# saiakarsh193/GenVox

Hardware: AMD Instinct MI355X
Metric: mel-frames/sec (teacher-forced batch) (higher is better)
Workload: dtype f32

## Files before the change

### genvox_amd/csrc/dec_resident.hip

```cpp
#include "gvx_kernels.h"

namespace gvx {

namespace {

using f32x16 = __attribute__((ext_vector_type(16))) float;

constexpr int RS_WAVES = 8;
constexpr int RS_THREADS = RS_WAVES * 64;
constexpr int RS_A = 1024, RS_D = 1024, RS_E = 512, RS_P = 256, RS_ATT = 128;
constexpr int RS_NKGW_ATT = (RS_P + RS_E + RS_A) / 8;
constexpr int RS_NKGW_DEC = (RS_A + RS_E + RS_D) / 8;
constexpr int RS_KG0_ATT = RS_P / 8;

template <int KIND> struct RsCfg {
    static constexpr bool XH = KIND == 0, ATT = KIND != 2;
    static constexpr int RT = KIND == 3 ? 2 : 1;
    static constexpr int NN = ATT ? 16 : 32, NC = 8;
    static constexpr int NRN = KIND == 0 ? 7 : (KIND == 1 ? 16 : (KIND == 2 ? 17 : 9));
    static constexpr int NLN = NN - NRN;
    static constexpr int WAVE_W = NLN * (XH ? 1536 : 1024 * RT);
    static constexpr int OFF_RED = RS_WAVES * WAVE_W;
    static constexpr int OFF_RED2 = OFF_RED + RS_WAVES * 16 * 64 * 4;
    static constexpr int OFF_HS = OFF_RED2 + (XH ? RS_WAVES * 8 * 64 * 4 : 0);
    static constexpr int OFF_HS2 = OFF_HS + 32 * 8 * 4 * RT;
    static constexpr int OFF_CTRL = OFF_HS2 + 32 * 4 * 4;
    static constexpr int LDS_BYTES = OFF_CTRL + 256;
};
constexpr int RS_LDS_BYTES = RsCfg<0>::LDS_BYTES > RsCfg<2>::LDS_BYTES ? RsCfg<0>::LDS_BYTES : RsCfg<2>::LDS_BYTES;
static_assert(RS_LDS_BYTES <= 160 * 1024 && RsCfg<1>::LDS_BYTES <= RS_LDS_BYTES && RsCfg<3>::LDS_BYTES <= RS_LDS_BYTES, "resident decoder LDS");
constexpr int RC_HA = 0;
constexpr int RC_CTX = 1;
constexpr int RC_HD = 2;
constexpr int RC_ABORT = 3;
constexpr int RC_LOCK = 4;
constexpr int RC_IDLE = 5;
constexpr int RC_PRE = 6;
constexpr int RC_Y1 = 7;
constexpr int RC_EXIT = 8;
constexpr int RC_WANT = 10;

struct RsArgs {
    const float* att_frag; const float* att_bias; const float* wq_t; const float* dec_frag; const float* dec_bias;
    const float* pre_gate;
    const float* proj_hd_t; const float* proj_ctx_t; const float* pre_w1; const uint8_t* keep1;
    float* prenet; const float* y1; float* p_slab; const int32_t* n_done; int PSB;
    float* h_a; float* hc; float* q_slab; float* c_a; float* c_d;
    const uint8_t* tr_keep_a; const uint8_t* tr_keep_d; float* tr_c_a; float* tr_c_d; float* tr_pre_a; float* tr_pre_d;
    float tr_scale_a, tr_scale_d;
    unsigned* sync;
    unsigned att_frag_bytes;
    int B, T;
    unsigned spin_limit;
    int debug, layout;
    int kg_pre;
};

#ifdef GVX_STAMPS
constexpr int RS_STAMP_T = 20;
__device__ unsigned long long rs_stamps[4][10][16];
__device__ unsigned long long rs_wg_stamps[224][4];
__device__ unsigned long long rs_wg_stamps_ar[224][4];
#define RS_STAMP(ev) do { if (stamp_wg && t == RS_STAMP_T && lane == 0) rs_stamps[KIND][wave][ev] = wall_clock64(); } while (0)
#define RS_WGSTAMP(i) do { if (t == RS_STAMP_T && tid == 0) rs_wg_stamps[bid][i] = wall_clock64(); } while (0)
#define RS_ARSTAMP(i) do { if (t == RS_STAMP_T && tid == 0) rs_wg_stamps_ar[bid][i] = wall_clock64(); } while (0)
#else
#define RS_STAMP(ev) do { } while (0)
#define RS_WGSTAMP(i) do { } while (0)
#define RS_ARSTAMP(i) do { } while (0)
#endif

__device__ __forceinline__ float sigmoidf_(float x) { return __builtin_amdgcn_rcpf(1.f + __expf(-x)); }
__device__ __forceinline__ float tanhf_(float x) { return 1.f - 2.f * __builtin_amdgcn_rcpf(__expf(2.f * x) + 1.f); }

struct RsPoll {
    const unsigned* f_att; const unsigned* f_dec; const unsigned* f_ctx; unsigned* tmo;
    const unsigned* f_pre; const unsigned* f_y1; const unsigned* stop;
    unsigned limit; int B, T, bid;
    int n_att;
    int sleep;
};

__device__ __forceinline__ bool rs_count(int* ctrl, int word, unsigned v, unsigned Tu, int lane) {
    const unsigned s0 = (unsigned)__hip_atomic_load(ctrl + word, __ATOMIC_RELAXED, __HIP_MEMORY_SCOPE_WORKGROUP);
    unsigned n = s0;
    while (n < Tu && __all(v > n)) ++n;
    if (lane == 0 && n != s0) __hip_atomic_store(ctrl + word, (int)n, __ATOMIC_RELEASE, __HIP_MEMORY_SCOPE_WORKGROUP);
    return n != s0;
}
__device__ __forceinline__ void rs_poll_once(int* ctrl, const RsPoll& q, int lane, int mask) {
    constexpr unsigned none = 0xffffffffu;
    unsigned va = none, vd = none, vc = none, vp = none, vy = none;
    if (mask & (1 << RC_HA)) {
        const unsigned a0 = __hip_atomic_load(q.f_att + lane, __ATOMIC_RELAXED, __HIP_MEMORY_SCOPE_AGENT);
        const unsigned a1 = lane + 64 < q.n_att ? __hip_atomic_load(q.f_att + 64 + lane, __ATOMIC_RELAXED, __HIP_MEMORY_SCOPE_AGENT) : none;
        va = min(a0, a1);
    }
    if (mask & (1 << RC_HD)) {
        const unsigned d0 = __hip_atomic_load(q.f_dec + lane, __ATOMIC_RELAXED, __HIP_MEMORY_SCOPE_AGENT);
        const unsigned d1 = __hip_atomic_load(q.f_dec + 64 + lane, __ATOMIC_RELAXED, __HIP_MEMORY_SCOPE_AGENT);
        vd = min(d0, d1);
    }
    if (mask & (1 << RC_CTX)) vc = lane < q.B ? __hip_atomic_load(q.f_ctx + lane * 32, __ATOMIC_RELAXED, __HIP_MEMORY_SCOPE_AGENT) : none;
    if (q.f_pre) {
        if (mask & (1 << RC_PRE)) vp = lane < 8 ? __hip_atomic_load(q.f_pre + lane * 32, __ATOMIC_RELAXED, __HIP_MEMORY_SCOPE_AGENT) : none;
        if (mask & (1 << RC_Y1)) vy = lane < q.B ? __hip_atomic_load(q.f_y1 + lane * 32, __ATOMIC_RELAXED, __HIP_MEMORY_SCOPE_AGENT) : none;
    }
    __builtin_amdgcn_fence(__ATOMIC_ACQUIRE, "wavefront");
    const unsigned Tu = (unsigned)q.T;
    bool moved = false;
    if (mask & (1 << RC_HA)) moved |= rs_count(ctrl, RC_HA, va, Tu, lane);
    if (mask & (1 << RC_HD)) moved |= rs_count(ctrl, RC_HD, vd, Tu, lane);
    if (mask & (1 << RC_CTX)) moved |= rs_count(ctrl, RC_CTX, vc, Tu, lane);
    if (q.f_pre) {
        if (mask & (1 << RC_PRE)) moved |= rs_count(ctrl, RC_PRE, vp, Tu, lane);
        if (mask & (1 << RC_Y1)) moved |= rs_count(ctrl, RC_Y1, vy, Tu, lane);
    }
    int idle = 0;
    if (lane == 0) {
        idle = moved ? 0 : __hip_atomic_load(ctrl + RC_IDLE, __ATOMIC_RELAXED, __HIP_MEMORY_SCOPE_WORKGROUP) + 1;
        __hip_atomic_store(ctrl + RC_IDLE, idle, __ATOMIC_RELAXED, __HIP_MEMORY_SCOPE_WORKGROUP);
    }
    idle = __builtin_amdgcn_readfirstlane(idle);
    if (idle == 0 || (idle & 15) != 0) return;
    bool give_up = __hip_atomic_load(q.tmo, __ATOMIC_RELAXED, __HIP_MEMORY_SCOPE_AGENT) != 0u;
    if (q.stop && __hip_atomic_load(q.stop, __ATOMIC_RELAXED, __HIP_MEMORY_SCOPE_AGENT) != 0u) give_up = true;
    if ((unsigned)idle > q.limit) {
        if (lane == 0) __hip_atomic_store(q.tmo, 0x500u + (unsigned)(q.bid & 0xff), __ATOMIC_RELAXED, __HIP_MEMORY_SCOPE_AGENT);
        give_up = true;
    }
    if (give_up && lane == 0) __hip_atomic_store(ctrl + RC_ABORT, 1, __ATOMIC_RELEASE, __HIP_MEMORY_SCOPE_WORKGROUP);
}

__device__ __forceinline__ void rs_gate(int* ctrl, int word, int need, const RsPoll& q, int lane) {
    while (__hip_atomic_load(ctrl + word, __ATOMIC_ACQUIRE, __HIP_MEMORY_SCOPE_WORKGROUP) < need) {
        if (__hip_atomic_load(ctrl + RC_ABORT, __ATOMIC_RELAXED, __HIP_MEMORY_SCOPE_WORKGROUP) != 0) return;
        int got = 0;
        if (lane == 0) {
            int expect = 0;
            got = __hip_atomic_compare_exchange_strong(ctrl + RC_LOCK, &expect, 1, __ATOMIC_ACQUIRE, __ATOMIC_RELAXED, __HIP_MEMORY_SCOPE_WORKGROUP) ? 1 : 0;
            if (got) got = __hip_atomic_exchange(ctrl + RC_WANT, 0, __ATOMIC_RELAXED, __HIP_MEMORY_SCOPE_WORKGROUP) | (1 << word);
            else __hip_atomic_fetch_or(ctrl + RC_WANT, 1 << word, __ATOMIC_RELAXED, __HIP_MEMORY_SCOPE_WORKGROUP);
        }
        got = __builtin_amdgcn_readfirstlane(got);
        if (got) {
            rs_poll_once(ctrl, q, lane, got);
            if (lane == 0) __hip_atomic_store(ctrl + RC_LOCK, 0, __ATOMIC_RELEASE, __HIP_MEMORY_SCOPE_WORKGROUP);
            if (q.sleep == 8) __builtin_amdgcn_s_sleep(8);
            else if (q.sleep == 32) __builtin_amdgcn_s_sleep(32);
        } else {
            __builtin_amdgcn_s_sleep(1);
        }
    }
}
__device__ __forceinline__ void rs_cbar() {
    asm volatile("s_waitcnt lgkmcnt(0)" ::: "memory");
    __builtin_amdgcn_s_barrier();
    asm volatile("" ::: "memory");
}

typedef __attribute__((ext_vector_type(4))) unsigned rs_u32x4;
__device__ __forceinline__ rs_u32x4 rs_rsrc(const void* p, unsigned bytes) {
    const unsigned long long a = reinterpret_cast<unsigned long long>(p);
    rs_u32x4 r;
    r.x = (unsigned)a; r.y = (unsigned)(a >> 32) & 0xffffu; r.z = bytes; r.w = 0x00020000u;
    return r;
}
__device__ __forceinline__ void rs_glds(rs_u32x4 rsrc, unsigned voff, unsigned soff, unsigned lds_addr) {
    unsigned keep;
    asm volatile("s_mov_b32 %0, m0\n\ts_mov_b32 m0, %1\n\ts_nop 0\n\tbuffer_load_dwordx4 %2, %3, %4 offen lds\n\ts_mov_b32 m0, %0"
                 : "=&s"(keep) : "s"(lds_addr), "v"(voff), "s"(rsrc), "s"(soff) : "memory");
}

#define RS_MFMA32(W, X)                                                   \
    acc = __builtin_amdgcn_mfma_f32_32x32x2f32((W).x, (X).x, acc, 0, 0, 0); \
    acc = __builtin_amdgcn_mfma_f32_32x32x2f32((W).y, (X).y, acc, 0, 0, 0); \
    acc = __builtin_amdgcn_mfma_f32_32x32x2f32((W).z, (X).z, acc, 0, 0, 0); \
    acc = __builtin_amdgcn_mfma_f32_32x32x2f32((W).w, (X).w, acc, 0, 0, 0);
#define RS_MFMA32B(W, X)                                                    \
    acc2 = __builtin_amdgcn_mfma_f32_32x32x2f32((W).x, (X).x, acc2, 0, 0, 0); \
    acc2 = __builtin_amdgcn_mfma_f32_32x32x2f32((W).y, (X).y, acc2, 0, 0, 0); \
    acc2 = __builtin_amdgcn_mfma_f32_32x32x2f32((W).z, (X).z, acc2, 0, 0, 0); \
    acc2 = __builtin_amdgcn_mfma_f32_32x32x2f32((W).w, (X).w, acc2, 0, 0, 0);
#define RS_MFMA16(W, X)                                                     \
    acc2 = __builtin_amdgcn_mfma_f32_16x16x1f32((W).x, (X).x, acc2, 0, 0, 0); \
    acc2 = __builtin_amdgcn_mfma_f32_16x16x1f32((W).y, (X).y, acc2, 0, 0, 0); \
    acc2 = __builtin_amdgcn_mfma_f32_16x16x1f32((W).z, (X).z, acc2, 0, 0, 0); \
    acc2 = __builtin_amdgcn_mfma_f32_16x16x1f32((W).w, (X).w, acc2, 0, 0, 0);

#define RS_VFMAC(A, W, X) asm("v_fmac_f32 %0, %1, %2" : "+v"(A) : "v"(W), "v"(X));
#define RS_VDOT(A, W, X) RS_VFMAC(A, (W).x, (X).x) RS_VFMAC(A, (W).y, (X).y) RS_VFMAC(A, (W).z, (X).z) RS_VFMAC(A, (W).w, (X).w)
#define RS_DPPSWAP(v) __int_as_float(__builtin_amdgcn_update_dpp(0, __float_as_int(v), 0xB1, 0xF, 0xF, true))
#define RS_XROW1(X) make_float4(RS_DPPSWAP((X).x), RS_DPPSWAP((X).y), RS_DPPSWAP((X).z), RS_DPPSWAP((X).w))
#define RS_MUL32(W, X) if (V) { RS_VDOT(av[0], W, X) if (two_rows) { const float4 x1_ = RS_XROW1(X); RS_VDOT(av[1], W, x1_) } } else { RS_MFMA32(W, X) }
#define RS_MUL32B(W, X) if (V) { RS_VDOT(av2[0], W, X) if (two_rows) { const float4 x1_ = RS_XROW1(X); RS_VDOT(av2[1], W, x1_) } } else { RS_MFMA32B(W, X) }
#define RS_MUL16(W, X) if (V) { RS_VDOT(av2[0], W, X) if (two_rows) { const float4 x1_ = RS_XROW1(X); RS_VDOT(av2[1], W, x1_) } } else { RS_MFMA16(W, X) }
template <bool B> struct RsBool { static constexpr bool value = B; };

}

typedef const __attribute__((address_space(4))) RsArgs* RsKarg;

template <int KIND, bool AR, bool TR = false, bool KA = AR>
__device__ __forceinline__ void rs_body(const RsArgs& p, char* smem, const int bid) {
    static_assert(!(AR && TR), "the tape belongs to the teacher-forced loop");
    using Cfg = RsCfg<KIND>;
    constexpr bool XH = Cfg::XH, ATT = Cfg::ATT;
    constexpr int NN = Cfg::NN, NC = Cfg::NC, NRN = Cfg::NRN, NLN = Cfg::NLN;
    constexpr int NKGW = ATT ? RS_NKGW_ATT : RS_NKGW_DEC;
    constexpr int H = ATT ? RS_A : RS_D;
    constexpr int NRH = XH ? NRN : 1, NCH = XH ? NC : 1;
    constexpr int RT = Cfg::RT;
    constexpr int NR2 = RT == 2 ? NRN : 1, NC2 = RT == 2 ? NC : 1;

    const int dec0 = p.layout == 2 ? 64 : 96;
    int tile, xt = 0, xhalf = 0;
    if (KIND == 0) { const int m = bid >> 1, odd = bid & 1; tile = 3 * m + 2 * odd; xt = 3 * m + 1; xhalf = odd; }
    else if (KIND == 1) tile = 96 + (bid - 64);
    else if (KIND == 3) tile = 2 * bid;
    else tile = bid - dec0;

    int* ctrl = reinterpret_cast<int*>(smem + Cfg::OFF_CTRL);
    float* red = reinterpret_cast<float*>(smem + Cfg::OFF_RED);
    float* red2 = reinterpret_cast<float*>(smem + Cfg::OFF_RED2);
    float* hs = reinterpret_cast<float*>(smem + Cfg::OFF_HS);
    float* hs2 = reinterpret_cast<float*>(smem + Cfg::OFF_HS2);
    const int tid = threadIdx.x, lane = tid & 63;
    const int wave = __builtin_amdgcn_readfirstlane(tid >> 6);
    const int B = p.B, T = p.T;
    const unsigned blkb = (unsigned)B * 32u;
    unsigned* const tmo_w = p.sync + HANDOFF_TIMEOUT;
    const int rep = bid % RS_REP;
    const RsPoll poll{p.sync + RS_FLAG_ATT + rep * 128, p.sync + RS_FLAG_DEC + rep * 128, p.sync + RS_FLAG_CTX + (bid % RS_REP1) * 32 * 32, tmo_w,
                      AR ? p.sync + RS_FLAG_PRE + (bid % RS_REP_PRE) * 8 * 32 : nullptr, AR ? p.sync + RS_FLAG_Y1 : nullptr, AR ? p.sync + HANDOFF_STOP : nullptr,
                      (p.spin_limit ? p.spin_limit : HANDOFF_SPIN_LIMIT) * 16u, B, T, bid, dec0,
                      (!ATT && (p.debug & 16)) ? 32 : ((p.debug & 8) ? 8 : 0)};
    const int bl = lane & 31, h = lane >> 5;
    const bool x_mine = ((lane >> 4) & 1) == xhalf;
    const int mlane = x_mine ? lane : (lane ^ 16);
    const bool vmode = B <= 2 && !(p.debug & 64), two_rows = B == 2;
    const unsigned x_lane = (unsigned)((vmode ? (two_rows ? (bl & 1) : 0) : (bl < B ? bl : 0)) * 8 + 4 * h) * 4u;

    const float4* wsrc = reinterpret_cast<const float4*>(ATT ? p.att_frag : p.dec_frag);
    constexpr bool ARD = AR && KIND == 2;
    constexpr bool PP = AR && ATT;
    constexpr int NSUB = ARD ? 2 : 1;
    const int kg_pre = AR ? RS_KG0_ATT : __builtin_amdgcn_readfirstlane(p.kg_pre);
    const int nkgw = ATT ? kg_pre + (RS_E + RS_A) / 8 : RS_NKGW_DEC;
    const int kn0 = ATT ? kg_pre + 64 + 16 * wave : (wave < 4 ? 32 * wave : 32 * wave + 64);
    auto kni = [&](int i) -> int { return ARD ? (i < 16 ? 192 + 16 * wave + i : 16 * wave + (i - 16)) : kn0 + i; };
    const int kc0 = ATT ? kg_pre + 8 * wave : 128 + 8 * wave;
    const float4* wt = wsrc + (long)tile * nkgw * 64 + lane;
    const float4* wx = wsrc + (long)xt * nkgw * 64 + mlane;
    float4 wn[NRN], wc[NC], hn[NRH], hc[NCH], wn2[NR2], wc2[NC2];
    const float4* wt2 = wt + (long)nkgw * 64;
#pragma unroll
    for (int i = 0; i < NRN; ++i) wn[i] = wt[(long)kni(i) * 64];
#pragma unroll
    for (int i = 0; i < NC; ++i) wc[i] = wt[(long)(kc0 + i) * 64];
#pragma unroll
    for (int i = 0; i < NR2; ++i) wn2[i] = RT == 2 ? wt2[(long)kni(i) * 64] : make_float4(0.f, 0.f, 0.f, 0.f);
#pragma unroll
    for (int i = 0; i < NC2; ++i) wc2[i] = RT == 2 ? wt2[(long)(kc0 + i) * 64] : make_float4(0.f, 0.f, 0.f, 0.f);
#pragma unroll
    for (int i = 0; i < NRH; ++i) hn[i] = XH ? wx[(long)kni(i) * 64] : make_float4(0.f, 0.f, 0.f, 0.f);
#pragma unroll
    for (int i = 0; i < NCH; ++i) hc[i] = XH ? wx[(long)(kc0 + i) * 64] : make_float4(0.f, 0.f, 0.f, 0.f);
    float4* lw = reinterpret_cast<float4*>(smem + wave * Cfg::WAVE_W);
    float4* lh = lw + NLN * 64;
    const int hidx = (mlane & 15) + 16 * (mlane >> 5);
#pragma unroll
    for (int i = 0; i < NLN; ++i) {
        lw[i * RT * 64 + lane] = wt[(long)kni(NRN + i) * 64];
        if (RT == 2) lw[(i * RT + 1) * 64 + lane] = wt2[(long)kni(NRN + i) * 64];
        if (XH && x_mine) lh[i * 32 + hidx] = wx[(long)kni(NRN + i) * 64];
    }

    constexpr int NP = (PP && KIND == 1) ? 4 : 1;
    float4 wp[NP], w1f[NP];
    const bool l2_wg = AR && KIND == 1 && bid - 64 < 8;
#pragma unroll
    for (int i = 0; i < NP; ++i) {
        wp[i] = (PP && KIND == 1) ? wt[(long)(4 * wave + i) * 64] : make_float4(0.f, 0.f, 0.f, 0.f);
        w1f[i] = l2_wg ? *reinterpret_cast<const float4*>(p.pre_w1 + (long)(32 * (bid - 64) + bl) * RS_P + 8 * (4 * wave + i) + 4 * h) : make_float4(0.f, 0.f, 0.f, 0.f);
    }
    const rs_u32x4 rw_att = rs_rsrc(p.att_frag, p.att_frag_bytes);
    const unsigned lds_base = (unsigned)(unsigned long long)(__attribute__((address_space(3))) char*)smem;
    const unsigned stage_t = lds_base + (unsigned)Cfg::OFF_RED + (unsigned)wave * 4096u;
    const unsigned stage_h = lds_base + (unsigned)Cfg::OFF_RED2 + (unsigned)wave * 2048u;
    const unsigned v_half = (((unsigned)bl < 16u ? 16u * (unsigned)xhalf + (unsigned)bl : 32u + 16u * (unsigned)xhalf + ((unsigned)bl - 16u)) * 16u) + (unsigned)h * 1024u;

    const bool cell_wave = wave < 4 * RT;
    const bool cell2_wave = XH && (wave == 4 || wave == 5);
    const int ctile = tile + (RT == 2 ? (wave >> 2) : 0);
    const int g = wave & 3, jloc = 2 * g + h, j = ctile * 8 + jloc;
    const int b2 = (lane & 15) + 16 * (wave - 4), g2 = lane >> 4, jloc2 = 4 * xhalf + g2, j2 = xt * 8 + jloc2;
    float* c_mem = ATT ? p.c_a : p.c_d;
    const float* bias = ATT ? p.att_bias : p.dec_bias;
    float c_state = 0.f;
    float4 bias4 = make_float4(0.f, 0.f, 0.f, 0.f);
    if (cell_wave) {
        if (bl < B) c_state = c_mem[(long)bl * H + j];
        bias4 = *reinterpret_cast<const float4*>(bias + ctile * 32 + 8 * g + 4 * h);
    } else if (cell2_wave) {
        if (b2 < B) c_state = c_mem[(long)b2 * H + j2];
        bias4 = *reinterpret_cast<const float4*>(bias + xt * 32 + 4 * jloc2);
    }
    const bool slab_wave = ATT ? wave < RS_ATT / 32 : (AR && wave < 3);

#ifdef GVX_STAMPS
    const bool stamp_wg = bid == 0 || bid == 64 || bid == dec0;
#endif
    for (int t = 0; t < T; ++t) {
        RS_STAMP(0);
        RS_WGSTAMP(0);
        RsKarg ka = nullptr;
        if (KA) { ka = (RsKarg)__builtin_amdgcn_kernarg_segment_ptr(); asm volatile("" : "+s"(ka)); }
        if (ATT && !AR && !TR && t >= RS_HA_SLOTS && (wave == 6 || ((XH || RT == 2) && wave == 7))) rs_gate(ctrl, RC_HD, t + 1 - RS_HA_SLOTS, poll, lane);
        float4 add4 = bias4;
        if (PP && XH) {
            const unsigned kg = (unsigned)(4 * wave);
#pragma unroll
            for (int i = 0; i < 4; ++i) rs_glds(rw_att, (unsigned)lane * 16u, ((unsigned)tile * NKGW + kg + (unsigned)i) * 1024u, stage_t + (unsigned)i * 1024u);
#pragma unroll
            for (int i = 0; i < 2; ++i) rs_glds(rw_att, v_half, ((unsigned)xt * NKGW + kg + 2u * (unsigned)i) * 1024u, stage_h + (unsigned)i * 1024u);
        }
        if (ATT && !PP) {
            if (cell_wave && bl < B) {
                const float4 ad = *reinterpret_cast<const float4*>(p.pre_gate + ((long)t * B + bl) * 4 * RS_A + ctile * 32 + 8 * g + 4 * h);
                add4.x += ad.x; add4.y += ad.y; add4.z += ad.z; add4.w += ad.w;
            } else if (cell2_wave && b2 < B) {
                const float4 ad = *reinterpret_cast<const float4*>(p.pre_gate + ((long)t * B + b2) * 4 * RS_A + xt * 32 + 4 * jloc2);
                add4.x += ad.x; add4.y += ad.y; add4.z += ad.z; add4.w += ad.w;
            }
        }
        f32x16 acc2x;
        float av2x[2] = {0.f, 0.f};
        auto body = [&](auto vc) __attribute__((always_inline)) {
        constexpr bool V = decltype(vc)::value;
        f32x16 acc, acc2;
#pragma unroll
        for (int q = 0; q < 16; ++q) { acc[q] = 0.f; acc2[q] = 0.f; }
        float av[2] = {0.f, 0.f}, av2[2] = {0.f, 0.f};
        auto prenet_part = [&]() __attribute__((always_inline)) {
            rs_gate(ctrl, RC_PRE, t, poll, lane);
            RS_ARSTAMP(2);
            const __amdgpu_buffer_rsrc_t rx = make_rsrc(ka->prenet + (long)(4 * wave) * B * 8);
            float4 xp[4];
#pragma unroll
            for (int u = 0; u < 4; ++u) xp[u] = load_sc1(rx, x_lane + (unsigned)u * blkb);
            if (XH) {
                asm volatile("s_waitcnt vmcnt(0)" ::: "memory");
                const float4* st = reinterpret_cast<const float4*>(red + wave * 16 * 64);
                const float4* sh = reinterpret_cast<const float4*>(red2 + wave * 8 * 64);
#pragma unroll
                for (int u = 0; u < 4; ++u) {
                    const float4 wl = st[u * 64 + lane];
                    const float4 hl = sh[u * 32 + hidx];
                    RS_MUL32(wl, xp[u])
                    RS_MUL16(hl, xp[u])
                }
            } else {
#pragma unroll
                for (int u = 0; u < 4; ++u) { RS_MUL32(wp[u < NP ? u : 0], xp[u]) }
            }
        };

        {
#pragma unroll
        for (int sub = 0; sub < NSUB; ++sub) {
            const float* xsrc;
            int word, need;
            if (ATT) { xsrc = p.h_a + (long)(TR ? t : t % RS_HA_SLOTS) * RS_A * B + (long)(16 * wave) * B * 8; word = RC_HA; need = t; }
            else if (ARD && sub == 0) { xsrc = p.hc + (long)t * B * (RS_D + RS_E) + (long)(16 * wave) * B * 8; word = RC_HD; need = t; }
            else if (ARD) { xsrc = p.h_a + (long)((t + 1) % RS_HA_SLOTS) * RS_A * B + (long)(16 * wave) * B * 8; word = RC_HA; need = t + 1; }
            else if (wave < 4) { xsrc = p.h_a + (long)(TR ? t + 1 : (t + 1) % RS_HA_SLOTS) * RS_A * B + (long)(32 * wave) * B * 8; word = RC_HA; need = t + 1; }
            else { xsrc = p.hc + (long)t * B * (RS_D + RS_E) + (long)(32 * (wave - 4)) * B * 8; word = RC_HD; need = t; }
            rs_gate(ctrl, word, need, poll, lane);
            if (sub == NSUB - 1) { RS_STAMP(1); RS_WGSTAMP(1); }
            const __amdgpu_buffer_rsrc_t rx = make_rsrc(xsrc);
            constexpr int XG = (XH || RT == 2) ? 2 : 4;
            constexpr int XD = ARD ? 3 : 2;
            constexpr int NNS = NN / NSUB;
            float4 xb[XD][XG];
#pragma unroll
            for (int d = 0; d < XD - 1; ++d)
#pragma unroll
                for (int u = 0; u < XG; ++u) xb[d][u] = load_sc1(rx, x_lane + (unsigned)(XG * d + u) * blkb);
#pragma unroll
            for (int gi = 0; gi < NNS / XG; ++gi) {
                if (gi + XD - 1 < NNS / XG) {
#pragma unroll
                    for (int u = 0; u < XG; ++u) xb[(gi + XD - 1) % XD][u] = load_sc1(rx, x_lane + (unsigned)(XG * (gi + XD - 1) + u) * blkb);
                }
#pragma unroll
                for (int u = 0; u < XG; ++u) {
                    const int i = sub * NNS + XG * gi + u;
                    const float4 xv = xb[gi % XD][u];
                    if (i < NRN) {
                        RS_MUL32(wn[i], xv)
                        if (XH) { RS_MUL16(hn[i < NRH ? i : 0], xv) }
                        if (RT == 2) { RS_MUL32B(wn2[i < NR2 ? i : 0], xv) }
                    } else {
                        const float4 wl = lw[(i - NRN) * RT * 64 + lane];
                        RS_MUL32(wl, xv)
                        if (XH) { const float4 hl = lh[(i - NRN) * 32 + hidx]; RS_MUL16(hl, xv) }
                        if (RT == 2) { const float4 wl2 = lw[((i - NRN) * RT + 1) * 64 + lane]; RS_MUL32B(wl2, xv) }
                    }
                }
            }
        }
        }
        RS_STAMP(2);
        {
            const float* xsrc = p.hc + (long)(ATT ? t : t + 1) * B * (RS_D + RS_E) + (long)RS_D * B + (long)(8 * wave) * B * 8;
            if (ATT) rs_gate(ctrl, RC_CTX, t, poll, lane);
            else if (AR) rs_gate(ctrl, RC_CTX, t + 1, poll, lane);
            else if (t + 2 <= T) rs_gate(ctrl, RC_HA, t + 2, poll, lane);
            else rs_gate(ctrl, RC_CTX, t + 1, poll, lane);
            RS_STAMP(3);
            RS_WGSTAMP(2);
            const __amdgpu_buffer_rsrc_t rx = make_rsrc(xsrc);
            constexpr int XG = 4;
            float4 xc[XG], xn[XG];
#pragma unroll
            for (int u = 0; u < XG; ++u) xc[u] = load_sc1(rx, x_lane + (unsigned)u * blkb);
#pragma unroll
            for (int gi = 0; gi < NC / XG; ++gi) {
                if (gi + 1 < NC / XG) {
#pragma unroll
                    for (int u = 0; u < XG; ++u) xn[u] = load_sc1(rx, x_lane + (unsigned)(XG * (gi + 1) + u) * blkb);
                }
#pragma unroll
                for (int u = 0; u < XG; ++u) {
                    const int i = XG * gi + u;
                    RS_MUL32(wc[i], xc[u])
                    if (XH) { RS_MUL16(hc[i < NCH ? i : 0], xc[u]) }
                    if (RT == 2) { RS_MUL32B(wc2[i < NC2 ? i : 0], xc[u]) }
                }
#pragma unroll
                for (int u = 0; u < XG; ++u) xc[u] = xn[u];
            }
        }
        if (AR && KIND == 1) {
            if (l2_wg && t >= 1) {
                unsigned km = 0;
                if (wave < 4 && bl < B) km = *reinterpret_cast<const unsigned*>(ka->keep1 + ((long)t * B + bl) * RS_P + 32 * (bid - 64) + 8 * wave + 4 * h);
                rs_gate(ctrl, RC_Y1, t, poll, lane);
                RS_ARSTAMP(0);
                const __amdgpu_buffer_rsrc_t ry = make_rsrc(ka->y1 + (long)(4 * wave) * B * 8);
                float4 xy[4];
#pragma unroll
                for (int u = 0; u < 4; ++u) xy[u] = load_sc1(ry, x_lane + (unsigned)u * blkb);
                if (bid == 64 && tid == 0 && __hip_atomic_load(ka->n_done, __ATOMIC_RELAXED, __HIP_MEMORY_SCOPE_AGENT) >= B) {
                    __hip_atomic_store(p.sync + HANDOFF_STOP, (unsigned)t, __ATOMIC_RELAXED, __HIP_MEMORY_SCOPE_AGENT);
                    __hip_atomic_store(ctrl + RC_ABORT, 2, __ATOMIC_RELAXED, __HIP_MEMORY_SCOPE_WORKGROUP);
                }
                if (V) {
#pragma unroll
                    for (int u = 0; u < 4; ++u) { RS_MUL32B(w1f[u < NP ? u : 0], xy[u]) }
                    if (two_rows && (lane & 1)) { const float s2 = av2[0]; av2[0] = av2[1]; av2[1] = s2; }
#pragma unroll
                    for (int b = 0; b < 2; ++b) {
                        av2[b] += __shfl_xor(av2[b], 32, 64);
                        if (h == 0 && b < B) red[(wave * 16 + 4 * (bl >> 3) + (bl & 3)) * 64 + b + 32 * ((bl >> 2) & 1)] = av2[b];
                        av2[b] = 0.f;
                    }
                } else {
#pragma unroll
                    for (int u = 0; u < 4; ++u) { RS_MFMA32B(w1f[u < NP ? u : 0], xy[u]) }
#pragma unroll
                    for (int q = 0; q < 16; ++q) { red[(wave * 16 + q) * 64 + lane] = acc2[q]; acc2[q] = 0.f; }
                }
                rs_cbar();
                if (wave < 4) {
                    float4 o;
                    float* op = &o.x;
#pragma unroll
                    for (int qq = 0; qq < 4; ++qq) {
                        float tt = 0.f;
#pragma unroll
                        for (int w = 0; w < RS_WAVES; ++w) tt += red[(w * 16 + 4 * wave + qq) * 64 + lane];
                        op[qq] = tt;
                    }
                    if (bl < B) {
                        o.x = (km & 0xffu) ? 2.f * fmaxf(o.x, 0.f) : 0.f;
                        o.y = (km & 0xff00u) ? 2.f * fmaxf(o.y, 0.f) : 0.f;
                        o.z = (km & 0xff0000u) ? 2.f * fmaxf(o.z, 0.f) : 0.f;
                        o.w = (km & 0xff000000u) ? 2.f * fmaxf(o.w, 0.f) : 0.f;
                        const __amdgpu_buffer_rsrc_t rp = make_rsrc(ka->prenet + (long)(4 * (bid - 64) + wave) * B * 8);
                        store_sc1(rp, (unsigned)(bl * 8 + 4 * h) * 4u, o);
                    }
                    asm volatile("s_waitcnt vmcnt(0)" ::: "memory");
                }
                rs_cbar();
                if (tid < RS_REP_PRE && __hip_atomic_load(ctrl + RC_ABORT, __ATOMIC_RELAXED, __HIP_MEMORY_SCOPE_WORKGROUP) == 0)
                    __hip_atomic_store(p.sync + RS_FLAG_PRE + (tid * 8 + (bid - 64)) * 32, (unsigned)t, __ATOMIC_RELAXED, __HIP_MEMORY_SCOPE_AGENT);
                RS_ARSTAMP(1);
            }
        }
        if (AR && PP) prenet_part();
        RS_STAMP(4);
        if (AR) RS_ARSTAMP(3);
        {
        int tr = tid;
        asm volatile("" : "+v"(tr));
        const int el = tr & 63;
        if (V) {
            const int en = el & 31;
            if (two_rows && (el & 1)) {
                const float s0 = av[0], s2 = av2[0];
                av[0] = av[1]; av[1] = s0; av2[0] = av2[1]; av2[1] = s2;
            }
#pragma unroll
            for (int b = 0; b < 2; ++b) {
                av[b] += __shfl_xor(av[b], 32, 64);
                if (XH || RT == 2) av2[b] += __shfl_xor(av2[b], 32, 64);
                if (el < 32 && b < B) red[(wave * 16 + 4 * (en >> 3) + (en & 3)) * 64 + b + 32 * ((en >> 2) & 1)] = av[b];
                if (XH && el < 32 && ((el >> 4) & 1) == xhalf && b < B) red2[(wave * 8 + (el & 3)) * 64 + b + 16 * ((el & 15) >> 2)] = av2[b];
            }
        } else {
#pragma unroll
            for (int q = 0; q < 16; ++q) red[(wave * 16 + q) * 64 + el] = acc[q];
            if (XH) {
#pragma unroll
                for (int q = 0; q < 8; ++q) red2[(wave * 8 + q) * 64 + el] = acc2[q] + acc2[8 + q];
            }
        }
        if (RT == 2) {
            if (V) { av2x[0] = av2[0]; av2x[1] = av2[1]; } else acc2x = acc2;
        }
        }
        };
        if (vmode) body(RsBool<true>{}); else body(RsBool<false>{});

        int te = tid;
        asm volatile("" : "+v"(te));
        const int el = te & 63, ebl = el & 31, eh = el >> 5;
        float4 wq_a = make_float4(0.f, 0.f, 0.f, 0.f), wq_b = wq_a, wq_c = wq_a, wq_d = wq_a;
        float4 xe = wq_a;
        if (AR && !ATT && slab_wave) {
            const int dd = min(32 * wave + ebl, ka->PSB - 1);
            const float* wp_l = ka->proj_hd_t + ((long)tile * ka->PSB + dd) * 8;
            wq_a = *reinterpret_cast<const float4*>(wp_l);
            wq_b = *reinterpret_cast<const float4*>(wp_l + 4);
            wq_c = *reinterpret_cast<const float4*>(ka->proj_ctx_t + ((long)tile * ka->PSB + dd) * 4);
            const __amdgpu_buffer_rsrc_t rc = make_rsrc(p.hc + (long)(t + 1) * B * (RS_D + RS_E) + (long)RS_D * B + (long)(tile >> 1) * B * 8);
            xe = load_sc1(rc, (unsigned)((ebl < B ? ebl : 0) * 8 + 4 * (tile & 1)) * 4u);
        }
        if (ATT && slab_wave) {
            const float* wq_l = p.wq_t + ((long)tile * RS_ATT + 32 * wave + ebl) * 8;
            wq_a = *reinterpret_cast<const float4*>(wq_l);
            wq_b = *reinterpret_cast<const float4*>(wq_l + 4);
            if (XH) wq_c = *reinterpret_cast<const float4*>(p.wq_t + ((long)xt * RS_ATT + 32 * wave + ebl) * 8 + 4 * xhalf);
            if (RT == 2) {
                const float* wq_l2 = p.wq_t + ((long)(tile + 1) * RS_ATT + 32 * wave + ebl) * 8;
                wq_c = *reinterpret_cast<const float4*>(wq_l2);
                wq_d = *reinterpret_cast<const float4*>(wq_l2 + 4);
            }
        }
        rs_cbar();
        RS_STAMP(5);
        if (cell2_wave) {
            const int rb = wave - 4;
            const int eb2 = (el & 15) + 16 * rb, eg2 = el >> 4;
            float s2[4];
#pragma unroll
            for (int qq = 0; qq < 4; ++qq) {
                float tt = 0.f;
#pragma unroll
                for (int w = 0; w < RS_WAVES; ++w) tt += red2[(w * 8 + 4 * rb + qq) * 64 + el];
                s2[qq] = tt;
            }
            float hval = 0.f;
            if (eb2 < B) {
                const float p0 = s2[0] + add4.x, p1 = s2[1] + add4.y, p2 = s2[2] + add4.z, p3 = s2[3] + add4.w;
                c_state = sigmoidf_(p1) * c_state + sigmoidf_(p0) * tanhf_(p2);
                hval = sigmoidf_(p3) * tanhf_(c_state);
                if (TR) {
                    RsKarg kq = (RsKarg)__builtin_amdgcn_kernarg_segment_ptr();
                    asm volatile("" : "+s"(kq));
                    const unsigned u = (unsigned)eb2 * (unsigned)H + (unsigned)(xt * 8 + 4 * xhalf + eg2);
                    const long tb = (long)t * B * H;
                    reinterpret_cast<float4*>(kq->tr_pre_a + tb * 4)[u] = make_float4(p0, p1, p2, p3);
                    (kq->tr_c_a + tb + (long)B * H)[u] = c_state;
                    hval = (kq->tr_keep_a + tb)[u] ? hval * kq->tr_scale_a : 0.f;
                }
            }
            hs2[eb2 * 4 + eg2] = hval;
        }
#pragma unroll
        for (int ph = 0; ph < RT; ++ph) {
            if (ph == 1) {
                rs_cbar();
                if (vmode) {
                    const int en = el & 31;
#pragma unroll
                    for (int b = 0; b < 2; ++b)
                        if (el < 32 && b < B) red[(wave * 16 + 4 * (en >> 3) + (en & 3)) * 64 + b + 32 * ((en >> 2) & 1)] = av2x[b];
                } else {
#pragma unroll
                    for (int q = 0; q < 16; ++q) red[(wave * 16 + q) * 64 + el] = acc2x[q];
                }
                rs_cbar();
            }
            if (cell_wave && (wave >> 2) == ph) {
                float s[4];
#pragma unroll
                for (int qq = 0; qq < 4; ++qq) {
                    float tt = 0.f;
#pragma unroll
                    for (int w = 0; w < RS_WAVES; ++w) tt += red[(w * 16 + 4 * g + qq) * 64 + el];
                    s[qq] = tt;
                }
                float hval = 0.f;
                if (ebl < B) {
                    const float p0 = s[0] + add4.x, p1 = s[1] + add4.y, p2 = s[2] + add4.z, p3 = s[3] + add4.w;
                    c_state = sigmoidf_(p1) * c_state + sigmoidf_(p0) * tanhf_(p2);
                    hval = sigmoidf_(p3) * tanhf_(c_state);
                    if (TR) {
                        RsKarg kq = (RsKarg)__builtin_amdgcn_kernarg_segment_ptr();
                        asm volatile("" : "+s"(kq));
                        const unsigned u = (unsigned)ebl * (unsigned)H + (unsigned)((tile + (RT == 2 ? ph : 0)) * 8 + 2 * g + eh);
                        const long tb = (long)t * B * H;
                        reinterpret_cast<float4*>((ATT ? kq->tr_pre_a : kq->tr_pre_d) + tb * 4)[u] = make_float4(p0, p1, p2, p3);
                        ((ATT ? kq->tr_c_a : kq->tr_c_d) + tb + (long)B * H)[u] = c_state;
                        hval = ((ATT ? kq->tr_keep_a : kq->tr_keep_d) + tb)[u] ? hval * (ATT ? kq->tr_scale_a : kq->tr_scale_d) : 0.f;
                    }
                }
                hs[(ebl * RT + ph) * 8 + 2 * g + eh] = hval;
            }
        }
        rs_cbar();
        RS_STAMP(6);

        float* hdst = ATT ? p.h_a + (long)(TR ? t + 1 : (t + 1) % RS_HA_SLOTS) * RS_A * B : p.hc + (long)(t + 1) * B * (RS_D + RS_E);
        if (slab_wave) {
            f32x16 qa;
#pragma unroll
            for (int q = 0; q < 16; ++q) qa[q] = 0.f;
            const float* hrow = hs + ebl * 8 * RT + eh;
            qa = __builtin_amdgcn_mfma_f32_32x32x2f32(hrow[0], eh ? wq_a.y : wq_a.x, qa, 0, 0, 0);
            qa = __builtin_amdgcn_mfma_f32_32x32x2f32(hrow[2], eh ? wq_a.w : wq_a.z, qa, 0, 0, 0);
            qa = __builtin_amdgcn_mfma_f32_32x32x2f32(hrow[4], eh ? wq_b.y : wq_b.x, qa, 0, 0, 0);
            qa = __builtin_amdgcn_mfma_f32_32x32x2f32(hrow[6], eh ? wq_b.w : wq_b.z, qa, 0, 0, 0);
            if (RT == 2) {
                qa = __builtin_amdgcn_mfma_f32_32x32x2f32(hrow[8], eh ? wq_c.y : wq_c.x, qa, 0, 0, 0);
                qa = __builtin_amdgcn_mfma_f32_32x32x2f32(hrow[10], eh ? wq_c.w : wq_c.z, qa, 0, 0, 0);
                qa = __builtin_amdgcn_mfma_f32_32x32x2f32(hrow[12], eh ? wq_d.y : wq_d.x, qa, 0, 0, 0);
                qa = __builtin_amdgcn_mfma_f32_32x32x2f32(hrow[14], eh ? wq_d.w : wq_d.z, qa, 0, 0, 0);
            }
            if (XH) {
                const float* hrow2 = hs2 + ebl * 4 + eh;
                qa = __builtin_amdgcn_mfma_f32_32x32x2f32(hrow2[0], eh ? wq_c.y : wq_c.x, qa, 0, 0, 0);
                qa = __builtin_amdgcn_mfma_f32_32x32x2f32(hrow2[2], eh ? wq_c.w : wq_c.z, qa, 0, 0, 0);
            }
            if (AR && !ATT) {
                qa = __builtin_amdgcn_mfma_f32_32x32x2f32(eh ? xe.y : xe.x, eh ? wq_c.y : wq_c.x, qa, 0, 0, 0);
                qa = __builtin_amdgcn_mfma_f32_32x32x2f32(eh ? xe.w : xe.z, eh ? wq_c.w : wq_c.z, qa, 0, 0, 0);
            }
            float* tq = red + wave * 16 * 64;
#pragma unroll
            for (int gg = 0; gg < 4; ++gg)
#pragma unroll
                for (int rr = 0; rr < 4; ++rr) tq[(8 * gg + 4 * eh + rr) * 32 + ebl] = qa[4 * gg + rr];
            const int sdim = ATT ? RS_ATT : ka->PSB;
            const __amdgpu_buffer_rsrc_t rq = make_rsrc(ATT ? p.q_slab + (long)bid * B * RS_ATT + 32 * wave : ka->p_slab + (long)tile * B * sdim + 32 * wave);
#pragma unroll
            for (int ps = 0; ps < 4; ++ps) {
                const int row = 8 * ps + (el >> 3), c4 = el & 7;
                const float4 v = *reinterpret_cast<const float4*>(tq + row * 32 + 4 * c4);
                if (row < B && (ATT || 32 * wave + 4 * c4 < sdim)) store_sc1(rq, (unsigned)(row * sdim + 4 * c4) * 4u, v);
            }
        } else if (wave == 6) {
            const __amdgpu_buffer_rsrc_t rh = make_rsrc(hdst + (long)tile * B * 8);
            if (4 * el < 8 * B) store_sc1(rh, (unsigned)el * 16u, *reinterpret_cast<const float4*>(hs + (el >> 1) * 8 * RT + 4 * (el & 1)));
        } else if (RT == 2 && wave == 7) {
            const __amdgpu_buffer_rsrc_t rh = make_rsrc(hdst + (long)(tile + 1) * B * 8);
            if (4 * el < 8 * B) store_sc1(rh, (unsigned)el * 16u, *reinterpret_cast<const float4*>(hs + (el >> 1) * 16 + 8 + 4 * (el & 1)));
        } else if (XH && wave == 7) {
            const __amdgpu_buffer_rsrc_t rh = make_rsrc(hdst + (long)xt * B * 8);
            if (el < B) store_sc1(rh, (unsigned)(el * 8 + 4 * xhalf) * 4u, *reinterpret_cast<const float4*>(hs2 + 4 * el));
        }
        RS_STAMP(7);
        asm volatile("s_waitcnt vmcnt(0)" ::: "memory");
        RS_STAMP(8);
        if (AR && tid == 0) ctrl[RC_EXIT + (t & 1)] = __hip_atomic_load(ctrl + RC_ABORT, __ATOMIC_RELAXED, __HIP_MEMORY_SCOPE_WORKGROUP);
        rs_cbar();
        RS_STAMP(9);
        const bool leave = AR && __builtin_amdgcn_readfirstlane(ctrl[RC_EXIT + (t & 1)]) != 0;
        if (leave) break;
        int tf = tid;
        asm volatile("" : "+v"(tf));
        if (tf < RS_REP) __hip_atomic_store(p.sync + (ATT ? RS_FLAG_ATT + bid : RS_FLAG_DEC + (bid - dec0)) + tf * 128, (unsigned)t + 1u, __ATOMIC_RELAXED, __HIP_MEMORY_SCOPE_AGENT);
        else if (ATT && tf < RS_REP + RS_REP1)
            __hip_atomic_store(p.sync + RS_FLAG_Q + ((tf - RS_REP) * dec0 + bid) * 32, (unsigned)t + 1u, __ATOMIC_RELAXED, __HIP_MEMORY_SCOPE_AGENT);
        else if (AR && !ATT && tf < RS_REP + RS_REP_P)
            __hip_atomic_store(p.sync + RS_FLAG_P + ((tf - RS_REP) * 128 + (bid - dec0)) * 32, (unsigned)t + 1u, __ATOMIC_RELAXED, __HIP_MEMORY_SCOPE_AGENT);
        RS_WGSTAMP(3);
    }
    if (cell_wave && bl < B) c_mem[(long)bl * H + j] = c_state;
    if (cell2_wave && b2 < B) c_mem[(long)b2 * H + j2] = c_state;
}

template <bool TR>
__device__ __forceinline__ void rs_kernel_224(const RsArgs& p, char* rs_smem) {
    const int bid = (int)blockIdx.x;
    const int kind = bid < 64 ? 0 : (bid < 96 ? 1 : 2);
    const int off_ctrl = kind == 0 ? RsCfg<0>::OFF_CTRL : (kind == 1 ? RsCfg<1>::OFF_CTRL : RsCfg<2>::OFF_CTRL);
    if (threadIdx.x < 64) reinterpret_cast<int*>(rs_smem + off_ctrl)[threadIdx.x] = 0;
    __syncthreads();
    if (kind == 0) rs_body<0, false, TR, !TR>(p, rs_smem, bid);
    else if (kind == 1) rs_body<1, false, TR, !TR>(p, rs_smem, bid);
    else rs_body<2, false, TR, !TR>(p, rs_smem, bid);
}
template <bool TR>
__device__ __forceinline__ void rs_kernel_192(const RsArgs& p, char* rs_smem) {
    const int bid = (int)blockIdx.x;
    const int kind = bid < 64 ? 3 : 2;
    const int off_ctrl = kind == 3 ? RsCfg<3>::OFF_CTRL : RsCfg<2>::OFF_CTRL;
    if (threadIdx.x < 64) reinterpret_cast<int*>(rs_smem + off_ctrl)[threadIdx.x] = 0;
    __syncthreads();
    if (kind == 3) rs_body<3, false, TR>(p, rs_smem, bid);
    else rs_body<2, false, TR>(p, rs_smem, bid);
}
__global__ __launch_bounds__(RS_THREADS) void decoder_resident_kernel(RsArgs p) {
    extern __shared__ __attribute__((aligned(16))) char rs_smem[];
    rs_kernel_224<false>(p, rs_smem);
}
__global__ __launch_bounds__(RS_THREADS) void decoder_resident_pairs_kernel(RsArgs p) {
    extern __shared__ __attribute__((aligned(16))) char rs_smem[];
    rs_kernel_192<false>(p, rs_smem);
}

__global__ __launch_bounds__(RS_THREADS) void decoder_resident_train_kernel(RsArgs p) {
    extern __shared__ __attribute__((aligned(16))) char rs_smem[];
    rs_kernel_224<true>(p, rs_smem);
}
__global__ __launch_bounds__(RS_THREADS) void decoder_resident_train_pairs_kernel(RsArgs p) {
    extern __shared__ __attribute__((aligned(16))) char rs_smem[];
    rs_kernel_192<true>(p, rs_smem);
}

__global__ __launch_bounds__(RS_THREADS) void decoder_ar_resident_kernel(RsArgs p) {
    extern __shared__ __attribute__((aligned(16))) char rs_smem[];
    const int bid = (int)blockIdx.x;
    const int kind = bid < 64 ? 0 : (bid < 96 ? 1 : 2);
    const int off_ctrl = kind == 0 ? RsCfg<0>::OFF_CTRL : (kind == 1 ? RsCfg<1>::OFF_CTRL : RsCfg<2>::OFF_CTRL);
    if (threadIdx.x < 64) reinterpret_cast<int*>(rs_smem + off_ctrl)[threadIdx.x] = 0;
    __syncthreads();
    if (kind == 0) rs_body<0, true>(p, rs_smem, bid);
    else if (kind == 1) rs_body<1, true>(p, rs_smem, bid);
    else rs_body<2, true>(p, rs_smem, bid);
}

#ifdef GVX_STAMPS
hipError_t read_stamps_resident(unsigned long long* host480) {
    return hipMemcpyFromSymbol(host480, HIP_SYMBOL(rs_stamps), sizeof(unsigned long long) * 480);
}
hipError_t read_wg_stamps_resident_ar(unsigned long long* host896) {
    return hipMemcpyFromSymbol(host896, HIP_SYMBOL(rs_wg_stamps_ar), sizeof(unsigned long long) * 896);
}
hipError_t read_wg_stamps_resident(unsigned long long* host896) {
    return hipMemcpyFromSymbol(host896, HIP_SYMBOL(rs_wg_stamps), sizeof(unsigned long long) * 896);
}
#endif

hipError_t decoder_resident_init() {
    hipError_t e = hipFuncSetAttribute(reinterpret_cast<const void*>(decoder_resident_kernel), hipFuncAttributeMaxDynamicSharedMemorySize, RS_LDS_BYTES);
    if (e != hipSuccess) return e;
    for (const void* k : {reinterpret_cast<const void*>(decoder_resident_train_kernel), reinterpret_cast<const void*>(decoder_resident_pairs_kernel),
                          reinterpret_cast<const void*>(decoder_resident_train_pairs_kernel)})
        if ((e = hipFuncSetAttribute(k, hipFuncAttributeMaxDynamicSharedMemorySize, RS_LDS_BYTES)) != hipSuccess) return e;
    return hipFuncSetAttribute(reinterpret_cast<const void*>(decoder_ar_resident_kernel), hipFuncAttributeMaxDynamicSharedMemorySize, RS_LDS_BYTES);
}

bool decoder_resident_supported(int B, int L) { const int lay = attention_persistent_layout(B, L); return lay == 1 || lay == 2; }

hipError_t launch_decoder_resident(const DecResidentParams& p, hipStream_t s) {
    if (p.B < 1 || p.B > 32 || p.T < 1 || !p.att_frag || !p.dec_frag || !p.att_bias || !p.dec_bias || !p.wq_t || !p.pre_gate || !p.h_a ||
        !p.hc || !p.q_slab || !p.c_a || !p.c_d || !p.sync)
        return hipErrorInvalidValue;
    if (p.layout != 1 && p.layout != 2) return hipErrorInvalidValue;
    if (p.kg_pre < 1 || (size_t)p.att_frag_bytes != (size_t)128 * (size_t)(p.kg_pre + (RS_E + RS_A) / 8) * 1024) return hipErrorInvalidValue;
    RsArgs a{};
    a.att_frag = p.att_frag; a.att_bias = p.att_bias; a.wq_t = p.wq_t; a.dec_frag = p.dec_frag; a.dec_bias = p.dec_bias;
    a.pre_gate = p.pre_gate; a.h_a = p.h_a; a.hc = p.hc; a.q_slab = p.q_slab; a.c_a = p.c_a; a.c_d = p.c_d; a.sync = p.sync;
    a.att_frag_bytes = p.att_frag_bytes; a.B = p.B; a.T = p.T; a.spin_limit = p.spin_limit; a.debug = p.debug; a.layout = p.layout;
    a.kg_pre = p.kg_pre;
    const dim3 grid(p.layout == 2 ? 192 : 224);
    if (p.tr_keep_a) {
        if (!p.tr_keep_d || !p.tr_c_a || !p.tr_c_d || !p.tr_pre_a || !p.tr_pre_d) return hipErrorInvalidValue;
        a.tr_keep_a = p.tr_keep_a; a.tr_keep_d = p.tr_keep_d; a.tr_c_a = p.tr_c_a; a.tr_c_d = p.tr_c_d; a.tr_pre_a = p.tr_pre_a; a.tr_pre_d = p.tr_pre_d;
        a.tr_scale_a = p.tr_scale_a; a.tr_scale_d = p.tr_scale_d;
        if (p.layout == 2) decoder_resident_train_pairs_kernel<<<grid, dim3(RS_THREADS), RS_LDS_BYTES, s>>>(a);
        else decoder_resident_train_kernel<<<grid, dim3(RS_THREADS), RS_LDS_BYTES, s>>>(a);
    } else if (p.layout == 2) {
        decoder_resident_pairs_kernel<<<grid, dim3(RS_THREADS), RS_LDS_BYTES, s>>>(a);
    } else {
        decoder_resident_kernel<<<grid, dim3(RS_THREADS), RS_LDS_BYTES, s>>>(a);
    }
    return hipGetLastError();
}

hipError_t launch_decoder_ar_resident(const ArResidentParams& p, hipStream_t s) {
    if (p.B < 1 || p.B > 32 || p.T < 1 || !p.att_frag || !p.dec_frag || !p.att_bias || !p.dec_bias || !p.wq_t || !p.proj_hd_t || !p.proj_ctx_t ||
        !p.pre_w1 || !p.keep1 || !p.prenet || !p.y1 || !p.h_a || !p.hc || !p.q_slab || !p.p_slab || !p.c_a || !p.c_d || !p.n_done || !p.sync)
        return hipErrorInvalidValue;
    if (p.PSB < 8 || p.PSB > 96 || (p.PSB & 3) || p.att_frag_bytes == 0) return hipErrorInvalidValue;
    RsArgs a{};
    a.att_frag = p.att_frag; a.att_bias = p.att_bias; a.wq_t = p.wq_t; a.dec_frag = p.dec_frag; a.dec_bias = p.dec_bias;
    a.proj_hd_t = p.proj_hd_t; a.proj_ctx_t = p.proj_ctx_t; a.pre_w1 = p.pre_w1; a.keep1 = p.keep1; a.prenet = p.prenet; a.y1 = p.y1;
    a.p_slab = p.p_slab; a.n_done = p.n_done; a.PSB = p.PSB;
    a.h_a = p.h_a; a.hc = p.hc; a.q_slab = p.q_slab; a.c_a = p.c_a; a.c_d = p.c_d; a.sync = p.sync;
    a.att_frag_bytes = p.att_frag_bytes; a.B = p.B; a.T = p.T; a.spin_limit = p.spin_limit; a.debug = p.debug; a.layout = 1;
    a.kg_pre = RS_KG0_ATT;
    decoder_ar_resident_kernel<<<dim3(224), dim3(RS_THREADS), RS_LDS_BYTES, s>>>(a);
    return hipGetLastError();
}

}
```

### genvox_amd/csrc/gvx_api.hip

```cpp
#include "gvx_internal.h"

namespace gvx {
#ifdef GVX_STAMPS
hipError_t read_stamps_skinny(unsigned long long* host96);
hipError_t read_stamps_attention(unsigned long long* host96);
hipError_t read_stamps_persist(unsigned long long* host96);
hipError_t read_wg_spans(unsigned long long* host1024);
hipError_t read_stamps_resident(unsigned long long* host480);
hipError_t read_wg_stamps_resident(unsigned long long* host896);
hipError_t read_wg_stamps_resident_ar(unsigned long long* host896);
hipError_t read_row_stamps_persist_ar(unsigned long long* host256);
hipError_t read_loc_stamps_persist(unsigned long long* host32);
hipError_t read_row_stamps_persist(unsigned long long* host512);
#endif
hipError_t skinny_init();
hipError_t gemm_init();
hipError_t attention_init();
hipError_t attention_persistent_init();
}

using namespace gvx;

namespace {
thread_local std::string g_err;
std::mutex g_capture_mutex;
}
namespace gvx {
int set_error(int code, const char* msg) { g_err = msg; return code; }

int fail(int code, const char* fmt, ...) {
    char buf[1024];
    va_list ap;
    va_start(ap, fmt);
    vsnprintf(buf, sizeof buf, fmt, ap);
    va_end(ap);
    g_err = buf;
    return code;
}

std::mutex& capture_mutex() { return g_capture_mutex; }

WsPlan make_ws_plan(const gvx_model* m, int B, int L, int T, int mode) {
    const gvx_dims& d = m->d;
    const int E = d.embed_dim, H = E / 2, M = d.n_mels, P = d.prenet_dim, A = d.att_rnn_dim, D = d.dec_rnn_dim;
    const int pe = (d.enc_kernel - 1) / 2, pp = (d.postnet_kernel - 1) / 2;
    WsPlan w{};
    size_t off = 0;
    auto take = [&](size_t floats) { size_t o = off; off = align_up(off + floats * sizeof(float), 256); return o; };
    w.flags = take(128);
    w.sync = take(HANDOFF_WORDS);
    w.xa = take((size_t)B * (L + 2 * pe) * E);
    w.xb = take((size_t)B * (L + 2 * pe) * E);
    w.xg = take((size_t)B * L * 8 * H);
    w.enc_h = take((size_t)2 * 2 * B * H);
    w.enc_c = take((size_t)2 * B * H);
    w.memory = take((size_t)B * L * E);
    w.len_copy = take((size_t)B);
    w.pm = take((size_t)B * L * d.att_dim);
    w.frames = take((size_t)(T + 1) * B * M);
    w.pre1 = take((size_t)(T + 1) * B * P);
    w.prenet = take((size_t)(T + 1) * B * P);
    w.h_a = take((size_t)RS_HA_SLOTS * B * A);
    w.c_a = take((size_t)B * A);
    w.c_d = take((size_t)B * D);
    w.hc = take((size_t)(T + 1) * B * (D + E));
    w.w_cum = take((size_t)B * L);
    w.q_slab = take((size_t)(A / 8) * B * d.att_dim);
    w.proj = take((size_t)B * T * m->PSB());
    w.energies = take((size_t)B * L);
    w.align_tm = take((size_t)T * B * L);
    w.loc = take((size_t)B * L * d.att_dim);
    w.p_slab = take((size_t)(D / 8) * B * m->PSB());
    w.p_ctx = take((size_t)B * m->PSB());
    w.att_part = take((size_t)2 * B * 4 * A);
    w.dec_part = take((size_t)2 * B * 4 * D);
    w.pre_gate = take(mode == WS_TEACHER_FORCED && plan_teacher_forced(m, B, L, TF_INFERENCE).pre_gate ? (size_t)T * B * 4 * A : 0);
    w.xchg = take(attention_persistent_xchg_floats(B));
    w.ar_masks = take(((size_t)2 * T * B * P + 3) / 4);
    const int cmax = d.postnet_dim > M ? d.postnet_dim : M;
    w.ya = take((size_t)B * (T + 2 * pp) * cmax);
    w.yb = take((size_t)B * (T + 2 * pp) * cmax);
    w.total = off;
    return w;
}

gvx_model::GraphSet* touch_graph_set(gvx_model* m, std::vector<gvx_model::GraphSet>& cache, const gvx_model::LoopKey& key) {
    gvx_model::GraphSet* hit = nullptr;
    for (auto& gs : cache)
        if (gs.key == key) hit = &gs;
    if (!hit) {
        if (cache.size() >= gvx_model::GRAPH_SETS) {
            size_t lru = 0;
            for (size_t i = 1; i < cache.size(); ++i)
                if (cache[i].last_use < cache[lru].last_use) lru = i;
            for (auto e : cache[lru].execs)
                if (e) (void)hipGraphExecDestroy(e);
            cache.erase(cache.begin() + lru);
        }
        cache.emplace_back();
        hit = &cache.back();
        hit->key = key;
    }
    ++hit->sightings;
    hit->last_use = ++m->use_clock;
    return hit;
}

int check_common(const gvx_model* m, int B, int L, int T, void* ws, size_t ws_bytes, int mode) {
    if (!m) return fail(GVX_ERR_INVALID_ARG, "null model");
    if (!m->dev_blob) return fail(GVX_ERR_STATE, "weights not bound (call gvx_model_bind_blob)");
    if (B < 1 || B > 64) return fail(GVX_ERR_UNSUPPORTED, "batch %d not in [1, 64] (shard larger batches across calls / GPUs)", B);
    if (L < 1 || T < 1) return fail(GVX_ERR_INVALID_ARG, "L and T must be >= 1");
    if (!ws) return fail(GVX_ERR_WORKSPACE, "null workspace");
    if (reinterpret_cast<uintptr_t>(ws) & 255) return fail(GVX_ERR_WORKSPACE, "workspace must be 256-byte aligned");
    const size_t need = make_ws_plan(m, B, L, T, mode).total;
    if (ws_bytes < need) return fail(GVX_ERR_WORKSPACE, "workspace too small: %zu < %zu bytes", ws_bytes, need);
    if (!attention_supported(L, m->d.att_dim, m->d.att_loc_filters, m->d.att_loc_kernel, m->d.embed_dim))
        return fail(GVX_ERR_UNSUPPORTED, "L = %d is too long for the attention kernels' LDS budget", L);
    return GVX_OK;
}

}

namespace {

int check_dims(const gvx_dims& d) {
    if (d.n_tokens < 1) return fail(GVX_ERR_INVALID_ARG, "n_tokens must be >= 1");
    const int dims8[] = {d.embed_dim, d.prenet_dim, d.att_rnn_dim, d.dec_rnn_dim, d.att_dim, d.postnet_dim, d.n_mels};
    const char* names[] = {"embed_dim", "prenet_dim", "att_rnn_dim", "dec_rnn_dim", "att_dim", "postnet_dim", "n_mels"};
    for (int i = 0; i < 7; ++i)
        if (dims8[i] < 8 || dims8[i] % 8) return fail(GVX_ERR_UNSUPPORTED, "%s = %d must be a positive multiple of 8", names[i], dims8[i]);
    if (d.embed_dim % 16) return fail(GVX_ERR_UNSUPPORTED, "embed_dim = %d must be a multiple of 16 (BiLSTM halves are multiples of 8)", d.embed_dim);
    if (d.att_dim > 256) return fail(GVX_ERR_UNSUPPORTED, "att_dim = %d > 256 is not supported", d.att_dim);
    if (d.att_loc_filters < 1 || d.att_loc_filters > 32) return fail(GVX_ERR_UNSUPPORTED, "att_loc_filters = %d must be in [1, 32]", d.att_loc_filters);
    const int ks[] = {d.enc_kernel, d.att_loc_kernel, d.postnet_kernel};
    for (int k : ks)
        if (k < 1 || k % 2 == 0) return fail(GVX_ERR_UNSUPPORTED, "kernel size %d must be odd (the reference pads (k-1)/2 on both sides)", k);
    if (d.enc_n_conv < 1 || d.enc_n_conv > MAX_CONV || d.postnet_n_conv < 1 || d.postnet_n_conv > MAX_CONV)
        return fail(GVX_ERR_UNSUPPORTED, "number of convolutions must be in [1, %d]", MAX_CONV);
    return GVX_OK;
}

void read_knobs(gvx_model* m) {
    auto env = [](const char* name) { const char* e = std::getenv(name); return e ? e : ""; };
    auto flag = [&](const char* name, bool dflt) { const char c = env(name)[0]; return c == '\0' ? dflt : dflt ? c != '0' : c == '1'; };
    auto number = [&](const char* name, int dflt) { const char* e = env(name); return e[0] ? std::atoi(e) : dflt; };
    m->use_graph = !flag("GVX_NO_GRAPH", false);
    m->capture_first = flag("GVX_GRAPH_FIRST", false);
    m->attn_one_launch = !flag("GVX_ATTN_SPLIT", false);
    m->attn_persistent = flag("GVX_ATTN_PERSISTENT", true);
    for (const char* name : {"AMD_SERIALIZE_KERNEL", "HIP_LAUNCH_BLOCKING"})
        if (env(name)[0] != '\0' && env(name)[0] != '0') m->attn_persistent = false;
    m->ar_resident = flag("GVX_AR_RESIDENT", false);
    m->ar_split_h = flag("GVX_AR_SPLIT_H", true);
    m->enc_persistent = flag("GVX_ENC_PERSISTENT", true);
    m->enc_fork_after = number("GVX_ENC_FORK_AFTER", 1);
    m->train_resident = flag("GVX_TRAIN_RESIDENT", true);
    m->train_resident_loop = flag("GVX_TRAIN_RESIDENT_LOOP", true);
    m->tf_rows64 = flag("GVX_TF_ROWS64", false);
    m->tf_resident = flag("GVX_TF_RESIDENT", true);
    m->ar_resident_loop = flag("GVX_AR_RESIDENT_LOOP", true);
    m->tf_long_rows_224 = flag("GVX_TF_LONG_224", true);
    m->attn_prefetch = flag("GVX_ATTN_PREFETCH", true);
    m->pa_depth = number("GVX_PA_DEPTH", 4) == 6 ? 6 : 4;
    m->side_pool = env("GVX_SIDE_POOL")[0] == '2' ? 2u : 1u;
    m->spin_limit = (unsigned)std::strtoul(env("GVX_HANDOFF_SPIN_LIMIT"), nullptr, 10);
    m->rs_debug = number("GVX_RS_DEBUG", 0);
    m->debug_skip_resident = flag("GVX_DEBUG_SKIP_RESIDENT", false);
    m->debug_enc_skip_block = number("GVX_DEBUG_ENC_SKIP_BLOCK", -1);
    m->debug_plan = std::getenv("GVX_DEBUG_PLAN") != nullptr;
}

}

extern "C" {

const char* gvx_last_error(void) { return g_err.c_str(); }
int gvx_version(void) { return 1; }

int gvx_model_create(const gvx_dims* dims, gvx_model** out) {
    if (!dims || !out) return fail(GVX_ERR_INVALID_ARG, "null argument");
    int rc = check_dims(*dims);
    if (rc != GVX_OK) return rc;
    gvx_model* m = new gvx_model();
    m->d = *dims;
    m->blob = make_blob_layout(*dims);
    read_knobs(m);
    *out = m;
    return GVX_OK;
}

void gvx_model_destroy(gvx_model* m) {
    if (m) {
        if (m->gather_off) (void)hipFree(m->gather_off);
        if (m->gather_tid) (void)hipFree(m->gather_tid);
    }
    if (!m) return;
    if (m->ev_valid)
        for (auto& e : m->ev) (void)hipEventDestroy(e);
    for (auto& e : m->kev) (void)hipEventDestroy(e);
    m->drop_graphs();
    if (m->cap_stream) (void)hipStreamDestroy(m->cap_stream);
    if (m->pa_fork) (void)hipEventDestroy(m->pa_fork);
    if (m->pa_join) (void)hipEventDestroy(m->pa_join);
    if (m->enc_mid) (void)hipEventDestroy(m->enc_mid);
    if (m->ar_done_host) (void)hipHostFree(m->ar_done_host);
    for (hipEvent_t e : m->ar_ev)
        if (e) (void)hipEventDestroy(e);
    delete m;
}

size_t gvx_model_blob_bytes(const gvx_model* m) { return m ? m->blob.total * sizeof(float) : 0; }

int gvx_model_bind_blob(gvx_model* m, const void* device_blob) {
    if (!m || !device_blob) return fail(GVX_ERR_INVALID_ARG, "null argument");
    if (reinterpret_cast<uintptr_t>(device_blob) & 255) return fail(GVX_ERR_INVALID_ARG, "blob must be 256-byte aligned");
    if (m->dev_blob != device_blob) m->drop_graphs();
    m->dev_blob = reinterpret_cast<const float*>(device_blob);
    HIP_TRY(gemm_init());
    HIP_TRY(skinny_init());
    HIP_TRY(attention_init());
    HIP_TRY(attention_persistent_init());
    HIP_TRY(decoder_resident_init());
    return GVX_OK;
}

size_t gvx_workspace_bytes(const gvx_model* m, int B, int L, int T) {
    if (!m || B < 1 || L < 1 || T < 1) return 0;
    return make_ws_plan(m, B, L, T).total;
}

size_t gvx_workspace_bytes_autoregressive(const gvx_model* m, int B, int L, int max_steps) {
    if (!m || B < 1 || L < 1 || max_steps < 1) return 0;
    return make_ws_plan(m, B, L, max_steps, WS_AUTOREGRESSIVE).total;
}

}

namespace {

int conv_layer(const gvx_model* m, const float* in, float* out, int B, int T, int cin, int cout, int k, size_t w_off, size_t b_off,
               int act, int out_halo, hipStream_t s) {
    const int p = (k - 1) / 2;
    GemmParams g{};
    g.A = in; g.amap = RowMap{T, (long)(T + 2 * p) * cin, (long)cin};
    g.W = m->dev_blob + w_off; g.ldw = (long)k * cin;
    g.C = out + (long)out_halo * cout; g.cmap = RowMap{T, (long)(T + 2 * out_halo) * cout, (long)cout};
    g.bias = m->dev_blob + b_off;
    g.M = B * T; g.N = cout; g.K = k * cin; g.act = act;
    HIP_TRY(launch_gemm(g, s));
    return GVX_OK;
}

int encoder_impl(gvx_model* m, const int64_t* tokens, const int32_t* lengths, int B, int L, float* memory_out, void* ws,
                 const WsPlan& wp, hipStream_t s, const float* conv_out = nullptr, float* c_seq_out = nullptr, float* xg_out = nullptr,
                 hipEvent_t dense_done = nullptr) {
    const gvx_dims& d = m->d;
    const int E = d.embed_dim, H = E / 2, pe = (d.enc_kernel - 1) / 2;
    float* xa = ws_ptr<float>(ws, wp.xa);
    float* xb = ws_ptr<float>(ws, wp.xb);
    float* xg = ws_ptr<float>(ws, wp.xg);
    float* enc_h = ws_ptr<float>(ws, wp.enc_h);
    float* enc_c = ws_ptr<float>(ws, wp.enc_c);
    int* flags = ws_ptr<int>(ws, wp.flags);
    float* cur = xa;
    float* nxt = xb;
    if (conv_out) {
        HIP_TRY(launch_to_channels_last(conv_out, xa, B, E, L, pe, nullptr, s));
    } else {
        HIP_TRY(launch_embed(tokens, m->dev_blob + m->blob.emb, d.n_tokens, xa, xb, B, L, E, pe, flags + FLAG_TOKEN, s));
        for (int i = 0; i < d.enc_n_conv; ++i) {
            if (dense_done && i == m->enc_fork_after) { HIP_TRY(hipEventRecord(dense_done, s)); dense_done = nullptr; }
            int rc = conv_layer(m, cur, nxt, B, L, E, E, d.enc_kernel, m->blob.enc_w[i], m->blob.enc_b[i], ACT_RELU, pe, s);
            if (rc != GVX_OK) return rc;
            float* t = cur; cur = nxt; nxt = t;
        }
    }
    if (dense_done) HIP_TRY(hipEventRecord(dense_done, s));
    {
        GemmParams g{};
        g.A = cur + (long)pe * E; g.amap = RowMap{L, (long)(L + 2 * pe) * E, (long)E};
        g.W = m->dev_blob + m->blob.enc_wih; g.ldw = E;
        g.C = xg; g.cmap = RowMap{B * L, 0, (long)8 * H};
        g.bias = m->dev_blob + m->blob.enc_bih;
        g.M = B * L; g.N = 8 * H; g.K = E; g.act = ACT_NONE;
        HIP_TRY(launch_gemm(g, s));
    }
    const bool resident = m->enc_persistent && encoder_persistent_supported(B, H);
    if (!resident) HIP_TRY(zero_async(enc_h, (size_t)4 * B * H * sizeof(float), s));
    if (!resident) HIP_TRY(zero_async(enc_c, (size_t)2 * B * H * sizeof(float), s));
    float* mem_ws = ws_ptr<float>(ws, wp.memory);
    if (!resident) HIP_TRY(zero_async(mem_ws, (size_t)B * L * E * sizeof(float), s));
    const int32_t* len_ws = nullptr;
    if (lengths) {
        int32_t* lc = ws_ptr<int32_t>(ws, wp.len_copy);
        HIP_TRY(hipMemcpyAsync(lc, lengths, (size_t)B * sizeof(int32_t), hipMemcpyDeviceToDevice, s));
        len_ws = lc;
    }
    auto enqueue = [&](hipStream_t st) -> int {
        for (int step = 0; step < L; ++step) {
            SkinnyJob jobs[2];
            for (int dir = 0; dir < 2; ++dir) {
                SkinnyJob& J = jobs[dir];
                std::memset(&J, 0, sizeof J);
                float* h_cur = enc_h + ((size_t)dir * 2 + (step & 1)) * B * H;
                float* h_nxt = enc_h + ((size_t)dir * 2 + ((step + 1) & 1)) * B * H;
                J.Wp = m->dev_blob + m->blob.enc_whh_frag[dir];
                J.x[0] = XSeg{h_cur, H};
                J.N = 4 * H; J.nkg = H / 8; J.mode = 0; J.B = B;
                J.c = enc_c + (size_t)dir * B * H;
                J.h_out = h_nxt;
                J.addend = xg + (size_t)dir * 4 * H; J.add_bs = (long)L * 8 * H; J.add_ts = 8 * H;
                J.lengths = len_ws; J.step = step; J.reverse = dir; J.seq_len = L;
                J.seq_out = mem_ws + (size_t)dir * H; J.seq_bs = (long)L * E; J.seq_ts = E;
                if (c_seq_out) J.c_seq_out = c_seq_out + (size_t)dir * H;
                J.h_prev = h_cur;
            }
            HIP_TRY(launch_skinny(jobs, 2, SK_ENCODER, st));
        }
        return GVX_OK;
    };
    if (resident) {
        unsigned* sync = ws_ptr<unsigned>(ws, wp.sync);
        void* const zp[2] = {enc_h, sync + HANDOFF_TIMEOUT};
        const size_t zb[2] = {(size_t)4 * B * H * sizeof(float), sizeof(unsigned)};
        HIP_TRY(launch_zero_many(zp, zb, 2, s));
        EncPersistParams ep{};
        ep.Wp[0] = m->dev_blob + m->blob.enc_whh_frag[0]; ep.Wp[1] = m->dev_blob + m->blob.enc_whh_frag[1];
        ep.xg = xg; ep.lengths = len_ws; ep.hx = enc_h; ep.seq_out = mem_ws; ep.c_seq_out = c_seq_out;
        ep.sync = sync; ep.spin_limit = m->spin_limit; ep.B = B; ep.L = L; ep.H = H;
        ep.debug_skip_block = m->debug_enc_skip_block;
        HIP_TRY(launch_encoder_persistent(ep, s));
        float* outs[2] = {mem_ws, c_seq_out};
        const size_t counts[2] = {(size_t)B * L * E, (size_t)B * L * E};
        HIP_TRY(launch_poison_on_timeout(sync + HANDOFF_TIMEOUT, flags + FLAG_TIMEOUT, outs, counts, c_seq_out ? 2 : 1, s));
    } else {
        const gvx_model::LoopKey key{ws, mem_ws, m->dev_blob, B, L, 0, lengths != nullptr};
        const int rc = run_chunk(m, m->use_graph && !c_seq_out ? touch_graph_set(m, m->enc_graphs, key) : nullptr, 0, s, enqueue);
        if (rc != GVX_OK) return rc;
    }
    if (xg_out) HIP_TRY(hipMemcpyAsync(xg_out, xg, (size_t)B * L * 8 * H * sizeof(float), hipMemcpyDeviceToDevice, s));
    if (memory_out != mem_ws)
        HIP_TRY(hipMemcpyAsync(memory_out, mem_ws, (size_t)B * L * E * sizeof(float), hipMemcpyDeviceToDevice, s));
    return GVX_OK;
}

int postnet_impl(gvx_model* m, const float* mel_in, const int32_t* mel_lengths, int B, int T, float* mel_post_out, float* ya,
                 float* yb, hipStream_t s) {
    const gvx_dims& d = m->d;
    const int M = d.n_mels, pp = (d.postnet_kernel - 1) / 2, n = d.postnet_n_conv;
    HIP_TRY(launch_to_channels_last(mel_in, ya, B, M, T, pp, mel_lengths, s));
    float* cur = ya;
    float* nxt = yb;
    for (int i = 0; i < n; ++i) {
        const int cin = i == 0 ? M : d.postnet_dim, cout = i == n - 1 ? M : d.postnet_dim;
        const bool last = i == n - 1;
        const int out_halo = last ? 0 : pp;
        const bool fused_halo = out_halo > 0 && T >= out_halo;
        if (out_halo > 0 && !fused_halo) HIP_TRY(launch_zero_halo(nxt, B, T, pp, cout, s));
        GemmParams g{};
        g.A = cur; g.amap = RowMap{T, (long)(T + 2 * pp) * cin, (long)cin};
        g.W = m->dev_blob + m->blob.post_w[i]; g.ldw = (long)d.postnet_kernel * cin;
        g.C = nxt + (long)out_halo * cout; g.cmap = RowMap{T, (long)(T + 2 * out_halo) * cout, (long)cout};
        g.bias = m->dev_blob + m->blob.post_b[i];
        g.M = B * T; g.N = cout; g.K = d.postnet_kernel * cin; g.act = last ? ACT_NONE : ACT_TANH;
        g.row_len = last ? nullptr : mel_lengths;
        g.c_halo = fused_halo ? out_halo : 0;
        HIP_TRY(launch_gemm(g, s));
        float* t = cur; cur = nxt; nxt = t;
    }
    HIP_TRY(launch_residual_to_channels_first(mel_in, cur, mel_post_out, B, M, T, mel_lengths, s));
    return GVX_OK;
}

struct PostnetPlan { size_t ya, yb, total; };
PostnetPlan make_postnet_plan(const gvx_model* m, int B, int T) {
    const gvx_dims& d = m->d;
    const int pp = (d.postnet_kernel - 1) / 2, cmax = d.postnet_dim > d.n_mels ? d.postnet_dim : d.n_mels;
    const size_t buf = align_up((size_t)B * (T + 2 * pp) * cmax * sizeof(float), 256);
    PostnetPlan p;
    p.ya = align_up((128 + HANDOFF_WORDS) * sizeof(float), 256);
    p.yb = p.ya + buf;
    p.total = p.yb + buf;
    return p;
}

}

extern "C" {

int gvx_teacher_forced_rows_per_call(const gvx_model* m, int L) {
    if (!m) return 0;
    return plan_teacher_forced(m, 64, L, TF_INFERENCE).kind != 0 ? 64 : 32;
}

int gvx_teacher_forced_resident(const gvx_model* m, int B, int L) {
    if (!m || B < 1 || L < 1) return 0;
    return plan_teacher_forced(m, B, L, TF_INFERENCE).kind != 0 ? 1 : 0;
}

int gvx_teacher_forced_loop_kind(const gvx_model* m, int B, int L) {
    if (!m || B < 1 || L < 1) return 0;
    return plan_teacher_forced(m, B, L, TF_INFERENCE).kind;
}

int gvx_autoregressive_loop_kind(const gvx_model* m, int B, int L) {
    if (!m || B < 1 || L < 1) return 0;
    return plan_autoregressive(m, B, L).kind;
}

int gvx_autoregressive_windowed_loop_kind(const gvx_model* m, int B, int L) {
    if (!m || B < 1 || L < 1) return 0;
    return plan_autoregressive(m, B, L, true).kind;
}

int gvx_debug_decoder_plan_windowed(const gvx_model* m, int B, int L, int* out) {
    if (!m || !out) return fail(GVX_ERR_INVALID_ARG, "null argument");
    if (B < 1 || L < 1) return fail(GVX_ERR_INVALID_ARG, "B, L >= 1 (got %d, %d)", B, L);
    const ArLoopPlan a = plan_autoregressive(m, B, L, true);
    out[0] = a.kind; out[1] = a.split_h; out[2] = a.fold; out[3] = a.graph;
    return GVX_OK;
}

int gvx_debug_decoder_plan(const gvx_model* m, int mode, int B, int L, int* out) {
    if (!m || !out) return fail(GVX_ERR_INVALID_ARG, "null argument");
    if (mode < 0 || mode > 2 || B < 1 || L < 1) return fail(GVX_ERR_INVALID_ARG, "mode must be 0, 1 or 2 and B, L >= 1 (got %d, %d, %d)", mode, B, L);
    const TfLoopPlan t = plan_teacher_forced(m, B, L, (TfMode)mode);
    const ArLoopPlan a = plan_autoregressive(m, B, L);
    const int v[12] = {t.kind, t.pa_layout, t.tile_layout, t.rows64, t.pre_gate, t.timeout_check, t.side_stream, t.graph,
                       a.kind, a.split_h, a.fold, a.graph};
    for (int i = 0; i < 12; ++i) out[i] = v[i];
    return GVX_OK;
}

long long gvx_debug_graph_replays(const gvx_model* m) { return m ? (long long)m->graph_replays : -1; }

int gvx_debug_encoder_resident(const gvx_model* m, int B) {
    if (!m || B < 1) return 0;
    return m->enc_persistent && encoder_persistent_supported(B, m->H()) ? 1 : 0;
}

int gvx_model_set_persistent_attention(gvx_model* m, int enable) {
    if (!m) return fail(GVX_ERR_INVALID_ARG, "null argument");
    m->attn_persistent = enable != 0;
    return GVX_OK;
}

int gvx_model_set_resident_kernels(gvx_model* m, int enable) {
    if (!m) return fail(GVX_ERR_INVALID_ARG, "null argument");
    m->attn_persistent = m->enc_persistent = m->tf_resident = enable != 0;
    if (!enable) m->ar_resident = false;
    return GVX_OK;
}

int gvx_workspace_status(const gvx_model* m, void* ws, size_t ws_bytes, void* stream, int32_t* host_out) {
    if (!m || !ws || !host_out) return fail(GVX_ERR_INVALID_ARG, "null argument");
    const WsPlan wp = make_ws_plan(m, 1, 1, 1, WS_AUTOREGRESSIVE);
    if (ws_bytes < wp.flags + 4 * sizeof(int32_t)) return fail(GVX_ERR_WORKSPACE, "workspace too small");
    hipStream_t s = (hipStream_t)stream;
    int32_t h[4] = {0, 0, 0, 0}, tmo = 0;
    int32_t* flags = ws_ptr<int32_t>(ws, wp.flags);
    HIP_TRY(hipMemcpyAsync(h, flags, sizeof h, hipMemcpyDeviceToHost, s));
    if (ws_bytes >= wp.sync + HANDOFF_WORDS * sizeof(unsigned))
        HIP_TRY(hipMemcpyAsync(&tmo, reinterpret_cast<const char*>(ws) + wp.sync + HANDOFF_TIMEOUT * sizeof(unsigned), sizeof tmo,
                               hipMemcpyDeviceToHost, s));
    HIP_TRY(zero_async(flags + FLAG_TOKEN, sizeof(int32_t), s));
    HIP_TRY(zero_async(flags + FLAG_TIMEOUT, sizeof(int32_t), s));
    if (ws_bytes >= wp.sync + HANDOFF_WORDS * sizeof(unsigned))
        HIP_TRY(zero_async(ws_ptr<unsigned>(ws, wp.sync) + HANDOFF_TIMEOUT, sizeof(unsigned), s));
    HIP_TRY(hipStreamSynchronize(s));
    host_out[0] = h[FLAG_TOKEN];
    host_out[1] = h[FLAG_TIMEOUT] ? h[FLAG_TIMEOUT] : tmo;
    return GVX_OK;
}

int gvx_encoder_forward(gvx_model* m, const int64_t* tokens, const int32_t* lengths, int B, int L, float* memory_out,
                        void* ws, size_t ws_bytes, void* stream) {
    int rc = check_common(m, B, L, 1, ws, ws_bytes, WS_AUTOREGRESSIVE);
    if (rc != GVX_OK) return rc;
    if (!tokens || !memory_out) return fail(GVX_ERR_INVALID_ARG, "null argument");
    return encoder_impl(m, tokens, lengths, B, L, memory_out, ws, make_ws_plan(m, B, L, 1, WS_AUTOREGRESSIVE), (hipStream_t)stream);
}

int gvx_decoder_teacher_forced(gvx_model* m, const float* memory, const int32_t* lengths, int B, int L, const float* mel_in, int T,
                               const uint8_t* keep_masks, float* mel_out, float* gate_out, float* align_out, void* ws,
                               size_t ws_bytes, void* stream) {
    int rc = check_common(m, B, L, T, ws, ws_bytes);
    if (rc != GVX_OK) return rc;
    if (!memory || !mel_in || !keep_masks || !mel_out || !gate_out || !align_out) return fail(GVX_ERR_INVALID_ARG, "null argument");
    const WsPlan wp = make_ws_plan(m, B, L, T);
    rc = decoder_tf_impl(m, memory, lengths, B, L, mel_in, T, keep_masks, mel_out, gate_out, align_out, ws, wp, (hipStream_t)stream);
    if (rc != GVX_OK) return rc;
    float* outs[3] = {mel_out, gate_out, align_out};
    const size_t counts[3] = {(size_t)B * m->d.n_mels * T, (size_t)B * T, (size_t)B * T * L};
    return poison_if_timed_out(m, B, L, ws, wp, outs, counts, 3, (hipStream_t)stream);
}

int gvx_encoder_lstm_forward(gvx_model* m, const float* conv_out, const int32_t* lengths, int B, int L, float* memory_out,
                             float* cell_states_out, float* input_preact_out, void* ws, size_t ws_bytes, void* stream) {
    int rc = check_common(m, B, L, 1, ws, ws_bytes, WS_AUTOREGRESSIVE);
    if (rc != GVX_OK) return rc;
    if (!conv_out || !memory_out) return fail(GVX_ERR_INVALID_ARG, "null argument");
    if (cell_states_out) HIP_TRY(zero_async(cell_states_out, (size_t)B * L * m->d.embed_dim * sizeof(float), (hipStream_t)stream));
    return encoder_impl(m, nullptr, lengths, B, L, memory_out, ws, make_ws_plan(m, B, L, 1, WS_AUTOREGRESSIVE), (hipStream_t)stream, conv_out,
                        cell_states_out, input_preact_out);
}

int gvx_decoder_teacher_forced_train(gvx_model* m, const float* memory, const int32_t* lengths, int B, int L, const float* mel_in, int T,
                                     const uint8_t* keep_masks, const uint8_t* att_keep, const uint8_t* dec_keep, float p_att, float p_dec,
                                     float* mel_out, float* gate_out, float* align_out, float* att_hidden_all, float* att_cell_all,
                                     float* dec_cell_all, float* dec_hidden_context_all, float* att_preact_all, float* dec_preact_all,
                                     void* ws, size_t ws_bytes, void* stream) {
    int rc = check_common(m, B, L, T, ws, ws_bytes);
    if (rc != GVX_OK) return rc;
    if (!memory || !mel_in || !keep_masks || !att_keep || !dec_keep || !mel_out || !gate_out || !align_out) return fail(GVX_ERR_INVALID_ARG, "null argument");
    if (!(p_att >= 0.f && p_att < 1.f && p_dec >= 0.f && p_dec < 1.f)) return fail(GVX_ERR_INVALID_ARG, "dropout probabilities must be in [0, 1)");
    if (plan_teacher_forced(m, B, L, TF_TRAIN_PARTIAL_TAPE).rows64)
        return fail(GVX_ERR_UNSUPPORTED, "training mode with %d rows on a GVX_TF_ROWS64 handle: the 64-row loop has no dropout and no tape (at most 32 rows per call)", B);
    hipStream_t s = (hipStream_t)stream;
    const int A = m->d.att_rnn_dim, D = m->d.dec_rnn_dim, E = m->d.embed_dim;
    const LstmDropout tr{att_keep, dec_keep, 1.f / (1.f - p_att), 1.f / (1.f - p_dec), att_hidden_all, att_cell_all, dec_cell_all, att_preact_all, dec_preact_all};
    if (att_hidden_all) HIP_TRY(zero_async(att_hidden_all, (size_t)B * A * sizeof(float), s));
    if (att_cell_all) HIP_TRY(zero_async(att_cell_all, (size_t)B * A * sizeof(float), s));
    if (dec_cell_all) HIP_TRY(zero_async(dec_cell_all, (size_t)B * D * sizeof(float), s));
    const WsPlan wp = make_ws_plan(m, B, L, T);
    rc = decoder_tf_impl(m, memory, lengths, B, L, mel_in, T, keep_masks, mel_out, gate_out, align_out, ws, wp, s, false, &tr);
    if (rc != GVX_OK) return rc;
    {
        float* outs[3] = {mel_out, gate_out, align_out};
        const size_t counts[3] = {(size_t)B * m->d.n_mels * T, (size_t)B * T, (size_t)B * T * L};
        rc = poison_if_timed_out(m, B, L, ws, wp, outs, counts, 3, s);
        if (rc != GVX_OK) return rc;
    }
    if (dec_hidden_context_all)
        HIP_TRY(hipMemcpyAsync(dec_hidden_context_all, ws_ptr<float>(ws, wp.hc), (size_t)(T + 1) * B * (D + E) * sizeof(float),
                               hipMemcpyDeviceToDevice, s));
    return GVX_OK;
}

int gvx_train_export(const gvx_model* m, const void* ws_c, size_t ws_bytes, int B, int L, int T, int what, float* dst, void* stream) {
    void* ws = const_cast<void*>(ws_c);
    if (!m || !ws || !dst) return fail(GVX_ERR_INVALID_ARG, "null argument");
    const WsPlan wp = make_ws_plan(m, B, L, T);
    if (ws_bytes < wp.total) return fail(GVX_ERR_WORKSPACE, "workspace too small");
    const gvx_dims& d = m->d;
    hipStream_t s = (hipStream_t)stream;
    const size_t rows = (size_t)(T + 1) * B;
    switch (what) {
        case 0: HIP_TRY(hipMemcpyAsync(dst, ws_ptr<float>(ws, wp.frames), rows * d.n_mels * sizeof(float), hipMemcpyDeviceToDevice, s)); break;
        case 1: HIP_TRY(hipMemcpyAsync(dst, ws_ptr<float>(ws, wp.pre1), rows * d.prenet_dim * sizeof(float), hipMemcpyDeviceToDevice, s)); break;
        case 2: return gvx_train_unblock(ws_ptr<float>(ws, wp.prenet), dst, T + 1, B, d.prenet_dim, stream);
        case 3: HIP_TRY(hipMemcpyAsync(dst, ws_ptr<float>(ws, wp.pm), (size_t)B * L * d.att_dim * sizeof(float), hipMemcpyDeviceToDevice, s)); break;
        default: return fail(GVX_ERR_INVALID_ARG, "gvx_train_export: unknown buffer %d", what);
    }
    return GVX_OK;
}

size_t gvx_postnet_workspace_bytes(const gvx_model* m, int B, int T) {
    if (!m || B < 1 || T < 1) return 0;
    return make_postnet_plan(m, B, T).total;
}

int gvx_postnet_forward(gvx_model* m, const float* mel_in, const int32_t* mel_lengths, int B, int T, float* mel_post_out, void* ws,
                        size_t ws_bytes, void* stream) {
    if (!m) return fail(GVX_ERR_INVALID_ARG, "null model");
    if (!m->dev_blob) return fail(GVX_ERR_STATE, "weights not bound (call gvx_model_bind_blob)");
    if (B < 1 || T < 1) return fail(GVX_ERR_INVALID_ARG, "B and T must be >= 1");
    if ((long)B * T > (1L << 30)) return fail(GVX_ERR_UNSUPPORTED, "B * T = %ld frames exceed the GEMM row index range", (long)B * T);
    if (!ws) return fail(GVX_ERR_WORKSPACE, "null workspace");
    if (reinterpret_cast<uintptr_t>(ws) & 255) return fail(GVX_ERR_WORKSPACE, "workspace must be 256-byte aligned");
    const PostnetPlan pp = make_postnet_plan(m, B, T);
    if (ws_bytes < pp.total) return fail(GVX_ERR_WORKSPACE, "workspace too small: %zu < %zu bytes", ws_bytes, pp.total);
    if (!mel_in || !mel_post_out) return fail(GVX_ERR_INVALID_ARG, "null argument");
    return postnet_impl(m, mel_in, mel_lengths, B, T, mel_post_out, ws_ptr<float>(ws, pp.ya), ws_ptr<float>(ws, pp.yb), (hipStream_t)stream);
}

int gvx_mask_padding(float* mel, float* mel_post, float* gate, const int32_t* mel_lengths, int B, int n_mels, int T, void* stream) {
    if (!mel_lengths || B < 1 || T < 1 || n_mels < 1) return fail(GVX_ERR_INVALID_ARG, "bad argument");
    HIP_TRY(launch_mask_padding(mel, mel_post, gate, mel_lengths, B, n_mels, T, (hipStream_t)stream));
    return GVX_OK;
}

int gvx_tacotron2_forward(gvx_model* m, const int64_t* tokens, const int32_t* token_lengths, int B, int L, const float* mel_in,
                          const int32_t* mel_lengths, int T, const uint8_t* keep_masks, float* mel_out, float* mel_post_out,
                          float* gate_out, float* align_out, void* ws, size_t ws_bytes, void* stream) {
    int rc = check_common(m, B, L, T, ws, ws_bytes);
    if (rc != GVX_OK) return rc;
    if (!tokens || !mel_in || !keep_masks || !mel_out || !gate_out || !align_out)
        return fail(GVX_ERR_INVALID_ARG, "null argument");
    hipStream_t s = (hipStream_t)stream;
    const WsPlan wp = make_ws_plan(m, B, L, T);
    const bool timed = m->timing && m->ev_valid;
    float* memory = ws_ptr<float>(ws, wp.memory);
    if (timed) HIP_TRY(hipEventRecord(m->ev[0], s));
    const bool overlap = plan_teacher_forced(m, B, L, TF_INFERENCE).side_stream;
    if (overlap) {
        rc = ensure_side_stream(m);
        if (rc != GVX_OK) return rc;
        HIP_TRY(hipEventRecord(m->pa_fork, s));
        HIP_TRY(hipStreamWaitEvent(m->pa_stream, m->pa_fork, 0));
        rc = encoder_impl(m, tokens, token_lengths, B, L, memory, ws, wp, m->pa_stream, nullptr, nullptr, nullptr, m->enc_mid);
        if (rc != GVX_OK) return rc;
        rc = decoder_init_states(m, memory, B, L, decoder_buffers(ws, wp), m->pa_stream);
        if (rc != GVX_OK) return rc;
        HIP_TRY(hipEventRecord(m->pa_join, m->pa_stream));
        HIP_TRY(hipStreamWaitEvent(s, m->enc_mid, 0));
        rc = decoder_prenet_part(m, B, L, mel_in, T, keep_masks, ws, wp, s);
        if (rc != GVX_OK) return rc;
        HIP_TRY(hipStreamWaitEvent(s, m->pa_join, 0));
    } else {
        rc = encoder_impl(m, tokens, token_lengths, B, L, memory, ws, wp, s);
        if (rc != GVX_OK) return rc;
    }
    if (timed) HIP_TRY(hipEventRecord(m->ev[1], s));
    rc = decoder_tf_impl(m, memory, token_lengths, B, L, mel_in, T, keep_masks, mel_out, gate_out, align_out, ws, wp, s, overlap);
    if (rc != GVX_OK) return rc;
    if (timed) HIP_TRY(hipEventRecord(m->ev[4], s));
    if (mel_post_out) {
        rc = postnet_impl(m, mel_out, nullptr, B, T, mel_post_out, ws_ptr<float>(ws, wp.ya), ws_ptr<float>(ws, wp.yb), s);
        if (rc != GVX_OK) return rc;
        if (mel_lengths) HIP_TRY(launch_mask_padding(mel_out, mel_post_out, gate_out, mel_lengths, B, m->d.n_mels, T, s));
    }
    float* outs[4] = {mel_out, gate_out, align_out, mel_post_out};
    const size_t nm = (size_t)B * m->d.n_mels * T;
    const size_t counts[4] = {nm, (size_t)B * T, (size_t)B * T * L, nm};
    rc = poison_if_timed_out(m, B, L, ws, wp, outs, counts, mel_post_out ? 4 : 3, s);
    if (rc != GVX_OK) return rc;
    if (timed) HIP_TRY(hipEventRecord(m->ev[5], s));
    return GVX_OK;
}

int gvx_tacotron2_loss(const float* mel_out, const float* mel_post_out, const float* gate_out, const float* mel_target,
                       const float* gate_target, int B, int n_mels, int T, float* loss_out, void* scratch, size_t scratch_bytes,
                       void* stream) {
    if (!mel_out || !mel_post_out || !gate_out || !mel_target || !gate_target || !loss_out || !scratch)
        return fail(GVX_ERR_INVALID_ARG, "null argument");
    if (B < 1 || n_mels < 1 || T < 1) return fail(GVX_ERR_INVALID_ARG, "B, n_mels and T must be >= 1");
    if (scratch_bytes < loss_scratch_bytes() || (reinterpret_cast<uintptr_t>(scratch) & 7))
        return fail(GVX_ERR_WORKSPACE, "scratch too small (%zu bytes needed) or not 8-byte aligned", loss_scratch_bytes());
    HIP_TRY(launch_tacotron2_loss(mel_out, mel_post_out, gate_out, mel_target, gate_target, (long)B * n_mels * T, (long)B * T,
                                  reinterpret_cast<double*>(scratch), loss_out, (hipStream_t)stream));
    return GVX_OK;
}

int gvx_prenet_masks_generate(uint8_t* masks_out, size_t n, uint64_t seed, void* stream) {
    if (!masks_out) return fail(GVX_ERR_INVALID_ARG, "null argument");
    HIP_TRY(launch_mask_gen(masks_out, n, seed, (hipStream_t)stream));
    return GVX_OK;
}

int gvx_stage_timing_enable(gvx_model* m, int enable) {
    if (!m) return fail(GVX_ERR_INVALID_ARG, "null model");
    if (enable && !m->ev_valid) {
        for (auto& e : m->ev) HIP_TRY(hipEventCreate(&e));
        m->ev_valid = true;
    }
    m->timing = enable != 0;
    return GVX_OK;
}

int gvx_kernel_timing_enable(gvx_model* m, int enable) {
    if (!m) return fail(GVX_ERR_INVALID_ARG, "null model");
    m->ktiming = enable != 0;
    return GVX_OK;
}

int gvx_kernel_times_ms(gvx_model* m, float* lstm_avg_ms, float* attn_avg_ms, int* n_steps) {
    if (!m || !lstm_avg_ms || !attn_avg_ms) return fail(GVX_ERR_INVALID_ARG, "null argument");
    if (m->n_lstm_ev < 1) return fail(GVX_ERR_STATE, "no timed decoder loop has run");
    HIP_TRY(hipEventSynchronize(m->kev[2]));
    float a = 0, b = 0;
    HIP_TRY(hipEventElapsedTime(&a, m->kev[0], m->kev[1]));
    HIP_TRY(hipEventElapsedTime(&b, m->kev[1], m->kev[2]));
    *lstm_avg_ms = a / m->n_lstm_ev;
    *attn_avg_ms = m->n_attn_ev > 0 ? b / m->n_attn_ev : 0.f;
    if (n_steps) *n_steps = m->n_lstm_ev;
    return GVX_OK;
}

int gvx_stage_times_ms(gvx_model* m, float* t5, int* launches) {
    if (!m || !t5) return fail(GVX_ERR_INVALID_ARG, "null argument");
    if (!m->ev_valid) return fail(GVX_ERR_STATE, "stage timing was not enabled");
    HIP_TRY(hipEventSynchronize(m->ev[5]));
    for (int i = 0; i < 5; ++i) HIP_TRY(hipEventElapsedTime(&t5[i], m->ev[i], m->ev[i + 1]));
    if (launches) *launches = m->last_decoder_launches;
    return GVX_OK;
}
#ifdef GVX_STAMPS
int gvx_debug_read_stamps_skinny(unsigned long long* host96) {
    HIP_TRY(hipDeviceSynchronize());
    HIP_TRY(gvx::read_stamps_skinny(host96));
    return GVX_OK;
}
int gvx_debug_read_stamps_persist(unsigned long long* host96) {
    HIP_TRY(hipDeviceSynchronize());
    HIP_TRY(gvx::read_stamps_persist(host96));
    return GVX_OK;
}
int gvx_debug_read_wg_spans(unsigned long long* host1024) {
    HIP_TRY(hipDeviceSynchronize());
    HIP_TRY(gvx::read_wg_spans(host1024));
    return GVX_OK;
}
int gvx_debug_read_stamps_resident(unsigned long long* host480) {
    HIP_TRY(hipDeviceSynchronize());
    HIP_TRY(gvx::read_stamps_resident(host480));
    return GVX_OK;
}
int gvx_debug_read_wg_stamps_resident(unsigned long long* host896, unsigned long long* rows512) {
    HIP_TRY(hipDeviceSynchronize());
    HIP_TRY(gvx::read_wg_stamps_resident(host896));
    HIP_TRY(gvx::read_row_stamps_persist(rows512));
    return GVX_OK;
}
int gvx_debug_read_loc_stamps(unsigned long long* host32) {
    HIP_TRY(hipDeviceSynchronize());
    HIP_TRY(gvx::read_loc_stamps_persist(host32));
    return GVX_OK;
}
int gvx_debug_read_stamps_ar(unsigned long long* host896, unsigned long long* rows256) {
    HIP_TRY(hipDeviceSynchronize());
    HIP_TRY(gvx::read_wg_stamps_resident_ar(host896));
    HIP_TRY(gvx::read_row_stamps_persist_ar(rows256));
    return GVX_OK;
}
int gvx_debug_read_stamps(unsigned long long* host96) {
    HIP_TRY(hipDeviceSynchronize());
    unsigned long long tmp[96];
    HIP_TRY(gvx::read_stamps_skinny(host96));
    HIP_TRY(gvx::read_stamps_attention(tmp));
    for (int i = 32; i < 96; ++i) host96[i] = tmp[i];
    return GVX_OK;
}
#endif

}
```

### genvox_amd/csrc/gvx_decoder.hip

```cpp
#include "gvx_internal.h"

using namespace gvx;

namespace gvx {

namespace {
bool resident_attention_serves(const gvx_model* m, int B, int L) {
    const gvx_dims& d = m->d;
    return attention_persistent_supported(B, L, d.att_dim, d.att_loc_filters, d.att_loc_kernel, d.embed_dim, d.att_rnn_dim, d.dec_rnn_dim);
}
}

TfLoopPlan plan_teacher_forced(const gvx_model* m, int B, int L, TfMode mode) {
    TfLoopPlan p{};
    const bool train = mode != TF_INFERENCE;
    const bool pa_shape = (B <= 32 || m->tf_rows64) && m->attn_persistent && m->attn_one_launch && resident_attention_serves(m, B, L);
    const bool pa = pa_shape && (!train || m->train_resident);
    p.pa_layout = attention_persistent_layout(B, L);
    const bool resident = pa && (p.pa_layout == 1 || p.pa_layout == 2) && m->tf_resident &&
                          (!train || (m->train_resident_loop && mode == TF_TRAIN_WHOLE_TAPE)) && decoder_resident_supported(B, L);
    p.kind = resident ? 2 : (pa ? 1 : 0);
    p.tile_layout = resident && p.pa_layout == 2 && B > 2 && B <= 16 && m->tf_long_rows_224 ? 1 : p.pa_layout;
    p.rows64 = p.kind == 1 && p.pa_layout == 3;
    p.pre_gate = p.timeout_check = pa_shape;
    p.side_stream = p.kind != 0;
    p.graph = m->use_graph && !m->ktiming && p.kind != 2 && (p.rows64 || !train);
    return p;
}

ArLoopPlan plan_autoregressive(const gvx_model* m, int B, int L, bool windowed) {
    ArLoopPlan p{};
    const gvx_dims& d = m->d;
    const int E = d.embed_dim, D = d.dec_rnn_dim, lay = attention_persistent_layout(B, L);
    const bool pa_any = m->attn_one_launch && resident_attention_serves(m, B, L);
    const bool pair = pa_any && B <= 32 && E / 4 == D / 8 && m->attn_persistent && m->tf_resident && m->ar_resident_loop &&
                      decoder_resident_supported(B, L) && (lay == 1 || (lay == 2 && B <= 16)) && d.prenet_dim == 256 && d.n_mels <= 80 &&
                      m->PSB() <= 96 && d.att_dim == 128;
    p.kind = pair ? 2 : (pa_any && lay == 1 && m->ar_resident ? 1 : 0);
    if (windowed && !(p.kind == 2 && lay == 1)) p.kind = 0;
    p.fold = B <= 32 && E / 4 == D / 8;
    p.split_h = p.kind == 0 && m->ar_split_h && m->attn_persistent && m->attn_one_launch && B <= 32 && d.att_dim > 32 && d.att_dim <= 128;
    p.graph = m->use_graph && p.kind != 2;
    return p;
}

DecoderBuffers decoder_buffers(void* ws, const WsPlan& wp) {
    DecoderBuffers b;
    b.pm = ws_ptr<float>(ws, wp.pm); b.frames = ws_ptr<float>(ws, wp.frames); b.pre1 = ws_ptr<float>(ws, wp.pre1);
    b.prenet = ws_ptr<float>(ws, wp.prenet); b.h_a = ws_ptr<float>(ws, wp.h_a); b.c_a = ws_ptr<float>(ws, wp.c_a);
    b.c_d = ws_ptr<float>(ws, wp.c_d); b.hc = ws_ptr<float>(ws, wp.hc); b.w_cum = ws_ptr<float>(ws, wp.w_cum);
    b.q_slab = ws_ptr<float>(ws, wp.q_slab); b.proj = ws_ptr<float>(ws, wp.proj); b.energies = ws_ptr<float>(ws, wp.energies);
    b.align_tm = ws_ptr<float>(ws, wp.align_tm); b.len_copy = ws_ptr<int32_t>(ws, wp.len_copy);
    b.loc = ws_ptr<float>(ws, wp.loc);
    b.p_slab = ws_ptr<float>(ws, wp.p_slab); b.p_ctx = ws_ptr<float>(ws, wp.p_ctx);
    b.att_part = ws_ptr<float>(ws, wp.att_part); b.dec_part = ws_ptr<float>(ws, wp.dec_part);
    b.pre_gate = ws_ptr<float>(ws, wp.pre_gate);
    return b;
}

int decoder_init_states(gvx_model* m, const float* memory, int B, int L, const DecoderBuffers& db, hipStream_t s) {
    const gvx_dims& d = m->d;
    const int E = d.embed_dim, A = d.att_rnn_dim, D = d.dec_rnn_dim;
    void* const zp[5] = {db.h_a, db.c_a, db.c_d, db.hc , db.w_cum};
    const size_t zb[5] = {(size_t)RS_HA_SLOTS * B * A * sizeof(float), (size_t)B * A * sizeof(float), (size_t)B * D * sizeof(float),
                          (size_t)B * (D + E) * sizeof(float), (size_t)B * L * sizeof(float)};
    HIP_TRY(launch_zero_many(zp, zb, 5, s));
    GemmParams g{};
    g.A = memory; g.amap = RowMap{B * L, 0, (long)E};
    g.W = m->dev_blob + m->blob.wmem; g.ldw = E;
    g.C = db.pm; g.cmap = RowMap{B * L, 0, (long)d.att_dim};
    g.M = B * L; g.N = d.att_dim; g.K = E; g.act = ACT_NONE;
    HIP_TRY(launch_gemm(g, s));
    return GVX_OK;
}

namespace {

void fill_att_job(const gvx_model* m, SkinnyJob& J, const float* prenet_t, int t, int B, const DecoderBuffers& db) {
    const gvx_dims& d = m->d;
    const int E = d.embed_dim, P = d.prenet_dim, A = d.att_rnn_dim, D = d.dec_rnn_dim;
    std::memset(&J, 0, sizeof J);
    const float* hc_t = db.hc + (size_t)t * B * (D + E);
    J.Wp = m->dev_blob + m->blob.att_frag; J.bias = m->dev_blob + m->blob.att_bias;
    J.x[0] = XSeg{prenet_t, P};
    J.x[1] = XSeg{hc_t + (size_t)D * B, E};
    J.x[2] = XSeg{db.h_a + (size_t)(t & 1) * B * A, A};
    J.N = 4 * A; J.nkg = (P + E + A) / 8; J.mode = 0; J.B = B;
    J.c = db.c_a;
    J.h_out = db.h_a + (size_t)((t + 1) & 1) * B * A;
    J.Wq_t = m->dev_blob + m->blob.wq_t; J.q_slab = db.q_slab; J.att_dim = d.att_dim;
}

void fill_dec_job(const gvx_model* m, SkinnyJob& J, int t, int B, const DecoderBuffers& db) {
    const gvx_dims& d = m->d;
    const int E = d.embed_dim, A = d.att_rnn_dim, D = d.dec_rnn_dim;
    std::memset(&J, 0, sizeof J);
    const float* hc_t = db.hc + (size_t)t * B * (D + E);
    float* hc_n = db.hc + (size_t)(t + 1) * B * (D + E);
    J.Wp = m->dev_blob + m->blob.dec_frag; J.bias = m->dev_blob + m->blob.dec_bias;
    J.x[0] = XSeg{db.h_a + (size_t)((t + 1) & 1) * B * A, A};
    J.x[1] = XSeg{hc_n + (size_t)D * B, E};
    J.x[2] = XSeg{hc_t, D};
    J.N = 4 * D; J.nkg = (A + E + D) / 8; J.mode = 0; J.B = B;
    J.c = db.c_d;
    J.h_out = hc_n;
}

void fill_loc(const gvx_model* m, LocJob& q, int t, int B, int L, const float* align_base, long align_bs, long align_ts,
              const DecoderBuffers& db) {
    const gvx_dims& d = m->d;
    q.w_prev = t > 0 ? align_base + (size_t)(t - 1) * align_ts : nullptr; q.w_prev_bs = align_bs;
    q.w_cum = db.w_cum;
    q.loc_conv_t = m->dev_blob + m->blob.loc_conv; q.loc_dense_t = m->dev_blob + m->blob.loc_dense;
    q.loc_out = db.loc;
    q.pm = m->attn_one_launch ? db.pm : nullptr;
    q.B = B; q.L = L; q.a = d.att_dim; q.kl = d.att_loc_kernel; q.G = attention_groups(B, L);
}

void fill_attn(const gvx_model* m, AttnParams& p, const float* memory, const int32_t* lengths, int t, int B, int L,
               float* align_out, long align_bs, long align_ts, const DecoderBuffers& db) {
    const gvx_dims& d = m->d;
    const int E = d.embed_dim, D = d.dec_rnn_dim;
    std::memset(&p, 0, sizeof p);
    p.q_slab = db.q_slab; p.n_slabs = d.att_rnn_dim / 8;
    p.w_cum = db.w_cum;
    p.loc = db.loc; p.v = m->dev_blob + m->blob.v;
    p.pm = db.pm; p.memory = memory; p.lengths = lengths;
    p.w_out = align_out + (size_t)t * align_ts; p.w_out_bs = align_bs;
    p.ctx_out = db.hc + (size_t)(t + 1) * B * (D + E) + (size_t)D * B;
    p.energies = db.energies;
    p.B = B; p.L = L; p.a = d.att_dim; p.F = d.att_loc_filters; p.kl = d.att_loc_kernel; p.E = E;
    p.G = m->attn_one_launch ? attention_slices(B, E) : attention_groups(B, L);
}

hipError_t launch_attn(const gvx_model* m, const AttnParams& p, hipStream_t s) {
    return m->attn_one_launch ? launch_attention_step(p, s) : launch_attention(p, s);
}

struct SidePool { hipStream_t s[2] = {nullptr, nullptr}; unsigned next = 0; };
std::mutex g_pool_mutex;
std::unordered_map<int, SidePool> g_side_pools;

struct ResidentTurn { hipEvent_t ev[4] = {nullptr, nullptr, nullptr, nullptr}; unsigned n = 0; };
std::mutex g_turn_mutex;
std::unordered_map<int, ResidentTurn> g_turns;

int turn_begin(hipStream_t s) {
    int dev = 0;
    HIP_TRY(hipGetDevice(&dev));
    ResidentTurn& t = g_turns[dev];
    if (!t.ev[0])
        for (auto& e : t.ev) HIP_TRY(hipEventCreateWithFlags(&e, hipEventDisableTiming));
    if (t.n > 0) HIP_TRY(hipStreamWaitEvent(s, t.ev[(t.n - 1) & 3], 0));
    return GVX_OK;
}
int turn_end(hipStream_t s) {
    int dev = 0;
    HIP_TRY(hipGetDevice(&dev));
    ResidentTurn& t = g_turns[dev];
    HIP_TRY(hipEventRecord(t.ev[t.n & 3], s));
    ++t.n;
    return GVX_OK;
}

}

int ensure_side_stream(gvx_model* m) {
    if (!m->pa_fork) {
        HIP_TRY(hipEventCreateWithFlags(&m->pa_fork, hipEventDisableTiming));
        HIP_TRY(hipEventCreateWithFlags(&m->pa_join, hipEventDisableTiming));
        HIP_TRY(hipEventCreateWithFlags(&m->enc_mid, hipEventDisableTiming));
    }
    int dev = 0;
    HIP_TRY(hipGetDevice(&dev));
    std::lock_guard<std::mutex> lock(g_pool_mutex);
    SidePool& pool = g_side_pools[dev];
    if (!pool.s[0]) {
        int least = 0, greatest = 0;
        HIP_TRY(hipDeviceGetStreamPriorityRange(&least, &greatest));
        for (auto& st : pool.s) HIP_TRY(hipStreamCreateWithPriority(&st, hipStreamNonBlocking, greatest));
    }
    m->pa_stream = pool.s[pool.next++ % m->side_pool];
    return GVX_OK;
}

namespace {

AttnPersistParams fill_attn_persist(const gvx_model* m, const DecoderBuffers& db, const float* memory, const int32_t* len_ws,
                                    unsigned* sync, int B, int L, int T) {
    const gvx_dims& d = m->d;
    const int E = d.embed_dim, D = d.dec_rnn_dim;
    AttnPersistParams pp{};
    pp.q_slab = db.q_slab;
    pp.v = m->dev_blob + m->blob.v; pp.pm = db.pm; pp.memory = memory; pp.lengths = len_ws;
    pp.loc_conv_t = m->dev_blob + m->blob.loc_conv; pp.loc_dense_t = m->dev_blob + m->blob.loc_dense;
    pp.w_out = db.align_tm; pp.w_out_bs = (long)L; pp.w_out_ts = (long)B * L;
    pp.ctx_base = db.hc + (size_t)B * (D + E) + (size_t)D * B; pp.ctx_ts = (long)B * (D + E);
    pp.sync = sync; pp.B = B; pp.L = L; pp.T = T; pp.kl = d.att_loc_kernel;
    pp.spin_limit = m->spin_limit;
    return pp;
}
void use_resident_flags(const gvx_model* m, AttnPersistParams& pp) {
    pp.q_flags = pp.sync + RS_FLAG_Q; pp.n_q_flags = pp.n_slabs;
    pp.ctx_flags = pp.sync + RS_FLAG_CTX;
    pp.debug = m->rs_debug;
}

int launch_resident_attention(gvx_model* m, const AttnPersistParams& pp, hipStream_t s) {
    HIP_TRY(hipEventRecord(m->pa_fork, s));
    HIP_TRY(hipStreamWaitEvent(m->pa_stream, m->pa_fork, 0));
    if (!m->debug_skip_resident) HIP_TRY(launch_attention_persistent(pp, m->pa_stream));
    HIP_TRY(hipEventRecord(m->pa_join, m->pa_stream));
    return GVX_OK;
}

template <class P>
void fill_resident_common(const gvx_model* m, const DecoderBuffers& db, unsigned* sync, int B, int T, P& rp) {
    const gvx_dims& d = m->d;
    rp.att_frag = m->dev_blob + m->blob.att_frag; rp.att_bias = m->dev_blob + m->blob.att_bias; rp.wq_t = m->dev_blob + m->blob.wq_t;
    rp.dec_frag = m->dev_blob + m->blob.dec_frag; rp.dec_bias = m->dev_blob + m->blob.dec_bias;
    rp.h_a = db.h_a; rp.hc = db.hc; rp.q_slab = db.q_slab; rp.c_a = db.c_a; rp.c_d = db.c_d;
    rp.sync = sync;
    rp.att_frag_bytes = (unsigned)(frag_floats(4 * d.att_rnn_dim, d.prenet_dim + d.embed_dim + d.att_rnn_dim) * sizeof(float));
    rp.B = B; rp.T = T; rp.spin_limit = m->spin_limit; rp.debug = m->rs_debug;
}

int ensure_ar_host_slots(gvx_model* m) {
    if (m->ar_done_host) return GVX_OK;
    HIP_TRY(hipHostMalloc(reinterpret_cast<void**>(&m->ar_done_host), 2 * sizeof(int32_t), hipHostMallocDefault));
    for (auto& e : m->ar_ev) HIP_TRY(hipEventCreateWithFlags(&e, hipEventDisableTiming));
    return GVX_OK;
}

}

int decoder_prenet_part(gvx_model* m, int B, int L, const float* mel_in, int T, const uint8_t* keep_masks, void* ws, const WsPlan& wp,
                        hipStream_t s) {
    const gvx_dims& d = m->d;
    const int M = d.n_mels, P = d.prenet_dim;
    const DecoderBuffers db = decoder_buffers(ws, wp);
    HIP_TRY(zero_async(db.frames, (size_t)B * M * sizeof(float), s));
    HIP_TRY(launch_frames_from_mel(mel_in, db.frames, B, M, T, s));
    const int rows = (T + 1) * B;
    GemmParams g{};
    g.A = db.frames; g.amap = RowMap{rows, 0, (long)M};
    g.W = m->dev_blob + m->blob.pre_w0; g.ldw = M;
    g.C = db.pre1; g.cmap = RowMap{rows, 0, (long)P};
    g.keep = keep_masks; g.keep_ld = P;
    g.M = rows; g.N = P; g.K = M; g.act = ACT_RELU;
    HIP_TRY(launch_gemm(g, s));
    g.A = db.pre1; g.amap = RowMap{rows, 0, (long)P};
    g.W = m->dev_blob + m->blob.pre_w1; g.ldw = P;
    g.C = db.prenet; g.cmap = RowMap{B, (long)B * P, 8}; g.c_nblk = (long)B * 8;
    g.keep = keep_masks + (size_t)rows * P;
    g.K = P;
    HIP_TRY(launch_gemm(g, s));
    if (plan_teacher_forced(m, B, L, TF_INFERENCE).pre_gate) {
        GemmParams h{};
        h.A = db.prenet; h.amap = RowMap{B, (long)B * P, 8}; h.a_kblk = (long)B * 8;
        h.W = m->dev_blob + m->blob.att_wpre; h.ldw = P;
        h.C = db.pre_gate; h.cmap = RowMap{T * B, 0, (long)4 * d.att_rnn_dim};
        h.M = T * B; h.N = 4 * d.att_rnn_dim; h.K = P; h.act = ACT_NONE;
        HIP_TRY(launch_gemm(h, s));
    }
    return GVX_OK;
}

int poison_if_timed_out(const gvx_model* m, int B, int L, void* ws, const WsPlan& wp, float* const* outs, const size_t* counts, int n,
                        hipStream_t s) {
    if (!plan_teacher_forced(m, B, L, TF_INFERENCE).timeout_check) return GVX_OK;
    HIP_TRY(launch_poison_on_timeout(ws_ptr<unsigned>(ws, wp.sync) + HANDOFF_TIMEOUT, ws_ptr<int>(ws, wp.flags) + FLAG_TIMEOUT, outs, counts, n, s));
    return GVX_OK;
}

namespace {

struct TfLoop {
    gvx_model* m; TfLoopPlan plan; DecoderBuffers db;
    const float* memory; const int32_t* len_ws; void* ws; unsigned* sync; float* xchg;
    int B, L, T;
    const LstmDropout* train;
};

void defer_context(const TfLoop& c, SkinnyJob& J, int t_ctx, bool first) {
    if (c.plan.kind == 0) return;
    const gvx_dims& d = c.m->d;
    J.defer_seg = 1;
    if (J.q_slab) {
        const int P = d.prenet_dim, E = d.embed_dim, A = d.att_rnn_dim;
        J.x[0] = XSeg{J.x[1].p, 0};
        J.kg0 = P / 8; J.nkg_w = (P + E + A) / 8; J.nkg = (E + A) / 8;
        J.addend = c.db.pre_gate + (size_t)(t_ctx + 1) * c.B * 4 * A; J.add_bs = 4 * A;
    }
    J.tmo = c.sync + HANDOFF_TIMEOUT;
    J.spin_limit = c.m->spin_limit;
    if (t_ctx >= 0) { J.ctx_cnt = c.sync + HANDOFF_CNT_CTX; J.ctx_target = (unsigned)c.B * (unsigned)(t_ctx + 1); }
    J.start_cnt = c.sync + HANDOFF_CNT_Q;
    if (first) { J.ready_cnt = c.sync + HANDOFF_READY; J.ready_target = (unsigned)attention_persistent_workgroups(c.B, c.L); }
}

void wire_tape(const LstmDropout& tr, SkinnyJob* att, SkinnyJob* dec, int t, size_t BA, size_t BD) {
    if (att) {
        att->h_keep = tr.att_keep + (size_t)t * BA; att->h_scale = tr.att_scale;
        if (tr.h_a_all) { att->x[2].p = tr.h_a_all + (size_t)t * BA; att->h_out = tr.h_a_all + (size_t)(t + 1) * BA; }
        if (tr.c_a_all) { att->c = tr.c_a_all + (size_t)t * BA; att->c_out = tr.c_a_all + (size_t)(t + 1) * BA; }
        if (tr.pre_a_all) att->pre_out = tr.pre_a_all + (size_t)t * 4 * BA;
    }
    if (dec) {
        if (tr.pre_d_all) dec->pre_out = tr.pre_d_all + (size_t)(t - 1) * 4 * BD;
        dec->h_keep = tr.dec_keep + (size_t)(t - 1) * BD; dec->h_scale = tr.dec_scale;
        if (tr.h_a_all) dec->x[0].p = tr.h_a_all + (size_t)t * BA;
        if (tr.c_d_all) { dec->c = tr.c_d_all + (size_t)(t - 1) * BD; dec->c_out = tr.c_d_all + (size_t)t * BD; }
    }
}

int tf_step_jobs(const TfLoop& c, int t, SkinnyJob* jobs) {
    const gvx_dims& d = c.m->d;
    SkinnyJob* att = t < c.T ? &jobs[0] : nullptr;
    SkinnyJob* dec = t > 0 ? &jobs[att ? 1 : 0] : nullptr;
    if (att) {
        fill_att_job(c.m, *att, c.db.prenet + (size_t)t * c.B * d.prenet_dim, t, c.B, c.db);
        defer_context(c, *att, t - 1, t == 0);
    }
    if (dec) {
        fill_dec_job(c.m, *dec, t - 1, c.B, c.db);
        defer_context(c, *dec, t - 1, false);
    }
    if (c.train) wire_tape(*c.train, att, dec, t, (size_t)c.B * d.att_rnn_dim, (size_t)c.B * d.dec_rnn_dim);
    return (att ? 1 : 0) + (dec ? 1 : 0);
}

int tf_step_jobs64(const TfLoop& c, int t, SkinnyJob* jobs) {
    const gvx_model* m = c.m;
    const gvx_dims& d = m->d;
    const int E = d.embed_dim, P = d.prenet_dim, A = d.att_rnn_dim, D = d.dec_rnn_dim, B = c.B, T = c.T;
    const DecoderBuffers& db = c.db;
    float* dec_part2[2] = {db.dec_part, db.dec_part + (size_t)B * 4 * D};
    int n = 0;
    if (t < T) {
        fill_att_job(m, jobs[n], db.prenet + (size_t)t * B * P, t, B, db);
        defer_context(c, jobs[n], t - 1, t == 0);
        ++n;
    }
    if (t >= 1 && t - 1 < T) {
        SkinnyJob& J = jobs[n];
        fill_dec_job(m, J, t - 1, B, db);
        J.x[2] = XSeg{nullptr, 0};
        J.nkg = (A + E) / 8; J.kg0 = 0; J.nkg_w = (A + E + D) / 8;
        J.mode = 2; J.bias = nullptr; J.c = nullptr; J.h_out = nullptr;
        J.y = dec_part2[t & 1];
        defer_context(c, J, t - 1, false);
        ++n;
    }
    if (t >= 2 && t - 2 < T) {
        SkinnyJob& J = jobs[n];
        std::memset(&J, 0, sizeof J);
        const float* hc_t = db.hc + (size_t)(t - 2) * B * (D + E);
        float* hc_n = db.hc + (size_t)(t - 1) * B * (D + E);
        J.Wp = m->dev_blob + m->blob.dec_frag; J.bias = m->dev_blob + m->blob.dec_bias;
        J.x[0] = XSeg{hc_t, D};
        J.N = 4 * D; J.nkg = D / 8; J.kg0 = (A + E) / 8; J.nkg_w = (A + E + D) / 8; J.mode = 0; J.B = B;
        J.c = db.c_d; J.h_out = hc_n;
        J.addend = dec_part2[(t - 1) & 1]; J.add_bs = 4 * D;
        J.start_cnt = c.sync + HANDOFF_CNT_Q;
        ++n;
    }
    return n;
}

template <class F>
int enqueue_or_replay(const TfLoop& c, int variant, hipStream_t s, F&& enqueue) {
    if (!c.plan.graph) return enqueue(s);
    const gvx_model::LoopKey key{c.ws, c.memory, c.m->dev_blob, c.B, c.L, c.T, c.len_ws != nullptr, 0.f, variant};
    return run_chunk(c.m, touch_graph_set(c.m, c.m->loop_graphs, key), 0, s, enqueue);
}

int tf_loop_resident(const TfLoop& c, hipStream_t s, int* launches) {
    gvx_model* m = c.m;
    const gvx_dims& d = m->d;
    DecResidentParams rp{};
    fill_resident_common(m, c.db, c.sync, c.B, c.T, rp);
    rp.pre_gate = c.db.pre_gate;
    rp.kg_pre = d.prenet_dim / 8;
    if (const LstmDropout* train = c.train) {
        rp.h_a = train->h_a_all;
        rp.tr_keep_a = train->att_keep; rp.tr_keep_d = train->dec_keep; rp.tr_scale_a = train->att_scale; rp.tr_scale_d = train->dec_scale;
        rp.tr_c_a = train->c_a_all; rp.tr_c_d = train->c_d_all; rp.tr_pre_a = train->pre_a_all; rp.tr_pre_d = train->pre_d_all;
    }
    rp.dec_frag_bytes = (unsigned)(frag_floats(4 * d.dec_rnn_dim, d.att_rnn_dim + d.embed_dim + d.dec_rnn_dim) * sizeof(float));
    rp.layout = c.plan.tile_layout;
    if (m->ktiming) HIP_TRY(hipEventRecord(m->kev[0], s));
    HIP_TRY(launch_decoder_resident(rp, s));
    if (m->ktiming) {
        HIP_TRY(hipEventRecord(m->kev[1], s));
        HIP_TRY(hipEventRecord(m->kev[2], s));
        m->n_lstm_ev = c.T; m->n_attn_ev = 0;
    }
    *launches = 1;
    return GVX_OK;
}

int tf_loop_beside_attention(const TfLoop& c, hipStream_t s, int* launches) {
    *launches = c.plan.rows64 ? c.T + 2 : c.T + 1;
    if (c.plan.rows64)
        return enqueue_or_replay(c, 48, s, [&](hipStream_t st) -> int {
            SkinnyJob jobs[3];
            for (int t = 0; t < c.T + 2; ++t) HIP_TRY(launch_skinny_pa64(jobs, tf_step_jobs64(c, t, jobs), st));
            return GVX_OK;
        });
    return enqueue_or_replay(c, c.m->pa_depth + 16 * c.plan.pa_layout, s, [&](hipStream_t st) -> int {
        SkinnyJob jobs[2];
        for (int t = 0; t < c.T; ++t) {
            tf_step_jobs(c, t, jobs);
            HIP_TRY(launch_skinny_pa(jobs[0], t > 0 ? &jobs[1] : nullptr, st, c.m->pa_depth, c.plan.pa_layout));
        }
        tf_step_jobs(c, c.T, jobs);
        HIP_TRY(launch_skinny(jobs, 1, SK_DECODER, st));
        return GVX_OK;
    });
}

int tf_loop_per_step(const TfLoop& c, hipStream_t s, int* launches) {
    const gvx_model* m = c.m;
    const gvx_dims& d = m->d;
    const int B = c.B, L = c.L, T = c.T;
    *launches = (m->attn_one_launch ? 2 : 3) * T + 1;
    return enqueue_or_replay(c, 0, s, [&](hipStream_t st) -> int {
        SkinnyJob jobs[2];
        for (int t = 0; t < T; ++t) {
            const int n = tf_step_jobs(c, t, jobs);
            LocJob lq;
            fill_loc(m, lq, t, B, L, c.db.align_tm, (long)L, (long)B * L, c.db);
            HIP_TRY(launch_skinny(jobs, n, SK_DECODER, st, &lq));
            AttnParams ap;
            fill_attn(m, ap, c.memory, c.len_ws, t, B, L, c.db.align_tm, (long)L, (long)B * L, c.db);
            if (m->attn_prefetch && m->attn_one_launch && B <= 32) {
                ap.pf_w[0] = m->dev_blob + m->blob.att_frag; ap.pf_w[1] = m->dev_blob + m->blob.dec_frag;
                ap.pf_nkg[0] = (d.prenet_dim + d.embed_dim + d.att_rnn_dim) / 8; ap.pf_nkg[1] = (d.att_rnn_dim + d.embed_dim + d.dec_rnn_dim) / 8;
                ap.pf_tiles0 = 4 * d.att_rnn_dim / 32; ap.pf_tiles = ap.pf_tiles0 + 4 * d.dec_rnn_dim / 32;
            }
            HIP_TRY(launch_attn(m, ap, st));
        }
        tf_step_jobs(c, T, jobs);
        HIP_TRY(launch_skinny(jobs, 1, SK_DECODER, st));
        return GVX_OK;
    });
}

int tf_time_step_launches(const TfLoop& c, hipStream_t s) {
    gvx_model* m = c.m;
    const int B = c.B, L = c.L, REPS = 64, tm = c.T > 1 ? c.T / 2 : 0;
    SkinnyJob jobs[3];
    fill_att_job(m, jobs[0], c.db.prenet + (size_t)tm * B * m->d.prenet_dim, tm, B, c.db);
    if (tm > 0) fill_dec_job(m, jobs[1], tm - 1, B, c.db);
    m->n_lstm_ev = REPS;
    m->n_attn_ev = 0;
    if (c.plan.kind == 0) {
        LocJob lq;
        fill_loc(m, lq, tm, B, L, c.db.align_tm, (long)L, (long)B * L, c.db);
        AttnParams ap;
        fill_attn(m, ap, c.memory, c.len_ws, tm, B, L, c.db.align_tm, (long)L, (long)B * L, c.db);
        ap.w_out = c.db.energies;
        ap.w_cum = c.db.energies;
        HIP_TRY(hipEventRecord(m->kev[0], s));
        for (int i = 0; i < REPS; ++i) HIP_TRY(launch_skinny(jobs, tm > 0 ? 2 : 1, SK_DECODER, s, &lq));
        HIP_TRY(hipEventRecord(m->kev[1], s));
        for (int i = 0; i < REPS; ++i) HIP_TRY(launch_attn(m, ap, s));
        HIP_TRY(hipEventRecord(m->kev[2], s));
        m->n_attn_ev = REPS;
        return GVX_OK;
    }
    HIP_TRY(hipStreamWaitEvent(s, m->pa_join, 0));
    int n = 0;
    if (c.plan.rows64) {
        n = tf_step_jobs64(c, tm > 2 ? tm : 2, jobs);
    } else {
        defer_context(c, jobs[0], tm - 1, false);
        if (tm > 0) defer_context(c, jobs[1], tm - 1, false);
        n = tm > 0 ? 2 : 1;
    }
    for (int i = 0; i < n; ++i) jobs[i].start_cnt = nullptr;
    HIP_TRY(hipEventRecord(m->kev[0], s));
    for (int i = 0; i < REPS; ++i)
        HIP_TRY(c.plan.rows64 ? launch_skinny_pa64(jobs, n, s) : launch_skinny_pa(jobs[0], tm > 0 ? &jobs[1] : nullptr, s, m->pa_depth, c.plan.pa_layout));
    HIP_TRY(hipEventRecord(m->kev[1], s));
    HIP_TRY(hipEventRecord(m->kev[2], s));
    return GVX_OK;
}

}

int decoder_tf_impl(gvx_model* m, const float* memory, const int32_t* lengths, int B, int L, const float* mel_in, int T,
                    const uint8_t* keep_masks, float* mel_out, float* gate_out, float* align_out, void* ws, const WsPlan& wp,
                    hipStream_t s, bool prenet_done, const LstmDropout* train) {
    const gvx_dims& d = m->d;
    const int E = d.embed_dim, M = d.n_mels, D = d.dec_rnn_dim;
    const DecoderBuffers db = decoder_buffers(ws, wp);
    unsigned* sync = ws_ptr<unsigned>(ws, wp.sync);
    HIP_TRY(zero_async(sync, HANDOFF_WORDS * sizeof(unsigned), s));
    const bool timed = m->timing && m->ev_valid;
    int rc = GVX_OK;
    if (!prenet_done) {
        rc = decoder_prenet_part(m, B, L, mel_in, T, keep_masks, ws, wp, s);
        if (rc != GVX_OK) return rc;
        rc = decoder_init_states(m, memory, B, L, db, s);
        if (rc != GVX_OK) return rc;
    }
    if (timed) HIP_TRY(hipEventRecord(m->ev[2], s));
    const int32_t* len_ws = nullptr;
    if (lengths) {
        HIP_TRY(hipMemcpyAsync(db.len_copy, lengths, (size_t)B * sizeof(int32_t), hipMemcpyDeviceToDevice, s));
        len_ws = db.len_copy;
    }
    if (m->ktiming) {
        rc = m->reserve_events(4);
        if (rc != GVX_OK) return rc;
        m->n_lstm_ev = m->n_attn_ev = 0;
    }
    const bool tape_whole = train && train->h_a_all && train->c_a_all && train->c_d_all && train->pre_a_all && train->pre_d_all;
    const TfLoopPlan plan = plan_teacher_forced(m, B, L, !train ? TF_INFERENCE : (tape_whole ? TF_TRAIN_WHOLE_TAPE : TF_TRAIN_PARTIAL_TAPE));
    const TfLoop c{m, plan, db, memory, len_ws, ws, sync, ws_ptr<float>(ws, wp.xchg), B, L, T, train};
    std::unique_lock<std::mutex> turn;
    if (plan.side_stream) {
        if (!prenet_done) {
            rc = ensure_side_stream(m);
            if (rc != GVX_OK) return rc;
        }
        turn = std::unique_lock<std::mutex>(g_turn_mutex);
        rc = turn_begin(s);
        if (rc != GVX_OK) return rc;
        AttnPersistParams pp = fill_attn_persist(m, db, memory, len_ws, sync, B, L, T);
        pp.n_slabs = attention_persistent_slabs(plan.tile_layout);
        pp.xchg = c.xchg;
        pp.q_first = 2;
        if (plan.kind == 2) use_resident_flags(m, pp);
        rc = launch_resident_attention(m, pp, s);
        if (rc != GVX_OK) return rc;
    }
    int launches = 0;
    switch (plan.kind) {
        case 2: rc = tf_loop_resident(c, s, &launches); break;
        case 1: rc = tf_loop_beside_attention(c, s, &launches); break;
        default: rc = tf_loop_per_step(c, s, &launches); break;
    }
    if (rc != GVX_OK) return rc;
    if (plan.side_stream) {
        HIP_TRY(hipStreamWaitEvent(s, m->pa_join, 0));
        ++launches;
        rc = turn_end(s);
        if (rc != GVX_OK) return rc;
        turn.unlock();
    }
    if (m->ktiming && plan.kind != 2) {
        rc = tf_time_step_launches(c, s);
        if (rc != GVX_OK) return rc;
    }
    HIP_TRY(launch_permute01(db.align_tm, align_out, T, B, L, s));
    m->last_decoder_launches = launches;
    if (timed) HIP_TRY(hipEventRecord(m->ev[3], s));
    {
        const int PS = m->PS();
        GemmParams g{};
        g.A = db.hc + (size_t)B * (D + E); g.amap = RowMap{B, (long)B * (D + E), 8}; g.a_kblk = (long)B * 8;
        g.W = m->dev_blob + m->blob.proj_w; g.ldw = D + E;
        g.C = db.proj; g.cmap = RowMap{B, (long)PS, (long)T * PS};
        g.bias = m->dev_blob + m->blob.proj_b;
        g.M = T * B; g.N = M + 1; g.K = D + E; g.act = ACT_NONE;
        HIP_TRY(launch_gemm(g, s));
        HIP_TRY(launch_split_projection(db.proj, mel_out, gate_out, B, M, T, s));
    }
    return GVX_OK;
}

namespace {

struct ArLoop {
    gvx_model* m; ArLoopPlan plan; DecoderBuffers db;
    const float* memory_ws; const int32_t* len_ws; const uint8_t* masks_ws; void* ws; unsigned* sync; float* xchg;
    int32_t* n_done; int32_t* n_frames_ws;
    int B, L, T;
    float gate_threshold;
    int32_t* centres; int win_back, win_ahead;
};

void print_ws_plan_once(const WsPlan& wp) {
    static bool printed = false;
    if (printed) return;
    printed = true;
#define GVX_PL(f) std::fprintf(stderr, "wsplan %s %zu\n", #f, wp.f);
    GVX_PL(xa) GVX_PL(xb) GVX_PL(xg) GVX_PL(enc_h) GVX_PL(enc_c) GVX_PL(flags) GVX_PL(sync) GVX_PL(memory) GVX_PL(pm) GVX_PL(frames) GVX_PL(pre1) GVX_PL(prenet) GVX_PL(h_a) GVX_PL(c_a) GVX_PL(c_d)
    GVX_PL(hc) GVX_PL(w_cum) GVX_PL(q_slab) GVX_PL(proj) GVX_PL(energies) GVX_PL(align_tm) GVX_PL(len_copy) GVX_PL(loc) GVX_PL(ar_masks)
    GVX_PL(p_slab) GVX_PL(p_ctx) GVX_PL(att_part) GVX_PL(dec_part) GVX_PL(pre_gate) GVX_PL(xchg) GVX_PL(ya) GVX_PL(yb) GVX_PL(total)
#undef GVX_PL
}

struct ArStep {
    const float* hc_t; float* hc_n; float* ctx_n; float* ha_new; float* att_part2; float* dec_part2;
    int kgP, kgE, kgA, kgD;
};
ArStep ar_step(const ArLoop& c, int t) {
    const gvx_dims& d = c.m->d;
    const int E = d.embed_dim, A = d.att_rnn_dim, D = d.dec_rnn_dim, B = c.B;
    ArStep q;
    q.hc_t = c.db.hc + (size_t)t * B * (D + E);
    q.hc_n = c.db.hc + (size_t)(t + 1) * B * (D + E);
    q.ctx_n = q.hc_n + (size_t)D * B;
    q.ha_new = c.db.h_a + (size_t)((t + 1) & 1) * B * A;
    q.att_part2 = c.db.att_part + (size_t)B * 4 * A;
    q.dec_part2 = c.db.dec_part + (size_t)B * 4 * D;
    q.kgP = d.prenet_dim / 8; q.kgE = E / 8; q.kgA = A / 8; q.kgD = D / 8;
    return q;
}

int ar_launch_a(const ArLoop& c, const ArStep& q, int t, hipStream_t st) {
    const gvx_model* m = c.m;
    const gvx_dims& d = m->d;
    const DecoderBuffers& db = c.db;
    const int P = d.prenet_dim, A = d.att_rnn_dim, D = d.dec_rnn_dim, B = c.B, L = c.L;
    const int kgP = q.kgP, kgE = q.kgE, kgA = q.kgA, kgD = q.kgD;
    SkinnyJob ja[2];
    std::memset(ja, 0, sizeof ja);
    {
        SkinnyJob& J = ja[0];
        J.Wp = m->dev_blob + m->blob.att_frag; J.bias = m->dev_blob + m->blob.att_bias;
        J.x[0] = XSeg{db.prenet, P};
        J.N = 4 * A; J.nkg = kgP; J.kg0 = 0; J.nkg_w = kgP + kgE + kgA; J.mode = 0; J.B = B;
        J.addend = db.att_part; J.add_bs = 4 * A; J.add_ts = 0;
        J.c = db.c_a; J.h_out = q.ha_new;
        J.Wq_t = m->dev_blob + m->blob.wq_t; J.q_slab = db.q_slab; J.att_dim = d.att_dim;
    }
    {
        SkinnyJob& J = ja[1];
        J.Wp = m->dev_blob + m->blob.dec_frag;
        J.x[0] = XSeg{q.hc_t, D};
        J.N = 4 * D; J.nkg = kgD; J.kg0 = kgA + kgE; J.nkg_w = kgA + kgE + kgD; J.mode = 2; J.B = B;
        J.y = db.dec_part;
    }
    if (c.plan.kind != 0) {
        if (t == 0) {
            ja[0].ready_cnt = c.sync + HANDOFF_READY; ja[0].ready_target = (unsigned)B;
            ja[0].tmo = c.sync + HANDOFF_TIMEOUT; ja[0].spin_limit = m->spin_limit;
        }
        HIP_TRY(launch_skinny(ja, 2, SK_AR, st));
        return GVX_OK;
    }
    LocJob lq;
    fill_loc(m, lq, t, B, L, db.align_tm, (long)L, (long)B * L, db);
    HIP_TRY(launch_skinny(ja, 2, SK_AR, st, &lq));
    AttnParams ap;
    fill_attn(m, ap, c.memory_ws, c.len_ws, t, B, L, db.align_tm, (long)L, (long)B * L, db);
    if (c.centres) {
        ap.c_prev = t > 0 ? c.centres + (t - 1) : nullptr; ap.c_out = c.centres + t; ap.c_bs = (long)c.T;
        ap.win_back = c.win_back; ap.win_ahead = c.win_ahead;
    }
    if (!c.plan.split_h) {
        HIP_TRY(launch_attn(m, ap, st));
        return GVX_OK;
    }
    SkinnyJob jb[2];
    std::memset(jb, 0, sizeof jb);
    {
        SkinnyJob& J = jb[0];
        J.Wp = m->dev_blob + m->blob.dec_frag;
        J.x[0] = XSeg{q.ha_new, A};
        J.N = 4 * D; J.nkg = kgA; J.kg0 = 0; J.nkg_w = kgA + kgE + kgD; J.mode = 2; J.B = B;
        J.y = q.dec_part2;
    }
    {
        SkinnyJob& J = jb[1];
        J.Wp = m->dev_blob + m->blob.att_frag;
        J.x[0] = XSeg{q.ha_new, A};
        J.N = 4 * A; J.nkg = kgA; J.kg0 = kgP + kgE; J.nkg_w = kgP + kgE + kgA; J.mode = 2; J.B = B;
        J.y = q.att_part2;
    }
    HIP_TRY(launch_skinny_attn(jb, 2, ap, st));
    return GVX_OK;
}

int ar_launch_cd(const ArLoop& c, const ArStep& q, int t, hipStream_t st) {
    const gvx_model* m = c.m;
    const gvx_dims& d = m->d;
    const DecoderBuffers& db = c.db;
    const int E = d.embed_dim, M = d.n_mels, P = d.prenet_dim, A = d.att_rnn_dim, D = d.dec_rnn_dim, B = c.B, T = c.T, PSB = m->PSB();
    const int kgP = q.kgP, kgE = q.kgE, kgA = q.kgA, kgD = q.kgD;
    const bool fold = c.plan.fold;
    SkinnyJob jc[3];
    std::memset(jc, 0, sizeof jc);
    {
        SkinnyJob& J = jc[0];
        J.Wp = m->dev_blob + m->blob.dec_frag; J.bias = m->dev_blob + m->blob.dec_bias;
        J.x[0] = XSeg{q.ha_new, A};
        J.x[1] = XSeg{q.ctx_n, E};
        J.N = 4 * D; J.nkg = kgA + kgE; J.kg0 = 0; J.nkg_w = kgA + kgE + kgD; J.mode = 0; J.B = B;
        J.addend = db.dec_part; J.add_bs = 4 * D; J.add_ts = 0;
        J.c = db.c_d; J.h_out = q.hc_n;
        J.Wq_t = m->dev_blob + m->blob.proj_hd_t; J.q_slab = db.p_slab; J.att_dim = PSB;
        if (fold) { J.xw = m->dev_blob + m->blob.proj_ctx_t; J.xsrc = q.ctx_n; }
    }
    {
        SkinnyJob& J = jc[1];
        J.Wp = m->dev_blob + m->blob.att_frag;
        J.x[0] = XSeg{q.ctx_n, 0};
        J.x[1] = XSeg{q.ctx_n, E};
        J.x[2] = XSeg{q.ha_new, A};
        J.N = 4 * A; J.nkg = kgE + kgA; J.kg0 = kgP; J.nkg_w = kgP + kgE + kgA; J.mode = 2; J.B = B;
        J.y = db.att_part;
    }
    if (c.plan.split_h) {
        SkinnyJob& Jd = jc[0];
        Jd.x[0] = XSeg{q.ctx_n, E}; Jd.x[1] = XSeg{nullptr, 0};
        Jd.nkg = kgE; Jd.kg0 = kgA;
        Jd.addend2 = q.dec_part2;
        SkinnyJob& Ja = jc[1];
        Ja.x[0] = XSeg{q.ctx_n, E}; Ja.x[1] = XSeg{nullptr, 0}; Ja.x[2] = XSeg{nullptr, 0};
        Ja.nkg = kgE; Ja.kg0 = kgP;
        Ja.addend = q.att_part2; Ja.add_bs = 4 * A;
    }
    if (c.plan.kind != 0)
        for (int i = 0; i < 2; ++i) {
            SkinnyJob& J = jc[i];
            J.defer_seg = 1;
            J.ctx_cnt = c.sync + HANDOFF_CNT_CTX; J.ctx_target = (unsigned)B * (unsigned)(t + 1);
            J.tmo = c.sync + HANDOFF_TIMEOUT; J.spin_limit = m->spin_limit;
            if (i == 0) J.start_cnt = c.sync + HANDOFF_CNT_Q;
        }
    if (!fold) {
        SkinnyJob& J = jc[2];
        J.Wp = m->dev_blob + m->blob.proj_ctx_frag; J.bias = m->dev_blob + m->blob.proj_b;
        J.x[0] = XSeg{q.ctx_n, E};
        J.N = M + 1; J.nkg = kgE; J.mode = 1; J.B = B; J.act = ACT_NONE;
        J.y = db.p_ctx;
    }
    HIP_TRY(launch_skinny(jc, fold ? 2 : 3, SK_AR, st));
    const bool more = t + 1 < T;
    HIP_TRY(launch_ar_project(db.p_slab, D / 8, db.p_ctx, db.proj + (size_t)t * B * PSB, M, c.gate_threshold, t, B, c.n_frames_ws, c.n_done,
                              m->dev_blob + m->blob.pre_w0_t, m->dev_blob + m->blob.pre_w1_t, P,
                              more ? c.masks_ws + (size_t)(t + 1) * B * P : nullptr,
                              more ? c.masks_ws + ((size_t)T + t + 1) * B * P : nullptr, db.prenet, st));
    return GVX_OK;
}

int ar_enqueue_steps(const ArLoop& c, hipStream_t st, int t0, int t1) {
    for (int t = t0; t < t1; ++t) {
        const ArStep q = ar_step(c, t);
        int rc = ar_launch_a(c, q, t, st);
        if (rc == GVX_OK) rc = ar_launch_cd(c, q, t, st);
        if (rc != GVX_OK) return rc;
    }
    return GVX_OK;
}

int ar_loop_resident(const ArLoop& c, hipStream_t s, int* steps) {
    gvx_model* m = c.m;
    const gvx_dims& d = m->d;
    const DecoderBuffers& db = c.db;
    const int B = c.B, T = c.T, P = d.prenet_dim, PSB = m->PSB();
    std::unique_lock<std::mutex> turn(g_turn_mutex);
    int rc = turn_begin(s);
    if (rc != GVX_OK) return rc;
    AttnPersistParams pp = fill_attn_persist(m, db, c.memory_ws, c.len_ws, c.sync, B, c.L, T);
    pp.n_slabs = attention_persistent_slabs(1);
    pp.xchg = c.xchg;
    pp.q_first = 1;
    use_resident_flags(m, pp);
    pp.p_slab = db.p_slab; pp.PSB = PSB; pp.n_mels = d.n_mels; pp.proj_b = m->dev_blob + m->blob.proj_b; pp.proj_out = db.proj;
    pp.pre_w0_t = m->dev_blob + m->blob.pre_w0_t; pp.keep0 = c.masks_ws; pp.y1 = db.pre1;
    pp.n_frames = c.n_frames_ws; pp.n_done = c.n_done; pp.gate_threshold = c.gate_threshold;
    pp.p_flags = c.sync + RS_FLAG_P; pp.y1_flags = c.sync + RS_FLAG_Y1;
    pp.centres = c.centres; pp.win_back = c.win_back; pp.win_ahead = c.win_ahead;
    rc = launch_resident_attention(m, pp, s);
    if (rc != GVX_OK) return rc;
    ArResidentParams rp{};
    fill_resident_common(m, db, c.sync, B, T, rp);
    rp.proj_hd_t = m->dev_blob + m->blob.proj_hd_t; rp.proj_ctx_t = m->dev_blob + m->blob.proj_ctx_t;
    rp.pre_w1 = m->dev_blob + m->blob.pre_w1; rp.keep1 = c.masks_ws + (size_t)T * B * P;
    rp.prenet = db.prenet; rp.y1 = db.pre1;
    rp.p_slab = db.p_slab;
    rp.n_done = c.n_done;
    rp.PSB = PSB;
    HIP_TRY(launch_decoder_ar_resident(rp, s));
    HIP_TRY(hipStreamWaitEvent(s, m->pa_join, 0));
    rc = turn_end(s);
    if (rc != GVX_OK) return rc;
    turn.unlock();
    rc = ensure_ar_host_slots(m);
    if (rc != GVX_OK) return rc;
    HIP_TRY(hipMemcpyAsync(m->ar_done_host, c.sync + HANDOFF_STOP, sizeof(int32_t), hipMemcpyDeviceToHost, s));
    HIP_TRY(hipStreamSynchronize(s));
    *steps = m->ar_done_host[0] > 0 && m->ar_done_host[0] < T ? m->ar_done_host[0] : T;
    return GVX_OK;
}

int ar_loop_chunked(const ArLoop& c, hipStream_t s, int* steps) {
    gvx_model* m = c.m;
    const gvx_dims& d = m->d;
    const DecoderBuffers& db = c.db;
    const int B = c.B, L = c.L, T = c.T;
    if (c.plan.fold) {
        SkinnyJob J;
        std::memset(&J, 0, sizeof J);
        J.Wp = m->dev_blob + m->blob.proj_ctx_frag; J.bias = m->dev_blob + m->blob.proj_b;
        J.x[0] = XSeg{db.hc + (size_t)d.dec_rnn_dim * B, d.embed_dim};
        J.N = d.n_mels + 1; J.nkg = d.embed_dim / 8; J.mode = 1; J.B = B; J.act = ACT_NONE;
        J.y = db.p_ctx;
        HIP_TRY(launch_skinny(&J, 1, SK_AR, s));
    }
    if (c.plan.kind == 1) {
        AttnPersistParams pp = fill_attn_persist(m, db, c.memory_ws, c.len_ws, c.sync, B, L, T);
        pp.n_slabs = d.att_rnn_dim / 8;
        pp.q_first = 1;
        const int rc = launch_resident_attention(m, pp, s);
        if (rc != GVX_OK) return rc;
    }
    const int CHUNK = 16;
    gvx_model::GraphSet* gset = nullptr;
    if (c.plan.graph) {
        gvx_model::LoopKey key{c.ws, c.memory_ws, m->dev_blob, B, L, T, c.len_ws != nullptr};
        key.threshold = c.gate_threshold;
        key.variant = c.plan.kind == 1 ? 1 : (c.plan.split_h ? 2 : 0);
        key.centres = c.centres; key.win_back = c.win_back; key.win_ahead = c.win_ahead;
        gset = touch_graph_set(m, m->ar_graphs, key);
    }
    int rc = ensure_ar_host_slots(m);
    if (rc != GVX_OK) return rc;
    auto enqueue_chunk = [&](int t0, int slot) -> int {
        const int t1 = t0 + CHUNK < T ? t0 + CHUNK : T;
        const int r = run_chunk(m, gset, (size_t)(t0 / CHUNK), s, [&](hipStream_t st) { return ar_enqueue_steps(c, st, t0, t1); });
        if (r != GVX_OK) return r;
        HIP_TRY(hipMemcpyAsync(m->ar_done_host + slot, c.n_done, sizeof(int32_t), hipMemcpyDeviceToHost, s));
        HIP_TRY(hipEventRecord(m->ar_ev[slot], s));
        return GVX_OK;
    };
    rc = enqueue_chunk(0, 0);
    if (rc != GVX_OK) return rc;
    int t_enq = CHUNK < T ? CHUNK : T, slot = 0;
    for (;;) {
        const int t_chunk_end = t_enq;
        const bool more = t_enq < T;
        if (more) {
            rc = enqueue_chunk(t_enq, slot ^ 1);
            if (rc != GVX_OK) return rc;
            t_enq = t_enq + CHUNK < T ? t_enq + CHUNK : T;
        }
        HIP_TRY(hipEventSynchronize(m->ar_ev[slot]));
        *steps = t_chunk_end;
        if (m->ar_done_host[slot] >= B || !more) break;
        slot ^= 1;
    }
    if (c.plan.kind == 1) {
        HIP_TRY(launch_handoff_set(c.sync + HANDOFF_STOP, s));
        HIP_TRY(hipStreamWaitEvent(s, m->pa_join, 0));
    }
    return GVX_OK;
}

int decoder_ar_impl(gvx_model* m, const float* memory, const int32_t* lengths, int B, int L, int max_steps, float gate_threshold,
                    const uint8_t* keep_masks, float* mel_out, float* gate_out, float* align_out, int32_t* n_frames_out, int* steps_run_out,
                    void* ws, size_t ws_bytes, void* stream, int window_back, int window_ahead, int32_t* centres_out) {
    int rc = check_common(m, B, L, max_steps, ws, ws_bytes, WS_AUTOREGRESSIVE);
    if (rc != GVX_OK) return rc;
    if (!memory || !keep_masks || !mel_out || !gate_out || !align_out || !n_frames_out)
        return fail(GVX_ERR_INVALID_ARG, "null argument");
    hipStream_t s = (hipStream_t)stream;
    const gvx_dims& d = m->d;
    const int E = d.embed_dim, M = d.n_mels, P = d.prenet_dim, A = d.att_rnn_dim, T = max_steps;
    const WsPlan wp = make_ws_plan(m, B, L, T, WS_AUTOREGRESSIVE);
    const DecoderBuffers db = decoder_buffers(ws, wp);
    if (m->debug_plan) print_ws_plan_once(wp);
    unsigned* sync = ws_ptr<unsigned>(ws, wp.sync);
    HIP_TRY(zero_async(sync, HANDOFF_WORDS * sizeof(unsigned), s));
    int32_t* flags = ws_ptr<int32_t>(ws, wp.flags);
    float* memory_ws = ws_ptr<float>(ws, wp.memory);
    if (memory != memory_ws)
        HIP_TRY(hipMemcpyAsync(memory_ws, memory, (size_t)B * L * E * sizeof(float), hipMemcpyDeviceToDevice, s));
    uint8_t* masks_ws = ws_ptr<uint8_t>(ws, wp.ar_masks);
    HIP_TRY(hipMemcpyAsync(masks_ws, keep_masks, (size_t)2 * T * B * P, hipMemcpyDeviceToDevice, s));
    const int32_t* len_ws = nullptr;
    if (lengths) {
        HIP_TRY(hipMemcpyAsync(db.len_copy, lengths, (size_t)B * sizeof(int32_t), hipMemcpyDeviceToDevice, s));
        len_ws = db.len_copy;
    }
    rc = decoder_init_states(m, memory_ws, B, L, db, s);
    if (rc != GVX_OK) return rc;
    const ArLoop c{m, plan_autoregressive(m, B, L, centres_out != nullptr), db, memory_ws, len_ws, masks_ws, ws, sync, ws_ptr<float>(ws, wp.xchg),
                   flags + FLAG_AR_DONE, flags + FLAG_AR_FRAMES, B, L, T, gate_threshold, centres_out, window_back, window_ahead};
    if (c.plan.kind != 0) {
        rc = ensure_side_stream(m);
        if (rc != GVX_OK) return rc;
    }
    HIP_TRY(zero_async(db.prenet, (size_t)B * P * sizeof(float), s));
    HIP_TRY(zero_async(db.att_part, (size_t)B * 4 * A * sizeof(float), s));
    HIP_TRY(zero_async(c.n_done, sizeof(int32_t), s));
    HIP_TRY(zero_async(c.n_frames_ws, (size_t)64 * sizeof(int32_t), s));
    int t = 0;
    rc = c.plan.kind == 2 ? ar_loop_resident(c, s, &t) : ar_loop_chunked(c, s, &t);
    if (rc != GVX_OK) return rc;
    HIP_TRY(launch_ar_stop(db.proj, M, -1.f, t - 1, B, c.n_frames_ws, c.n_done, s));
    HIP_TRY(hipMemcpyAsync(n_frames_out, c.n_frames_ws, (size_t)B * sizeof(int32_t), hipMemcpyDeviceToDevice, s));
    HIP_TRY(launch_ar_emit_all(db.proj, mel_out, gate_out, B, M, T, t, c.n_frames_ws, s));
    HIP_TRY(launch_permute01_partial(db.align_tm, align_out, t, T, B, L, c.n_frames_ws, s));
    if (centres_out) HIP_TRY(launch_ar_centres_finish(centres_out, c.n_frames_ws, c.plan.kind != 0 ? sync + HANDOFF_TIMEOUT : nullptr, B, T, s));
    if (c.plan.kind != 0) {
        float* outs[3] = {mel_out, gate_out, align_out};
        const size_t counts[3] = {(size_t)B * M * T, (size_t)B * T, (size_t)B * T * L};
        HIP_TRY(launch_poison_on_timeout(sync + HANDOFF_TIMEOUT, flags + FLAG_TIMEOUT, outs, counts, 3, s));
    }
    HIP_TRY(hipStreamSynchronize(s));
    if (steps_run_out) *steps_run_out = t;
    return GVX_OK;
}

}
}

extern "C" int gvx_decoder_autoregressive(gvx_model* m, const float* memory, const int32_t* lengths, int B, int L, int max_steps,
                                          float gate_threshold, const uint8_t* keep_masks, float* mel_out, float* gate_out, float* align_out,
                                          int32_t* n_frames_out, int* steps_run_out, void* ws, size_t ws_bytes, void* stream) {
    return decoder_ar_impl(m, memory, lengths, B, L, max_steps, gate_threshold, keep_masks, mel_out, gate_out, align_out, n_frames_out,
                           steps_run_out, ws, ws_bytes, stream, 0, 0, nullptr);
}

extern "C" int gvx_decoder_autoregressive_windowed(gvx_model* m, const float* memory, const int32_t* lengths, int B, int L, int max_steps,
                                                   float gate_threshold, const uint8_t* keep_masks, float* mel_out, float* gate_out,
                                                   float* align_out, int32_t* n_frames_out, int* steps_run_out, void* ws, size_t ws_bytes,
                                                   void* stream, int window_back, int window_ahead, int32_t* centres_out) {
    if (window_back < 0 || window_ahead < 0)
        return fail(GVX_ERR_INVALID_ARG, "window_back and window_ahead must be >= 0 (got %d, %d)", window_back, window_ahead);
    if (!centres_out) return fail(GVX_ERR_INVALID_ARG, "null argument: centres_out is the window's state and is mandatory");
    if (L > 0) {
        window_back = window_back < L ? window_back : L;
        window_ahead = window_ahead < L ? window_ahead : L;
    }
    return decoder_ar_impl(m, memory, lengths, B, L, max_steps, gate_threshold, keep_masks, mel_out, gate_out, align_out, n_frames_out,
                           steps_run_out, ws, ws_bytes, stream, window_back, window_ahead, centres_out);
}
```

### genvox_amd/csrc/gvx_internal.h

```cpp
#pragma once
#include "../../include/genvox_amd.h"
#include "gvx_kernels.h"

#include <cmath>
#include <cstdarg>
#include <cstdio>
#include <cstdlib>
#include <cstring>
#include <mutex>
#include <string>
#include <unordered_map>
#include <vector>

namespace gvx {

int fail(int code, const char* fmt, ...);

#define HIP_TRY(expr)                                                                          \
    do {                                                                                       \
        hipError_t _e = (expr);                                                                \
        if (_e != hipSuccess) return fail(GVX_ERR_HIP, "%s failed: %s", #expr, hipGetErrorString(_e)); \
    } while (0)

constexpr int MAX_CONV = 8;
constexpr double BN_EPS = 1e-5;

struct Blob {
    size_t emb;
    size_t enc_w[MAX_CONV], enc_b[MAX_CONV];
    size_t enc_wih, enc_bih, enc_whh_frag[2];
    size_t pre_w0, pre_w1, pre_w0_t, pre_w1_t;
    size_t att_frag, att_bias, att_wpre, wq_t, wmem, v, loc_conv, loc_dense;
    size_t dec_frag, dec_bias;
    size_t proj_w, proj_b, proj_frag, proj_hd_t, proj_ctx_frag, proj_ctx_t;
    size_t post_w[MAX_CONV], post_b[MAX_CONV];
    size_t total;
};
Blob make_blob_layout(const gvx_dims& d);

inline size_t frag_floats(int N, int K) { return (size_t)((N + 31) / 32) * (K / 8) * 64 * 4; }

struct WsPlan {
    size_t xa, xb, xg, enc_h, enc_c, flags, sync, memory;
    size_t pm, frames, pre1, prenet, h_a, c_a, c_d, hc, w_cum, q_slab, proj, energies, align_tm, len_copy, loc, ar_masks, p_slab, p_ctx;
    size_t att_part, dec_part, pre_gate, xchg;
    size_t ya, yb;
    size_t total;
};

}

struct gvx_model {
    gvx_dims d;
    gvx::Blob blob;
    const float* dev_blob = nullptr;
    bool use_graph = true;
    bool capture_first = false;
    bool attn_one_launch = true;
    bool attn_persistent = true;
    bool ar_resident = false;
    bool enc_persistent = true;
    bool ar_split_h = true;
    bool tf_rows64 = false;
    bool tf_resident = true;
    bool ar_resident_loop = true;
    bool tf_long_rows_224 = true;
    bool train_resident = true;
    bool train_resident_loop = true;
    bool attn_prefetch = true;
    int enc_fork_after = 1;
    int pa_depth = 4;
    unsigned side_pool = 1;
    unsigned spin_limit = 0;
    int rs_debug = 0;
    bool debug_skip_resident = false;
    int debug_enc_skip_block = -1;
    bool debug_plan = false;
    bool timing = false;
    hipEvent_t ev[6] = {nullptr, nullptr, nullptr, nullptr, nullptr, nullptr};
    bool ev_valid = false;
    int last_decoder_launches = 0;
    struct LoopKey {
        const void* ws; const void* memory; const void* blob; int B, L, T; bool has_len;
        float threshold = 0.f;
        int variant = 0;
        const void* centres = nullptr; int win_back = 0, win_ahead = 0;
        bool operator==(const LoopKey& o) const {
            return ws == o.ws && memory == o.memory && blob == o.blob && B == o.B && L == o.L && T == o.T &&
                   has_len == o.has_len && threshold == o.threshold && variant == o.variant && centres == o.centres &&
                   win_back == o.win_back && win_ahead == o.win_ahead;
        }
    };
    struct GraphSet {
        LoopKey key;
        int sightings = 0;
        uint64_t last_use = 0;
        std::vector<hipGraphExec_t> execs;
    };
    static constexpr size_t GRAPH_SETS = 4;
    std::vector<GraphSet> ar_graphs, loop_graphs, enc_graphs;
    uint64_t use_clock = 0;
    uint64_t graph_replays = 0;
    hipStream_t pa_stream = nullptr;
    hipEvent_t pa_fork = nullptr, pa_join = nullptr, enc_mid = nullptr;
    int32_t* ar_done_host = nullptr;
    hipEvent_t ar_ev[2] = {nullptr, nullptr};
    std::vector<std::string> gather_names;
    std::vector<int64_t> gather_numel;
    int32_t* gather_off = nullptr;
    uint8_t* gather_tid = nullptr;
    void drop_graphs() {
        for (auto* c : {&ar_graphs, &loop_graphs, &enc_graphs}) {
            for (auto& gs : *c)
                for (auto e : gs.execs)
                    if (e) (void)hipGraphExecDestroy(e);
            c->clear();
        }
    }
    hipStream_t cap_stream = nullptr;
    bool ktiming = false;
    std::vector<hipEvent_t> kev;
    int n_lstm_ev = 0, n_attn_ev = 0;
    int reserve_events(size_t n) {
        while (kev.size() < n) {
            hipEvent_t e;
            if (hipEventCreate(&e) != hipSuccess) return GVX_ERR_HIP;
            kev.push_back(e);
        }
        return GVX_OK;
    }
    int H() const { return d.embed_dim / 2; }
    int PS() const { return (d.n_mels + 1 + 3) & ~3; }
    int PSB() const { return (d.n_mels + 1 + 7) & ~7; }
};

namespace gvx {

enum TfMode : int { TF_INFERENCE = 0, TF_TRAIN_WHOLE_TAPE = 1, TF_TRAIN_PARTIAL_TAPE = 2 };
struct TfLoopPlan {
    int kind;
    int pa_layout;
    int tile_layout;
    bool rows64;
    bool pre_gate;
    bool timeout_check;
    bool side_stream;
    bool graph;
};
struct ArLoopPlan {
    int kind;
    bool split_h;
    bool fold;
    bool graph;
};
TfLoopPlan plan_teacher_forced(const gvx_model* m, int B, int L, TfMode mode);
ArLoopPlan plan_autoregressive(const gvx_model* m, int B, int L, bool windowed = false);

enum WsMode : int { WS_TEACHER_FORCED = 0, WS_AUTOREGRESSIVE = 1 };

constexpr int FLAG_TOKEN = 0;
constexpr int FLAG_AR_DONE = 1;
constexpr int FLAG_TIMEOUT = 2;
constexpr int FLAG_AR_FRAMES = 64;

WsPlan make_ws_plan(const gvx_model* m, int B, int L, int T, int mode = WS_TEACHER_FORCED);
int check_common(const gvx_model* m, int B, int L, int T, void* ws, size_t ws_bytes, int mode = WS_TEACHER_FORCED);

template <typename T>
T* ws_ptr(void* ws, size_t off) { return reinterpret_cast<T*>(reinterpret_cast<char*>(ws) + off); }

inline hipError_t zero_async(void* p, size_t bytes, hipStream_t s) { return hipMemsetAsync(p, 0, bytes, s); }

gvx_model::GraphSet* touch_graph_set(gvx_model* m, std::vector<gvx_model::GraphSet>& cache, const gvx_model::LoopKey& key);
std::mutex& capture_mutex();

template <class F>
int run_chunk(gvx_model* m, gvx_model::GraphSet* gs, size_t chunk, hipStream_t s, F&& enqueue) {
    if (!m->use_graph || !gs || (gs->sightings < 2 && !m->capture_first)) return enqueue(s);
    if (gs->execs.size() <= chunk) gs->execs.resize(chunk + 1, nullptr);
    hipGraphExec_t exec = gs->execs[chunk];
    if (!exec) {
        std::lock_guard<std::mutex> lock(capture_mutex());
        hipGraph_t graph = nullptr;
        if (!m->cap_stream) HIP_TRY(hipStreamCreateWithFlags(&m->cap_stream, hipStreamNonBlocking));
        HIP_TRY(hipStreamBeginCapture(m->cap_stream, hipStreamCaptureModeThreadLocal));
        const int rc = enqueue(m->cap_stream);
        const hipError_t ce = hipStreamEndCapture(m->cap_stream, &graph);
        if (rc != GVX_OK) { if (graph) (void)hipGraphDestroy(graph); return rc; }
        HIP_TRY(ce);
        HIP_TRY(hipGraphInstantiate(&exec, graph, nullptr, nullptr, 0));
        HIP_TRY(hipGraphDestroy(graph));
        gs->execs[chunk] = exec;
    }
    HIP_TRY(hipGraphLaunch(exec, s));
    ++m->graph_replays;
    return GVX_OK;
}

struct DecoderBuffers {
    float *pm, *frames, *pre1, *prenet, *h_a, *c_a, *c_d, *hc, *w_cum, *q_slab, *proj, *energies, *align_tm, *loc, *p_slab, *p_ctx;
    float *att_part, *dec_part, *pre_gate;
    int32_t* len_copy;
};
DecoderBuffers decoder_buffers(void* ws, const WsPlan& wp);

struct LstmDropout {
    const uint8_t* att_keep; const uint8_t* dec_keep; float att_scale, dec_scale;
    float* h_a_all; float* c_a_all; float* c_d_all;
    float* pre_a_all; float* pre_d_all;
};

int ensure_side_stream(gvx_model* m);
int decoder_init_states(gvx_model* m, const float* memory, int B, int L, const DecoderBuffers& db, hipStream_t s);
int decoder_prenet_part(gvx_model* m, int B, int L, const float* mel_in, int T, const uint8_t* keep_masks, void* ws, const WsPlan& wp,
                        hipStream_t s);
int decoder_tf_impl(gvx_model* m, const float* memory, const int32_t* lengths, int B, int L, const float* mel_in, int T,
                    const uint8_t* keep_masks, float* mel_out, float* gate_out, float* align_out, void* ws, const WsPlan& wp,
                    hipStream_t s, bool prenet_done = false, const LstmDropout* train = nullptr);
int poison_if_timed_out(const gvx_model* m, int B, int L, void* ws, const WsPlan& wp, float* const* outs, const size_t* counts, int n,
                        hipStream_t s);

}
```

### genvox_amd/csrc/gvx_kernels.h

```cpp
#pragma once
#include <hip/hip_runtime.h>
#include <stddef.h>
#include <stdint.h>

#ifdef GVX_STAMPS
namespace gvx { namespace { __device__ unsigned long long gvx_stamps[3][32]; } }
#define GVX_STAMP(k, i)                                                                         \
    do {                                                                                        \
        if (blockIdx.x == 0 && blockIdx.y == 0 && threadIdx.x == 0) gvx::gvx_stamps[k][i] = wall_clock64(); \
    } while (0)
#else
#define GVX_STAMP(k, i) do { } while (0)
#endif

namespace gvx {

int set_error(int code, const char* msg);

inline size_t align_up(size_t x, size_t a) { return (x + a - 1) / a * a; }

enum Act : int { ACT_NONE = 0, ACT_RELU = 1, ACT_TANH = 2 };

struct RowMap {
    int R;
    long s1, s0;
};

struct GemmParams {
    const float* A; RowMap amap; long a_kblk = 8;
    const float* W; long ldw;
    float* C; RowMap cmap; long c_nblk = 8;
    const float* bias;
    const uint8_t* keep; long keep_ld;
    int M, N, K;
    int act;
    int splitk = 1; int kchunk = 0; long c_split = 0;
    bool kmajor = false; RowMap wmap{1, 0, 0};
    int m_begin = 0;
    const int32_t* row_len = nullptr;
    int c_halo = 0;
};
hipError_t launch_gemm(const GemmParams& p, hipStream_t s);
struct GemmPlan { hipError_t err; int tile; int rows_big; };
GemmPlan plan_gemm(const GemmParams& p);
void set_splitk(GemmParams& p, int splitk);
hipError_t launch_gemm_splitk(const GemmParams& p, int splitk, float* scratch, hipStream_t s);

struct XSeg { const float* p; int len; };

struct SkinnyJob {
    const float* Wp;
    const float* bias;
    XSeg x[3];
    int N;
    int nkg;
    int kg0, nkg_w;
    int mode;
    float* c;
    float* h_out;
    const float* addend; long add_bs, add_ts;
    const float* addend2;
    const int32_t* lengths; int step; int reverse; int seq_len;
    float* seq_out; long seq_bs, seq_ts;
    const float* h_prev;
    const uint8_t* h_keep; float h_scale;
    float* c_out; float* c_seq_out;
    float* pre_out;
    const float* Wq_t;
    float* q_slab; int att_dim;
    const float* xw; const float* xsrc;
    int defer_seg;
    const unsigned* ctx_cnt; unsigned ctx_target;
    unsigned* start_cnt;
    const unsigned* ready_cnt; unsigned ready_target;
    unsigned* tmo;
    unsigned spin_limit;
    float* y;
    const uint8_t* keep; long keep_stride;
    int act;
    int B;
};
struct LocJob {
    const float* w_prev; long w_prev_bs;
    const float* w_cum;
    const float* loc_conv_t;
    const float* loc_dense_t;
    const float* pm;
    float* loc_out;
    int B, L, a, kl, G;
};
enum SkinnyKind : int { SK_DECODER = 0, SK_ENCODER = 1, SK_AR = 2, SK_TRAIN = 3 };
hipError_t launch_skinny(const SkinnyJob* jobs, int njobs, int kind, hipStream_t s, const LocJob* loc = nullptr);
struct AttnParams;
hipError_t launch_skinny_attn(const SkinnyJob* jobs, int njobs, const AttnParams& ap, hipStream_t s);
struct EncPersistParams {
    const float* Wp[2];
    const float* xg;
    const int32_t* lengths;
    float* hx;
    float* seq_out;
    float* c_seq_out;
    unsigned* sync;
    unsigned spin_limit;
    int B, L, H;
    int debug_skip_block;
};
bool encoder_persistent_supported(int B, int H);
hipError_t launch_encoder_persistent(const EncPersistParams& p, hipStream_t s);
hipError_t launch_skinny_pa(const SkinnyJob& att, const SkinnyJob* dec, hipStream_t s, int depth = 4, int layout = 1);
hipError_t launch_skinny_pa64(const SkinnyJob* jobs, int njobs, hipStream_t s);

struct AttnParams {
    const float* q_slab; int n_slabs;
    float* w_cum;
    const float* loc;
    const float* v;
    const float* pm;
    const float* memory;
    const int32_t* lengths;
    float* energies;
    float* w_out; long w_out_bs;
    float* ctx_out;
    int B, L, a, F, kl, E, G;
    const float* pf_w[2]; int pf_nkg[2]; int pf_tiles0, pf_tiles;
    const int32_t* c_prev; int32_t* c_out; long c_bs; int win_back, win_ahead;
};
hipError_t launch_attention(const AttnParams& p, hipStream_t s);
hipError_t launch_attention_step(const AttnParams& p, hipStream_t s);
int attention_slices(int B, int E);
int attention_groups(int B, int L);
bool attention_supported(int L, int a, int F, int kl, int E);

constexpr int HANDOFF_CNT_Q = 0, HANDOFF_CNT_CTX = 1024, HANDOFF_READY = 2048, HANDOFF_TIMEOUT = 3072;
constexpr int HANDOFF_STOP = 3072 + 512;
constexpr int HANDOFF_PAIR = 4096;
constexpr int HANDOFF_WORDS = 69632;
constexpr unsigned HANDOFF_SPIN_LIMIT = 200000u;
struct AttnPersistParams {
    const float* q_slab; int n_slabs;
    const float* v; const float* pm; const float* memory; const int32_t* lengths;
    const float* loc_conv_t; const float* loc_dense_t;
    float* w_out; long w_out_bs, w_out_ts;
    float* ctx_base; long ctx_ts;
    unsigned* sync;
    int B, L, T, kl;
    unsigned spin_limit;
    float* xchg;
    unsigned q_first;
    const unsigned* q_flags; int n_q_flags;
    unsigned* ctx_flags;
    int debug;
    const float* p_slab; int PSB, n_mels;
    const float* proj_b;
    float* proj_out;
    const float* pre_w0_t;
    const uint8_t* keep0;
    float* y1;
    int32_t* n_frames; int32_t* n_done; float gate_threshold;
    const unsigned* p_flags;
    unsigned* y1_flags;
    int32_t* centres; int win_back, win_ahead;
};
constexpr int RS_REP = 32;
constexpr int RS_FLAG_ATT = 8192;
constexpr int RS_FLAG_DEC = RS_FLAG_ATT + RS_REP * 128;
constexpr int RS_REP1 = 8;
constexpr int RS_FLAG_CTX = RS_FLAG_DEC + RS_REP * 128;
constexpr int RS_FLAG_Q = RS_FLAG_CTX + RS_REP1 * 32 * 32;
constexpr int RS_FLAG_Y1 = RS_FLAG_Q + RS_REP1 * 96 * 32;
constexpr int RS_REP_PRE = 8;
constexpr int RS_FLAG_PRE = RS_FLAG_Y1 + 32 * 32;
constexpr int RS_REP_P = 4;
constexpr int RS_FLAG_P = RS_FLAG_PRE + RS_REP_PRE * 8 * 32;
static_assert(RS_FLAG_P + RS_REP_P * 128 * 32 <= HANDOFF_WORDS, "flag replicas inside the hand-off block");
constexpr int RS_HA_SLOTS = 8;
struct DecResidentParams {
    const float* att_frag; const float* att_bias; const float* wq_t;
    const float* dec_frag; const float* dec_bias;
    const float* pre_gate;
    float* h_a;
    float* hc;
    float* q_slab;
    float* c_a; float* c_d;
    unsigned* sync;
    unsigned att_frag_bytes, dec_frag_bytes;
    int B, T;
    unsigned spin_limit;
    int debug;
    int kg_pre;
    int layout;
    const uint8_t* tr_keep_a; const uint8_t* tr_keep_d; float tr_scale_a, tr_scale_d;
    float* tr_c_a; float* tr_c_d; float* tr_pre_a; float* tr_pre_d;
};
struct ArResidentParams {
    const float* att_frag; const float* att_bias; const float* wq_t;
    const float* dec_frag; const float* dec_bias;
    const float* proj_hd_t;
    const float* proj_ctx_t;
    const float* pre_w1;
    const uint8_t* keep1;
    float* prenet;
    const float* y1;
    float* h_a; float* hc; float* q_slab;
    float* p_slab;
    float* c_a; float* c_d;
    const int32_t* n_done;
    unsigned* sync;
    unsigned att_frag_bytes;
    int B, T, PSB;
    unsigned spin_limit;
    int debug;
};
bool decoder_resident_supported(int B, int L);
hipError_t launch_decoder_ar_resident(const ArResidentParams& p, hipStream_t s);
hipError_t decoder_resident_init();
hipError_t launch_decoder_resident(const DecResidentParams& p, hipStream_t s);

bool attention_persistent_supported(int B, int L, int a, int F, int kl, int E, int att_rnn_dim, int dec_rnn_dim);
int attention_persistent_layout(int B, int L);
int attention_persistent_slabs(int layout);
int attention_persistent_workgroups(int B, int L);
size_t attention_persistent_xchg_floats(int B);
hipError_t attention_persistent_init();
hipError_t launch_attention_persistent(const AttnPersistParams& p, hipStream_t s);
hipError_t launch_handoff_set(unsigned* word, hipStream_t s);

#if defined(__HIPCC__)
typedef __attribute__((ext_vector_type(4))) unsigned gvx_u32x4;
__device__ __forceinline__ __amdgpu_buffer_rsrc_t make_rsrc(const void* p) {
    return __builtin_amdgcn_make_buffer_rsrc(const_cast<void*>(p), 0, 0x7fffffff, 0x00020000);
}
__device__ __forceinline__ float4 load_sc1(__amdgpu_buffer_rsrc_t r, unsigned byte_off) {
    const gvx_u32x4 v = __builtin_amdgcn_raw_buffer_load_b128(r, (int)byte_off, 0, 16);
    return make_float4(__uint_as_float(v.x), __uint_as_float(v.y), __uint_as_float(v.z), __uint_as_float(v.w));
}
__device__ __forceinline__ float load_sc1_f32(__amdgpu_buffer_rsrc_t r, unsigned byte_off) {
    return __uint_as_float(__builtin_amdgcn_raw_buffer_load_b32(r, (int)byte_off, 0, 16));
}
__device__ __forceinline__ void store_sc1(__amdgpu_buffer_rsrc_t r, unsigned byte_off, float4 v) {
    gvx_u32x4 u;
    u.x = __float_as_uint(v.x); u.y = __float_as_uint(v.y); u.z = __float_as_uint(v.z); u.w = __float_as_uint(v.w);
    __builtin_amdgcn_raw_buffer_store_b128(u, r, (int)byte_off, 0, 16);
}
template <bool FEW_WAITERS = false>
__device__ __forceinline__ bool handoff_wait(const unsigned* cnt, unsigned target, unsigned* tmo, unsigned code, unsigned limit = 0u,
                                             const unsigned* stop = nullptr) {
    if (limit == 0u) limit = HANDOFF_SPIN_LIMIT;
    unsigned spins = 0;
    while (__hip_atomic_load(cnt, __ATOMIC_RELAXED, __HIP_MEMORY_SCOPE_AGENT) < target) {
        ++spins;
        if ((spins & (FEW_WAITERS ? 127u : 7u)) == 1u) {
            if (__hip_atomic_load(tmo, __ATOMIC_RELAXED, __HIP_MEMORY_SCOPE_AGENT) != 0u) return false;
            if (stop && __hip_atomic_load(stop, __ATOMIC_RELAXED, __HIP_MEMORY_SCOPE_AGENT) != 0u) return false;
            if (spins > (FEW_WAITERS ? 16u : 1u) * limit) {
                __hip_atomic_store(tmo, code, __ATOMIC_RELAXED, __HIP_MEMORY_SCOPE_AGENT);
                return false;
            }
        }
        if (FEW_WAITERS || spins < 8u) __builtin_amdgcn_s_sleep(FEW_WAITERS ? 2 : 8);
        else __builtin_amdgcn_s_sleep(64);
    }
    return true;
}
#endif

hipError_t launch_embed(const int64_t* tokens, const float* emb, int n_tokens, float* x, float* x2, int B, int L, int E, int halo,
                        int* err_flag, hipStream_t s);
hipError_t launch_frames_from_mel(const float* mel_in, float* frames, int B, int M, int T, hipStream_t s);
hipError_t launch_split_projection(const float* proj, float* mel_out, float* gate_out, int B, int M, int T, hipStream_t s);
hipError_t launch_to_channels_last(const float* src, float* dst, int B, int M, int T, int halo, const int32_t* lens, hipStream_t s);
hipError_t launch_residual_to_channels_first(const float* mel, const float* y, float* mel_post, int B, int M, int T,
                                             const int32_t* lens, hipStream_t s);
hipError_t launch_zero_halo(float* buf, int B, int T, int halo, int C, hipStream_t s);
hipError_t launch_mask_padding(float* mel, float* mel_post, float* gate, const int32_t* mel_lengths, int B, int M, int T,
                               hipStream_t s);
hipError_t launch_zero_many(void* const* ptrs, const size_t* bytes, int n_arrays, hipStream_t s);
hipError_t launch_poison_on_timeout(const unsigned* tmo, int* sticky, float* const* ptrs, const size_t* counts, int n_arrays, hipStream_t s);
hipError_t launch_permute01(const float* src, float* dst, int T, int B, int n, hipStream_t s);
size_t loss_scratch_bytes();
hipError_t launch_tacotron2_loss(const float* mel, const float* mel_post, const float* gate, const float* mel_t, const float* gate_t,
                                 long n_mel, long n_gate, double* scratch, float* out3, hipStream_t s);
hipError_t launch_mask_gen(uint8_t* out, size_t n, uint64_t seed, hipStream_t s);
hipError_t launch_ar_stop(const float* proj_t, int gate_col, float threshold, int t, int B,
                          int32_t* n_frames, int32_t* n_done, hipStream_t s);
hipError_t launch_ar_project(const float* p_slab, int n_slabs, const float* p_ctx, float* proj_t, int M, float threshold, int t, int B,
                             int32_t* n_frames, int32_t* n_done, const float* w0t, const float* w1t, int P, const uint8_t* keep0,
                             const uint8_t* keep1, float* prenet_out, hipStream_t s);
hipError_t launch_ar_centres_finish(int32_t* centres, const int32_t* n_frames, const unsigned* tmo, int B, int T, hipStream_t s);
hipError_t launch_ar_emit_all(const float* proj, float* mel_out, float* gate_out, int B, int M, int Tmax, int steps,
                              const int32_t* n_frames, hipStream_t s);
hipError_t launch_permute01_partial(const float* src, float* dst, int steps, int Tdst, int B, int n, const int32_t* n_frames,
                                    hipStream_t s);

}
```

Before: 1.862 million.

## Cede attention k-group half-fragments from att workgroups to kind-1 workgroups

Adds a cede variant of the 224-workgroup resident teacher-forced decoder. Kind-1 workgroups stage part of the kind-0 (attention LSTM) h-side weight fragments in LDS, compute those partial MFMA products, and publish them through a slab and flag. The kind-0 upper waves skip that work and instead wait for and load the handed-over partials. This rebalances per-step work across workgroup kinds, at the cost of extra cross-workgroup synchronisation, global traffic, and loss of the small-batch vmode path.

```diff
diff --git a/genvox_amd/csrc/dec_resident.hip b/genvox_amd/csrc/dec_resident.hip
--- a/genvox_amd/csrc/dec_resident.hip
+++ b/genvox_amd/csrc/dec_resident.hip
@@ -26,9 +26,11 @@
     static constexpr int OFF_HS2 = OFF_HS + 32 * 8 * 4 * RT;
     static constexpr int OFF_CTRL = OFF_HS2 + 32 * 4 * 4;
     static constexpr int LDS_BYTES = OFF_CTRL + 256;
+    static constexpr int OFF_CEDE = LDS_BYTES, CEDE_WAVE = 16 * 512;
 };
 constexpr int RS_LDS_BYTES = RsCfg<0>::LDS_BYTES > RsCfg<2>::LDS_BYTES ? RsCfg<0>::LDS_BYTES : RsCfg<2>::LDS_BYTES;
 static_assert(RS_LDS_BYTES <= 160 * 1024 && RsCfg<1>::LDS_BYTES <= RS_LDS_BYTES && RsCfg<3>::LDS_BYTES <= RS_LDS_BYTES, "resident decoder LDS");
+static_assert(RsCfg<1>::OFF_CEDE + RS_WAVES * RsCfg<1>::CEDE_WAVE <= RS_LDS_BYTES, "ceded half fragments in LDS");
 constexpr int RC_HA = 0;
 constexpr int RC_CTX = 1;
 constexpr int RC_HD = 2;
@@ -39,6 +41,7 @@
 constexpr int RC_Y1 = 7;
 constexpr int RC_EXIT = 8;
 constexpr int RC_WANT = 10;
+constexpr int RC_CEDE = 11;
 
 struct RsArgs {
     const float* att_frag; const float* att_bias; const float* wq_t; const float* dec_frag; const float* dec_bias;
@@ -79,6 +82,7 @@
     unsigned limit; int B, T, bid;
     int n_att;
     int sleep;
+    const unsigned* f_cede;
 };
 
 __device__ __forceinline__ bool rs_count(int* ctrl, int word, unsigned v, unsigned Tu, int lane) {
@@ -88,9 +92,10 @@
     if (lane == 0 && n != s0) __hip_atomic_store(ctrl + word, (int)n, __ATOMIC_RELEASE, __HIP_MEMORY_SCOPE_WORKGROUP);
     return n != s0;
 }
+template <bool XC>
 __device__ __forceinline__ void rs_poll_once(int* ctrl, const RsPoll& q, int lane, int mask) {
     constexpr unsigned none = 0xffffffffu;
-    unsigned va = none, vd = none, vc = none, vp = none, vy = none;
+    unsigned va = none, vd = none, vc = none, vp = none, vy = none, vx = none;
     if (mask & (1 << RC_HA)) {
         const unsigned a0 = __hip_atomic_load(q.f_att + lane, __ATOMIC_RELAXED, __HIP_MEMORY_SCOPE_AGENT);
         const unsigned a1 = lane + 64 < q.n_att ? __hip_atomic_load(q.f_att + 64 + lane, __ATOMIC_RELAXED, __HIP_MEMORY_SCOPE_AGENT) : none;
@@ -102,6 +107,7 @@
         vd = min(d0, d1);
     }
     if (mask & (1 << RC_CTX)) vc = lane < q.B ? __hip_atomic_load(q.f_ctx + lane * 32, __ATOMIC_RELAXED, __HIP_MEMORY_SCOPE_AGENT) : none;
+    if (XC && (mask & (1 << RC_CEDE))) vx = __hip_atomic_load(q.f_cede, __ATOMIC_RELAXED, __HIP_MEMORY_SCOPE_AGENT);
     if (q.f_pre) {
         if (mask & (1 << RC_PRE)) vp = lane < 8 ? __hip_atomic_load(q.f_pre + lane * 32, __ATOMIC_RELAXED, __HIP_MEMORY_SCOPE_AGENT) : none;
         if (mask & (1 << RC_Y1)) vy = lane < q.B ? __hip_atomic_load(q.f_y1 + lane * 32, __ATOMIC_RELAXED, __HIP_MEMORY_SCOPE_AGENT) : none;
@@ -112,6 +118,7 @@
     if (mask & (1 << RC_HA)) moved |= rs_count(ctrl, RC_HA, va, Tu, lane);
     if (mask & (1 << RC_HD)) moved |= rs_count(ctrl, RC_HD, vd, Tu, lane);
     if (mask & (1 << RC_CTX)) moved |= rs_count(ctrl, RC_CTX, vc, Tu, lane);
+    if (XC && (mask & (1 << RC_CEDE))) moved |= rs_count(ctrl, RC_CEDE, vx, Tu, lane);
     if (q.f_pre) {
         if (mask & (1 << RC_PRE)) moved |= rs_count(ctrl, RC_PRE, vp, Tu, lane);
         if (mask & (1 << RC_Y1)) moved |= rs_count(ctrl, RC_Y1, vy, Tu, lane);
@@ -132,6 +139,7 @@
     if (give_up && lane == 0) __hip_atomic_store(ctrl + RC_ABORT, 1, __ATOMIC_RELEASE, __HIP_MEMORY_SCOPE_WORKGROUP);
 }
 
+template <bool XC = false>
 __device__ __forceinline__ void rs_gate(int* ctrl, int word, int need, const RsPoll& q, int lane) {
     while (__hip_atomic_load(ctrl + word, __ATOMIC_ACQUIRE, __HIP_MEMORY_SCOPE_WORKGROUP) < need) {
         if (__hip_atomic_load(ctrl + RC_ABORT, __ATOMIC_RELAXED, __HIP_MEMORY_SCOPE_WORKGROUP) != 0) return;
@@ -144,7 +152,7 @@
         }
         got = __builtin_amdgcn_readfirstlane(got);
         if (got) {
-            rs_poll_once(ctrl, q, lane, got);
+            rs_poll_once<XC>(ctrl, q, lane, got);
             if (lane == 0) __hip_atomic_store(ctrl + RC_LOCK, 0, __ATOMIC_RELEASE, __HIP_MEMORY_SCOPE_WORKGROUP);
             if (q.sleep == 8) __builtin_amdgcn_s_sleep(8);
             else if (q.sleep == 32) __builtin_amdgcn_s_sleep(32);
@@ -182,6 +190,11 @@
     acc2 = __builtin_amdgcn_mfma_f32_32x32x2f32((W).y, (X).y, acc2, 0, 0, 0); \
     acc2 = __builtin_amdgcn_mfma_f32_32x32x2f32((W).z, (X).z, acc2, 0, 0, 0); \
     acc2 = __builtin_amdgcn_mfma_f32_32x32x2f32((W).w, (X).w, acc2, 0, 0, 0);
+#define RS_MFMA16C(W, X)                                                \
+    ac = __builtin_amdgcn_mfma_f32_16x16x1f32((W).x, (X).x, ac, 0, 0, 0); \
+    ac = __builtin_amdgcn_mfma_f32_16x16x1f32((W).y, (X).y, ac, 0, 0, 0); \
+    ac = __builtin_amdgcn_mfma_f32_16x16x1f32((W).z, (X).z, ac, 0, 0, 0); \
+    ac = __builtin_amdgcn_mfma_f32_16x16x1f32((W).w, (X).w, ac, 0, 0, 0);
 #define RS_MFMA16(W, X)                                                     \
     acc2 = __builtin_amdgcn_mfma_f32_16x16x1f32((W).x, (X).x, acc2, 0, 0, 0); \
     acc2 = __builtin_amdgcn_mfma_f32_16x16x1f32((W).y, (X).y, acc2, 0, 0, 0); \
@@ -201,9 +214,11 @@
 
 typedef const __attribute__((address_space(4))) RsArgs* RsKarg;
 
-template <int KIND, bool AR, bool TR = false, bool KA = AR>
+template <int KIND, bool AR, bool TR = false, bool KA = AR, bool CEDE = false>
 __device__ __forceinline__ void rs_body(const RsArgs& p, char* smem, const int bid) {
     static_assert(!(AR && TR), "the tape belongs to the teacher-forced loop");
+    static_assert(!CEDE || (!AR && !TR && KIND <= 2), "k-groups are ceded in the teacher-forced inference loop's 224-workgroup deal only");
+    constexpr bool CEDE_GIVE = CEDE && KIND == 0, CEDE_TAKE = CEDE && KIND == 1;
     using Cfg = RsCfg<KIND>;
     constexpr bool XH = Cfg::XH, ATT = Cfg::ATT;
     constexpr int NN = Cfg::NN, NC = Cfg::NC, NRN = Cfg::NRN, NLN = Cfg::NLN;
@@ -234,11 +249,12 @@
     const RsPoll poll{p.sync + RS_FLAG_ATT + rep * 128, p.sync + RS_FLAG_DEC + rep * 128, p.sync + RS_FLAG_CTX + (bid % RS_REP1) * 32 * 32, tmo_w,
                       AR ? p.sync + RS_FLAG_PRE + (bid % RS_REP_PRE) * 8 * 32 : nullptr, AR ? p.sync + RS_FLAG_Y1 : nullptr, AR ? p.sync + HANDOFF_STOP : nullptr,
                       (p.spin_limit ? p.spin_limit : HANDOFF_SPIN_LIMIT) * 16u, B, T, bid, dec0,
-                      (!ATT && (p.debug & 16)) ? 32 : ((p.debug & 8) ? 8 : 0)};
+                      (!ATT && (p.debug & 16)) ? 32 : ((p.debug & 8) ? 8 : 0),
+                      CEDE_GIVE ? p.sync + RS_FLAG_CEDE + (bid >> 1) * 32 : nullptr};
     const int bl = lane & 31, h = lane >> 5;
     const bool x_mine = ((lane >> 4) & 1) == xhalf;
     const int mlane = x_mine ? lane : (lane ^ 16);
-    const bool vmode = B <= 2 && !(p.debug & 64), two_rows = B == 2;
+    const bool vmode = !CEDE && B <= 2 && !(p.debug & 64), two_rows = B == 2;
     const unsigned x_lane = (unsigned)((vmode ? (two_rows ? (bl & 1) : 0) : (bl < B ? bl : 0)) * 8 + 4 * h) * 4u;
 
     const float4* wsrc = reinterpret_cast<const float4*>(ATT ? p.att_frag : p.dec_frag);
@@ -274,6 +290,15 @@
         lw[i * RT * 64 + lane] = wt[(long)kni(NRN + i) * 64];
         if (RT == 2) lw[(i * RT + 1) * 64 + lane] = wt2[(long)kni(NRN + i) * 64];
         if (XH && x_mine) lh[i * 32 + hidx] = wx[(long)kni(NRN + i) * 64];
+    }
+    if constexpr (CEDE_TAKE) {
+        const int cw = 4 + (wave & 3);
+        float4* lc = reinterpret_cast<float4*>(smem + Cfg::OFF_CEDE + wave * Cfg::CEDE_WAVE);
+        const float4* wxc = wsrc + (long)(3 * (bid - 64) + 1) * nkgw * 64 + lane;
+        if (((lane >> 4) & 1) == (wave >> 2)) {
+#pragma unroll
+            for (int i = 0; i < 16; ++i) lc[i * 32 + (lane & 15) + 16 * (lane >> 5)] = wxc[(long)(kg_pre + 64 + 16 * cw + i) * 64];
+        }
     }
 
     constexpr int NP = (PP && KIND == 1) ? 4 : 1;
@@ -316,7 +341,7 @@
         RS_WGSTAMP(0);
         RsKarg ka = nullptr;
         if (KA) { ka = (RsKarg)__builtin_amdgcn_kernarg_segment_ptr(); asm volatile("" : "+s"(ka)); }
-        if (ATT && !AR && !TR && t >= RS_HA_SLOTS && (wave == 6 || ((XH || RT == 2) && wave == 7))) rs_gate(ctrl, RC_HD, t + 1 - RS_HA_SLOTS, poll, lane);
+        if (ATT && !AR && !TR && t >= RS_HA_SLOTS && (wave == 6 || ((XH || RT == 2) && wave == 7))) rs_gate<CEDE_GIVE>(ctrl, RC_HD, t + 1 - RS_HA_SLOTS, poll, lane);
         float4 add4 = bias4;
         if (PP && XH) {
             const unsigned kg = (unsigned)(4 * wave);
@@ -343,7 +368,7 @@
         for (int q = 0; q < 16; ++q) { acc[q] = 0.f; acc2[q] = 0.f; }
         float av[2] = {0.f, 0.f}, av2[2] = {0.f, 0.f};
         auto prenet_part = [&]() __attribute__((always_inline)) {
-            rs_gate(ctrl, RC_PRE, t, poll, lane);
+            rs_gate<CEDE_GIVE>(ctrl, RC_PRE, t, poll, lane);
             RS_ARSTAMP(2);
             const __amdgpu_buffer_rsrc_t rx = make_rsrc(ka->prenet + (long)(4 * wave) * B * 8);
             float4 xp[4];
@@ -376,8 +401,41 @@
             else if (ARD) { xsrc = p.h_a + (long)((t + 1) % RS_HA_SLOTS) * RS_A * B + (long)(16 * wave) * B * 8; word = RC_HA; need = t + 1; }
             else if (wave < 4) { xsrc = p.h_a + (long)(TR ? t + 1 : (t + 1) % RS_HA_SLOTS) * RS_A * B + (long)(32 * wave) * B * 8; word = RC_HA; need = t + 1; }
             else { xsrc = p.hc + (long)t * B * (RS_D + RS_E) + (long)(32 * (wave - 4)) * B * 8; word = RC_HD; need = t; }
-            rs_gate(ctrl, word, need, poll, lane);
+            rs_gate<CEDE_GIVE>(ctrl, word, need, poll, lane);
             if (sub == NSUB - 1) { RS_STAMP(1); RS_WGSTAMP(1); }
+            if constexpr (CEDE_TAKE) {
+                const int cb = 2 * (bid - 64) + (wave >> 2), cw = 4 + (wave & 3);
+                int tc = tid;
+                asm volatile("" : "+v"(tc));
+                const int cl = tc & 63, cml = ((cl >> 4) & 1) == (wave >> 2) ? cl : (cl ^ 16);
+                const float4* lc = reinterpret_cast<const float4*>(smem + Cfg::OFF_CEDE + wave * Cfg::CEDE_WAVE) + (cml & 15) + 16 * (cml >> 5);
+                const __amdgpu_buffer_rsrc_t rxc = make_rsrc(p.h_a + (long)(t % RS_HA_SLOTS) * RS_A * B + (long)(16 * cw) * B * 8);
+                f32x16 ac;
+#pragma unroll
+                for (int q = 0; q < 16; ++q) ac[q] = 0.f;
+                float4 xq[2][4];
+#pragma unroll
+                for (int u = 0; u < 4; ++u) xq[0][u] = load_sc1(rxc, x_lane + (unsigned)u * blkb);
+#pragma unroll
+                for (int gi = 0; gi < 4; ++gi) {
+                    if (gi + 1 < 4) {
+#pragma unroll
+                        for (int u = 0; u < 4; ++u) xq[(gi + 1) & 1][u] = load_sc1(rxc, x_lane + (unsigned)(4 * (gi + 1) + u) * blkb);
+                    }
+#pragma unroll
+                    for (int u = 0; u < 4; ++u) {
+                        const float4 hl = lc[(4 * gi + u) * 32];
+                        const float4 xv = xq[gi & 1][u];
+                        RS_MFMA16C(hl, xv)
+                    }
+                }
+                const __amdgpu_buffer_rsrc_t rf = make_rsrc(p.p_slab + ((long)((t & 1) * 64 + cb) * 4 + (cw - 4)) * 32 * B);
+#pragma unroll
+                for (int q4 = 0; q4 < 4; ++q4) {
+                    const int b = 16 * (q4 & 1) + (cl & 15);
+                    if (b < B) store_sc1(rf, (unsigned)(((q4 >> 1) * B + b) * 4 + (cl >> 4)) * 16u, make_float4(ac[4 * q4], ac[4 * q4 + 1], ac[4 * q4 + 2], ac[4 * q4 + 3]));
+                }
+            }
             const __amdgpu_buffer_rsrc_t rx = make_rsrc(xsrc);
             constexpr int XG = (XH || RT == 2) ? 2 : 4;
             constexpr int XD = ARD ? 3 : 2;
@@ -389,6 +447,14 @@
                 for (int u = 0; u < XG; ++u) xb[d][u] = load_sc1(rx, x_lane + (unsigned)(XG * d + u) * blkb);
 #pragma unroll
             for (int gi = 0; gi < NNS / XG; ++gi) {
+                if constexpr (CEDE_TAKE) if (gi == 1) {
+                    asm volatile("s_waitcnt vmcnt(0)" ::: "memory");
+                    rs_cbar();
+                    int tf = tid;
+                    asm volatile("" : "+v"(tf));
+                    if (tf < 1) __hip_atomic_store(p.sync + RS_FLAG_CEDE + (bid - 64) * 32, (unsigned)t + 1u, __ATOMIC_RELAXED, __HIP_MEMORY_SCOPE_AGENT);
+                    RS_STAMP(10);
+                }
                 if (gi + XD - 1 < NNS / XG) {
 #pragma unroll
                     for (int u = 0; u < XG; ++u) xb[(gi + XD - 1) % XD][u] = load_sc1(rx, x_lane + (unsigned)(XG * (gi + XD - 1) + u) * blkb);
@@ -399,14 +465,25 @@
                     const float4 xv = xb[gi % XD][u];
                     if (i < NRN) {
                         RS_MUL32(wn[i], xv)
-                        if (XH) { RS_MUL16(hn[i < NRH ? i : 0], xv) }
+                        if (XH && (!CEDE_GIVE || wave < 4)) { RS_MUL16(hn[i < NRH ? i : 0], xv) }
                         if (RT == 2) { RS_MUL32B(wn2[i < NR2 ? i : 0], xv) }
                     } else {
                         const float4 wl = lw[(i - NRN) * RT * 64 + lane];
                         RS_MUL32(wl, xv)
-                        if (XH) { const float4 hl = lh[(i - NRN) * 32 + hidx]; RS_MUL16(hl, xv) }
+                        if (XH && (!CEDE_GIVE || wave < 4)) { const float4 hl = lh[(i - NRN) * 32 + hidx]; RS_MUL16(hl, xv) }
                         if (RT == 2) { const float4 wl2 = lw[((i - NRN) * RT + 1) * 64 + lane]; RS_MUL32B(wl2, xv) }
                     }
+                }
+            }
+            if constexpr (CEDE_GIVE) if (wave >= 4) {
+                rs_gate<CEDE_GIVE>(ctrl, RC_CEDE, t + 1, poll, lane);
+                RS_STAMP(10);
+                const __amdgpu_buffer_rsrc_t rf = make_rsrc(p.p_slab + ((long)((t & 1) * 64 + bid) * 4 + (wave - 4)) * 32 * B);
+#pragma unroll
+                for (int q4 = 0; q4 < 4; ++q4) {
+                    const int b = 16 * (q4 & 1) + (lane & 15);
+                    const float4 f = load_sc1(rf, (unsigned)(((q4 >> 1) * B + (b < B ? b : 0)) * 4 + (lane >> 4)) * 16u);
+                    acc2[4 * q4] = f.x; acc2[4 * q4 + 1] = f.y; acc2[4 * q4 + 2] = f.z; acc2[4 * q4 + 3] = f.w;
                 }
             }
         }
@@ -414,10 +491,10 @@
         RS_STAMP(2);
         {
             const float* xsrc = p.hc + (long)(ATT ? t : t + 1) * B * (RS_D + RS_E) + (long)RS_D * B + (long)(8 * wave) * B * 8;
-            if (ATT) rs_gate(ctrl, RC_CTX, t, poll, lane);
-            else if (AR) rs_gate(ctrl, RC_CTX, t + 1, poll, lane);
-            else if (t + 2 <= T) rs_gate(ctrl, RC_HA, t + 2, poll, lane);
-            else rs_gate(ctrl, RC_CTX, t + 1, poll, lane);
+            if (ATT) rs_gate<CEDE_GIVE>(ctrl, RC_CTX, t, poll, lane);
+            else if (AR) rs_gate<CEDE_GIVE>(ctrl, RC_CTX, t + 1, poll, lane);
+            else if (t + 2 <= T) rs_gate<CEDE_GIVE>(ctrl, RC_HA, t + 2, poll, lane);
+            else rs_gate<CEDE_GIVE>(ctrl, RC_CTX, t + 1, poll, lane);
             RS_STAMP(3);
             RS_WGSTAMP(2);
             const __amdgpu_buffer_rsrc_t rx = make_rsrc(xsrc);
@@ -446,7 +523,7 @@
             if (l2_wg && t >= 1) {
                 unsigned km = 0;
                 if (wave < 4 && bl < B) km = *reinterpret_cast<const unsigned*>(ka->keep1 + ((long)t * B + bl) * RS_P + 32 * (bid - 64) + 8 * wave + 4 * h);
-                rs_gate(ctrl, RC_Y1, t, poll, lane);
+                rs_gate<CEDE_GIVE>(ctrl, RC_Y1, t, poll, lane);
                 RS_ARSTAMP(0);
                 const __amdgpu_buffer_rsrc_t ry = make_rsrc(ka->y1 + (long)(4 * wave) * B * 8);
                 float4 xy[4];
@@ -532,7 +609,9 @@
         }
         }
         };
-        if (vmode) body(RsBool<true>{}); else body(RsBool<false>{});
+        if constexpr (CEDE) body(RsBool<false>{});
+        else if (vmode) body(RsBool<true>{});
+        else body(RsBool<false>{});
 
         int te = tid;
         asm volatile("" : "+v"(te));
@@ -703,15 +782,15 @@
     if (cell2_wave && b2 < B) c_mem[(long)b2 * H + j2] = c_state;
 }
 
-template <bool TR>
+template <bool TR, bool CEDE = false>
 __device__ __forceinline__ void rs_kernel_224(const RsArgs& p, char* rs_smem) {
     const int bid = (int)blockIdx.x;
     const int kind = bid < 64 ? 0 : (bid < 96 ? 1 : 2);
     const int off_ctrl = kind == 0 ? RsCfg<0>::OFF_CTRL : (kind == 1 ? RsCfg<1>::OFF_CTRL : RsCfg<2>::OFF_CTRL);
     if (threadIdx.x < 64) reinterpret_cast<int*>(rs_smem + off_ctrl)[threadIdx.x] = 0;
     __syncthreads();
-    if (kind == 0) rs_body<0, false, TR, !TR>(p, rs_smem, bid);
-    else if (kind == 1) rs_body<1, false, TR, !TR>(p, rs_smem, bid);
+    if (kind == 0) rs_body<0, false, TR, !TR, CEDE>(p, rs_smem, bid);
+    else if (kind == 1) rs_body<1, false, TR, !TR, CEDE>(p, rs_smem, bid);
     else rs_body<2, false, TR, !TR>(p, rs_smem, bid);
 }
 template <bool TR>
@@ -727,6 +806,10 @@
 __global__ __launch_bounds__(RS_THREADS) void decoder_resident_kernel(RsArgs p) {
     extern __shared__ __attribute__((aligned(16))) char rs_smem[];
     rs_kernel_224<false>(p, rs_smem);
+}
+__global__ __launch_bounds__(RS_THREADS) void decoder_resident_cede_kernel(RsArgs p) {
+    extern __shared__ __attribute__((aligned(16))) char rs_smem[];
+    rs_kernel_224<false, true>(p, rs_smem);
 }
 __global__ __launch_bounds__(RS_THREADS) void decoder_resident_pairs_kernel(RsArgs p) {
     extern __shared__ __attribute__((aligned(16))) char rs_smem[];
@@ -770,6 +853,7 @@
     hipError_t e = hipFuncSetAttribute(reinterpret_cast<const void*>(decoder_resident_kernel), hipFuncAttributeMaxDynamicSharedMemorySize, RS_LDS_BYTES);
     if (e != hipSuccess) return e;
     for (const void* k : {reinterpret_cast<const void*>(decoder_resident_train_kernel), reinterpret_cast<const void*>(decoder_resident_pairs_kernel),
+                          reinterpret_cast<const void*>(decoder_resident_cede_kernel),
                           reinterpret_cast<const void*>(decoder_resident_train_pairs_kernel)})
         if ((e = hipFuncSetAttribute(k, hipFuncAttributeMaxDynamicSharedMemorySize, RS_LDS_BYTES)) != hipSuccess) return e;
     return hipFuncSetAttribute(reinterpret_cast<const void*>(decoder_ar_resident_kernel), hipFuncAttributeMaxDynamicSharedMemorySize, RS_LDS_BYTES);
@@ -797,6 +881,9 @@
         else decoder_resident_train_kernel<<<grid, dim3(RS_THREADS), RS_LDS_BYTES, s>>>(a);
     } else if (p.layout == 2) {
         decoder_resident_pairs_kernel<<<grid, dim3(RS_THREADS), RS_LDS_BYTES, s>>>(a);
+    } else if (p.cede && p.B >= 3) {
+        a.p_slab = p.cede;
+        decoder_resident_cede_kernel<<<grid, dim3(RS_THREADS), RS_LDS_BYTES, s>>>(a);
     } else {
         decoder_resident_kernel<<<grid, dim3(RS_THREADS), RS_LDS_BYTES, s>>>(a);
     }
diff --git a/genvox_amd/csrc/gvx_api.hip b/genvox_amd/csrc/gvx_api.hip
--- a/genvox_amd/csrc/gvx_api.hip
+++ b/genvox_amd/csrc/gvx_api.hip
@@ -159,6 +159,7 @@
     m->train_resident_loop = flag("GVX_TRAIN_RESIDENT_LOOP", true);
     m->tf_rows64 = flag("GVX_TF_ROWS64", false);
     m->tf_resident = flag("GVX_TF_RESIDENT", true);
+    m->tf_cede = flag("GVX_TF_CEDE", true);
     m->ar_resident_loop = flag("GVX_AR_RESIDENT_LOOP", true);
     m->tf_long_rows_224 = flag("GVX_TF_LONG_224", true);
     m->attn_prefetch = flag("GVX_ATTN_PREFETCH", true);
diff --git a/genvox_amd/csrc/gvx_decoder.hip b/genvox_amd/csrc/gvx_decoder.hip
--- a/genvox_amd/csrc/gvx_decoder.hip
+++ b/genvox_amd/csrc/gvx_decoder.hip
@@ -389,6 +389,9 @@
     }
     rp.dec_frag_bytes = (unsigned)(frag_floats(4 * d.dec_rnn_dim, d.att_rnn_dim + d.embed_dim + d.dec_rnn_dim) * sizeof(float));
     rp.layout = c.plan.tile_layout;
+    static_assert(RS_CEDE_SLOT_FLOATS_PER_ROW == 2 * 4 * 1024, "a hand-over slot of the ceded k-groups is att_part / dec_part at 1024 units");
+    const bool slots = d.att_rnn_dim == 1024 && d.dec_rnn_dim == 1024 && c.db.dec_part == c.db.att_part + (size_t)c.B * RS_CEDE_SLOT_FLOATS_PER_ROW;
+    rp.cede = m->tf_cede && !c.train && rp.layout == 1 && c.B >= 3 && slots ? c.db.att_part : nullptr;
     if (m->ktiming) HIP_TRY(hipEventRecord(m->kev[0], s));
     HIP_TRY(launch_decoder_resident(rp, s));
     if (m->ktiming) {
diff --git a/genvox_amd/csrc/gvx_internal.h b/genvox_amd/csrc/gvx_internal.h
--- a/genvox_amd/csrc/gvx_internal.h
+++ b/genvox_amd/csrc/gvx_internal.h
@@ -63,6 +63,7 @@
     bool ar_split_h = true;
     bool tf_rows64 = false;
     bool tf_resident = true;
+    bool tf_cede = true;
     bool ar_resident_loop = true;
     bool tf_long_rows_224 = true;
     bool train_resident = true;
diff --git a/genvox_amd/csrc/gvx_kernels.h b/genvox_amd/csrc/gvx_kernels.h
--- a/genvox_amd/csrc/gvx_kernels.h
+++ b/genvox_amd/csrc/gvx_kernels.h
@@ -172,7 +172,9 @@
 constexpr int RS_FLAG_PRE = RS_FLAG_Y1 + 32 * 32;
 constexpr int RS_REP_P = 4;
 constexpr int RS_FLAG_P = RS_FLAG_PRE + RS_REP_PRE * 8 * 32;
-static_assert(RS_FLAG_P + RS_REP_P * 128 * 32 <= HANDOFF_WORDS, "flag replicas inside the hand-off block");
+constexpr int RS_FLAG_CEDE = RS_FLAG_P + RS_REP_P * 128 * 32;
+static_assert(RS_FLAG_CEDE + 32 * 32 <= HANDOFF_WORDS, "flag replicas inside the hand-off block");
+constexpr size_t RS_CEDE_SLOT_FLOATS_PER_ROW = 64 * 4 * 2 * 16;
 constexpr int RS_HA_SLOTS = 8;
 struct DecResidentParams {
     const float* att_frag; const float* att_bias; const float* wq_t;
@@ -182,6 +184,7 @@
     float* hc;
     float* q_slab;
     float* c_a; float* c_d;
+    float* cede;
     unsigned* sync;
     unsigned att_frag_bytes, dec_frag_bytes;
     int B, T;
```

Measured after the change: 1.824 million. -2.0%, worse.
